# ZikangYuan/sr_livo

Hardware: AMD Instinct MI355X
Metric: sweeps/s (full ESIKF solve of a 64k-pt Livox sweep vs 1M-pt voxel map) (higher is better)
Workload: dtype f64; 1 GPU; HEADLINE: stream of 4 distinct 65536-keypoint livox sweeps (own poses and priors), 978481-pt voxel map (1000000 target), max_num_residuals=2147483647, r=1, K=20; one full ESIKF solve per sweep, every sweep crosses PCIe once (uploaded on the copy stream during the solve before it: resident in HBM when its solve starts); sweeps drawn with seeds 20251309 + 100 j, keeping those that take sweep 0's 2 E; parallelism=single GPU

## Files before the change

include/srlivo_hip_debug.h:

```cpp
#ifndef SRLIVO_HIP_DEBUG_H
#define SRLIVO_HIP_DEBUG_H

#include "srlivo_hip.h"

#ifdef __cplusplus
extern "C" {
#endif

int srl_debug_set_select_mode(srl_ctx *ctx, int select_mode);

int srl_debug_radix_sort_pairs(srl_ctx *ctx, const uint32_t *keys, int n, int bits, uint32_t *keys_sorted, uint32_t *positions_sorted);

int srl_debug_color_map_rebuilds(srl_ctx *ctx, int32_t *voxel_table, int32_t *grid_table);

int srl_debug_set_frame_order_mode(srl_ctx *ctx, int mode);
int srl_debug_frame_order_used(srl_ctx *ctx, int *used);

int srl_debug_set_gather_counts(srl_ctx *ctx, int nranks, int rank, const int64_t *counts);

int srl_debug_set_ablate(srl_ctx *ctx, int bits);
int srl_debug_set_fused_reduce(srl_ctx *ctx, int enable);
int srl_debug_set_bound_culling(srl_ctx *ctx, int enable);
int srl_debug_set_pose_box(srl_ctx *ctx, int kind);
int srl_debug_set_arm_linger(srl_ctx *ctx, double host_linger_us, double kernel_linger_us);
int srl_debug_pass_stamps(srl_ctx *ctx, int enable, long long *gpu_out, long long *host_out);
int srl_debug_frame_timing(srl_ctx *ctx, int enable, double out16[16]);
int srl_debug_set_frame_epoch(srl_ctx *ctx, int frames_to_wrap);
int srl_debug_set_launch_shape(srl_ctx *ctx, int keypoints_per_wave, int waves_per_workgroup);
int srl_debug_set_search_select_mode(srl_ctx *ctx, int select_mode);
int srl_debug_heap_topk(const double *distances, int n, int K, int32_t *out_index);
int srl_debug_device_sqrt(srl_ctx *ctx, const double *in, int n, double *out);
int srl_debug_block_times(srl_ctx *ctx, double *out, int max_blocks, int *nblocks);

#ifdef __cplusplus
}
#endif
#endif
```

sr_livo_amd/capi.py:

```python
import ctypes as C
import os
import re

import numpy as np

_HERE = os.path.dirname(os.path.abspath(__file__))
LIB_PATH = os.environ.get("SRL_LIB_PATH") or os.path.join(_HERE, "libsrlivo_hip.so")
INCLUDE_DIR = os.path.join(os.path.dirname(_HERE), "include")

SRL_OK = 0
SRL_ERR_NO_DEVICE = -1
SRL_ERR_BAD_ARG = -3
SRL_ERR_UNSUPPORTED = -4
SRL_ERR_COMM = -7
SRL_ERR_NAN_PLANARITY = -8
SRL_ERR_NOT_ENOUGH_RESIDUALS = -9
SRL_COMM_ID_BYTES = 128


SRL_PEER_HANDLE_BYTES = 64


class SrlError(RuntimeError):
    def __init__(self, status, what, detail=""):
# ... 184 lines not shown
        "srl_fetch_residuals": ([p, p, p, p, p, p, p], C.c_int),
        "srl_search_neighbors": ([p, p, C.c_int, C.c_int, C.c_double, C.c_int, C.c_int, p, p, p], C.c_int),
        "srl_transform_points": ([p, p, C.c_int, dp, dp, dp, dp, p], C.c_int),
        "srl_frame_upload": ([p, p, C.c_int], C.c_int),
        "srl_frame_undistort": ([p, p, p, p, C.c_int, p, C.c_int, C.c_double, C.c_int, dp, dp, p, p], C.c_int),
        "srl_frame_take": ([p, p, C.c_int], C.c_int),
        "srl_frame_subsample": ([p, p, C.c_int, C.c_double, C.POINTER(C.c_int)], C.c_int),
        "srl_frame_take_subsampled": ([p, p, C.c_int, p, p, p], C.c_int),
        "srl_frame_size": ([p, C.POINTER(C.c_int)], C.c_int),
        "srl_frame_select_keypoints": ([p, dp, dp, dp, dp, C.c_double, p, C.POINTER(C.c_int)], C.c_int),
        "srl_frame_commit_report": ([p, dp, dp, dp, dp, C.c_double, C.c_int, C.c_double, C.c_int, p, p, p, C.POINTER(C.c_int),
                                     C.POINTER(C.c_int)], C.c_int),
        "srl_frame_commit": ([p, dp, dp, dp, dp, C.c_double, C.c_int, C.c_double, C.c_int, p, C.POINTER(C.c_int)], C.c_int),
        "srl_comm_unique_id": ([p], C.c_int),
        "srl_comm_init_rank": ([p, C.c_int, C.c_int, p], C.c_int),
        "srl_comm_destroy": ([p], C.c_int),
        "srl_comm_set_library": ([C.c_char_p], C.c_int),
        "srl_comm_suspend": ([p, C.c_int], C.c_int),
        "srl_comm_info": ([p, C.POINTER(C.c_int), C.POINTER(C.c_int), C.POINTER(C.c_int), C.POINTER(C.c_int), C.POINTER(C.c_int64)], C.c_int),
        "srl_comm_set_host_callbacks": ([p, C.c_int, C.c_int, ALLREDUCE_FN, ALLGATHER_FN, p], C.c_int),
        "srl_debug_set_gather_counts": ([p, C.c_int, C.c_int, C.POINTER(C.c_int64)], C.c_int),
        "srl_peer_export": ([p, p, C.POINTER(p)], C.c_int),
        "srl_peer_attach": ([p, C.c_int, C.c_int, p, C.POINTER(p)], C.c_int),
        "srl_peer_set_deadline_ms": ([p, C.c_int], C.c_int),
        "srl_peer_stats": ([p, C.POINTER(C.c_int64), C.POINTER(C.c_int)], C.c_int),
        "srl_peer_detach": ([p], C.c_int),
        "srl_shard_range": ([C.c_int, C.c_int, C.c_int, C.POINTER(C.c_int), C.POINTER(C.c_int)], None),
        "srl_shard_budget": ([C.c_int, C.POINTER(C.c_int64), C.c_int, C.c_int, C.POINTER(C.c_int64), C.POINTER(C.c_int)], None),
        "srl_get_timing": ([p, C.POINTER(Timing)], C.c_int),
        "srl_debug_block_times": ([p, p, C.c_int, C.POINTER(C.c_int)], C.c_int),
        "srl_debug_set_ablate": ([p, C.c_int], C.c_int),
        "srl_debug_set_fused_reduce": ([p, C.c_int], C.c_int),
        "srl_debug_set_bound_culling": ([p, C.c_int], C.c_int),
        "srl_debug_set_pose_box": ([p, C.c_int], C.c_int),
        "srl_debug_set_arm_linger": ([p, C.c_double, C.c_double], C.c_int),
        "srl_debug_pass_stamps": ([p, C.c_int, p, p], C.c_int),
        "srl_debug_frame_timing": ([p, C.c_int, p], C.c_int),
        "srl_debug_set_frame_epoch": ([p, C.c_int], C.c_int),
        "srl_set_armed_launch": ([p, C.c_int], C.c_int),
        "srl_disarm": ([p], C.c_int),
        "srl_solve_end": ([p], C.c_int),
        "srl_get_arm_stats": ([p, C.POINTER(C.c_uint64)], C.c_int),
        "srl_debug_set_launch_shape": ([p, C.c_int, C.c_int], C.c_int),
        "srl_debug_set_search_select_mode": ([p, C.c_int], C.c_int),
        "srl_debug_set_select_mode": ([p, C.c_int], C.c_int),
        "srl_debug_set_frame_order_mode": ([p, C.c_int], C.c_int),
        "srl_debug_radix_sort_pairs": ([p, p, C.c_int, C.c_int, p, p], C.c_int),
        "srl_debug_frame_order_used": ([p, C.POINTER(C.c_int)], C.c_int),
        "srl_debug_heap_topk": ([p, C.c_int, C.c_int, p], C.c_int),
        "srl_debug_device_sqrt": ([p, p, C.c_int, p], C.c_int),
        "srl_set_profiling": ([p, C.c_int], C.c_int),
        "srl_set_profiling_period": ([p, C.c_int], C.c_int),
        "srl_timing_mark": ([p], C.c_int),
        "srl_lio_create": ([C.c_int, C.POINTER(p)], C.c_int),
        "srl_lio_destroy": ([p], C.c_int),
        "srl_lio_ctx": ([p], p),
        "srl_lio_last_error": ([p], C.c_char_p),
        "srl_lio_set_extrinsics": ([p, dp, dp], C.c_int),
        "srl_lio_set_laser_point_cov": ([p, C.c_double], C.c_int),
        "srl_lio_last_solve_launches": ([p, C.POINTER(C.c_int)], C.c_int),
        "srl_lio_eskf_get_state": ([p, dp], C.c_int),
        "srl_lio_eskf_set_state": ([p, dp], C.c_int),
        "srl_lio_eskf_get_cov": ([p, dp], C.c_int),
        "srl_lio_eskf_set_cov": ([p, dp], C.c_int),
        "srl_lio_eskf_set_noise": ([p, C.c_double, C.c_double, C.c_double, C.c_double], C.c_int),
        "srl_lio_eskf_init_imu": ([p, dp, dp], C.c_int),
# ... 463 lines not shown
        return node.value if rc == 0 else None

    def fetch_neighbors(self, K=20):
        _, n, _ = self.sweep_shard()
        ids = np.empty((n, K), dtype=np.int32)
        status = np.empty(n, dtype=np.uint8)
        ncand = np.empty(n, dtype=np.int32)
        self._chk(self.lib.srl_fetch_neighbors(self.h, _ptr(ids), _ptr(status), _ptr(ncand)), "srl_fetch_neighbors")
        return ids, status, ncand

    def fetch_residuals(self):
        _, n, _ = self.sweep_shard()
        normal = np.empty((n, 3)); a2d = np.empty(n); w = np.empty(n); off = np.empty(n); d = np.empty(n); J = np.empty((n, 6))
        self._chk(self.lib.srl_fetch_residuals(self.h, _ptr(normal), _ptr(a2d), _ptr(w), _ptr(off), _ptr(d), _ptr(J)), "srl_fetch_residuals")
        return dict(normal=normal, a2D=a2d, weight=w, norm_offset=off, distance=d, jacobian=J)

    def search_neighbors(self, world_xyz, nb=1, size=1.0, K=20, thr=1):
        q = _f64(world_xyz, (-1, 3))
        ids = np.empty((len(q), K), dtype=np.int32)
        xyz = np.empty((len(q), K, 3), dtype=np.float32)
        nf = np.empty(len(q), dtype=np.int32)
        self._chk(self.lib.srl_search_neighbors(self.h, _ptr(q), len(q), nb, size, K, thr, _ptr(ids), _ptr(xyz), _ptr(nf)), "srl_search_neighbors")
        return ids, xyz, nf

    def set_launch_shape(self, kpw, wpb):
        self._chk(self.lib.srl_debug_set_launch_shape(self.h, int(kpw), int(wpb)), "srl_debug_set_launch_shape")

    def set_fused_reduce(self, on):
        self._chk(self.lib.srl_debug_set_fused_reduce(self.h, 1 if on else 0), "srl_debug_set_fused_reduce")

    def set_bound_culling(self, on):
        self._chk(self.lib.srl_debug_set_bound_culling(self.h, 1 if on else 0), "srl_debug_set_bound_culling")

    def set_search_select_mode(self, mode):
        self._chk(self.lib.srl_debug_set_search_select_mode(self.h, int(mode)), "srl_debug_set_search_select_mode")

    def set_armed_launch(self, on):
        mode = int(on) if on in (0, 1, 2) and not isinstance(on, bool) else (1 if on else 0)
        self._chk(self.lib.srl_set_armed_launch(self.h, mode), "srl_set_armed_launch")

    def solve_end(self):
        self._chk(self.lib.srl_solve_end(self.h), "srl_solve_end")

    def disarm(self):
        self._chk(self.lib.srl_disarm(self.h), "srl_disarm")

    def arm_stats(self):
        out = (C.c_uint64 * 4)()
        self._chk(self.lib.srl_get_arm_stats(self.h, out), "srl_get_arm_stats")
        return dict(zip(("armed", "fired", "cancelled", "expired"), (int(v) for v in out)))

    def set_pose_box(self, kind):
        self._chk(self.lib.srl_debug_set_pose_box(self.h, int(kind)), "srl_debug_set_pose_box")

    FRAME_STAGES = ("upload", "select_group", "select_download", "select_host_order", "select_gather", "commit_transform", "commit_download",
                    "insert_sort", "insert_segments", "insert_lookup_create", "insert_replay")

    def set_frame_epoch(self, frames_to_wrap):
        self._chk(self.lib.srl_debug_set_frame_epoch(self.h, int(frames_to_wrap)), "srl_debug_set_frame_epoch")

    def frame_timing(self, enable=True):
        out = np.zeros(16)
        self._chk(self.lib.srl_debug_frame_timing(self.h, 1 if enable else 0, _ptr(out)), "srl_debug_frame_timing")
        return dict(zip(self.FRAME_STAGES, (float(v) for v in out)))

    def pass_stamps(self, enable=True, read=True):
# ... 582 lines not shown
```

sr_livo_amd/csrc/srl_capi.cpp:

```cpp
#include "../../include/srlivo_hip.h"
#include "../../include/srlivo_hip_debug.h"
#include "host/srl_la.h"
#include "srl_device.h"
#include "srl_hash.h"
#include "srl_heap.h"

#include <hip/hip_runtime.h>
#include <sched.h>

#include <algorithm>
#include <atomic>
#include <chrono>
#include <climits>
#include <cstdio>
#include <cstdlib>
#include <cstring>
#include <mutex>
#include <string>
#include <vector>

struct SrlMapState;
int srl_map_insert_device(struct srl_ctx *ctx, const double *world_xyz, int n, double voxel_size, int cap,
                          double min_distance_points, int min_num_points, int *num_added);

#include "srl_ctx.h"
int srl_map_insert_report_device(srl_ctx *ctx, const double *world_xyz, int n, double voxel_size, int cap, double min_distance_points, int min_num_points,
                                 double ref_z, uint8_t *outcome, srl_cloud_point *cloud, int *num_cloud, int *num_added);

namespace {

unsigned next_pow2(unsigned v) { unsigned p = 1; while (p < v) p <<= 1; return p; }
inline long long steady_ns() { return std::chrono::duration_cast<std::chrono::nanoseconds>(std::chrono::steady_clock::now().time_since_epoch()).count(); }

constexpr int SRL_MAX_DEVICES = 64;
std::atomic<int> g_live_ctx[SRL_MAX_DEVICES];
inline int live_contexts(int device) { return (device >= 0 && device < SRL_MAX_DEVICES) ? g_live_ctx[device].load(std::memory_order_relaxed) : 1; }

int ensure_work(srl_ctx *ctx, int n) {
    if (n <= ctx->work_cap) return SRL_OK;
    const int cap = std::max(n, 1024);
    const int nblocks = std::max((cap + SRL_KPB - 1) / SRL_KPB, 1024 + 8);
    int rc;
    if ((rc = ensure(ctx, ctx->d_rec, (size_t)cap * 8))) return rc;
    if ((rc = ensure(ctx, ctx->d_status, (size_t)cap))) return rc;
    if ((rc = ensure(ctx, ctx->d_bound, (size_t)cap * 4))) return rc;
    ctx->bound_n = 0;
    if ((rc = ensure(ctx, ctx->d_partials, (size_t)nblocks * SRL_PART_STRIDE))) return rc;
    if ((rc = ensure(ctx, ctx->d_binfo, (size_t)nblocks))) return rc;
    ctx->work_cap = cap;
    ctx->block_cap = nblocks;
    return SRL_OK;
}

bool srl_is_pinned(const void *p) {
    hipPointerAttribute_t attr;
    if (hipPointerGetAttributes(&attr, p) != hipSuccess) { (void)hipGetLastError(); return false; }
    return attr.type == hipMemoryTypeHost;
}

int srl_ring_init(srl_ctx *ctx) {
    if (ctx->h_ring) return SRL_OK;
    HIPCHK(ctx, hipHostMalloc((void **)&ctx->h_ring, (size_t)srl_ctx::RING_SLOTS * srl_ctx::RING_SLOT_BYTES, hipHostMallocDefault));
    for (int i = 0; i < srl_ctx::RING_SLOTS; i++) { HIPCHK(ctx, hipEventCreateWithFlags(&ctx->ring_ev[i], hipEventDisableTiming)); ctx->ring_busy[i] = false; }
    return SRL_OK;
}

int ensure_taps(srl_ctx *ctx, int n, int K) {
    if (n <= ctx->tap_cap && K <= ctx->tap_K) return SRL_OK;
    const int cap = std::max(n, ctx->tap_cap), kk = std::max(K, ctx->tap_K);
    int rc;
    if ((rc = ensure(ctx, ctx->d_tap_ids, (size_t)cap * kk))) return rc;
    if ((rc = ensure(ctx, ctx->d_tap_ncand, (size_t)cap))) return rc;
    if ((rc = ensure(ctx, ctx->d_tap_normal, (size_t)cap * 3))) return rc;
    if ((rc = ensure(ctx, ctx->d_tap_a2d, (size_t)cap))) return rc;
    if ((rc = ensure(ctx, ctx->d_tap_offset, (size_t)cap))) return rc;
    ctx->tap_cap = cap;
    ctx->tap_K = kk;
    return SRL_OK;
}
// ... 66 lines not shown
    }
    {
        const size_t row_bytes = (size_t)(SRL_FUSED_MAX_BLOCKS + SRL_FUSED_MAX_GROUPS) * SRL_ROW_GRANULES * 8;
        if (hipMalloc((void **)&ctx->d_granules, row_bytes) != hipSuccess || hipMemset(ctx->d_granules, 0, row_bytes) != hipSuccess) { delete ctx; return SRL_ERR_HIP; }
    }
    if (hipHostMalloc((void **)&ctx->h_mail, sizeof(SrlMailbox), hipHostMallocCoherent | hipHostMallocMapped) != hipSuccess) {
        delete ctx;
        return SRL_ERR_HIP;
    }
    std::memset(ctx->h_mail, 0, sizeof(SrlMailbox));
    for (int i = 0; i < 4; i++) hipEventCreate(&ctx->ev[i]);
    if (device < SRL_MAX_DEVICES) g_live_ctx[device].fetch_add(1, std::memory_order_relaxed);
    ctx->counted = true;
    *out = ctx;
    return SRL_OK;
}

int srl_ctx_destroy(srl_ctx *ctx) {
    if (!ctx) return SRL_OK;
    hipSetDevice(ctx->device);
    if (ctx->counted && ctx->device < SRL_MAX_DEVICES) g_live_ctx[ctx->device].fetch_sub(1, std::memory_order_relaxed);
    if (ctx->armed) srl_ctx_disarm(ctx);
    if (ctx->stream) hipStreamSynchronize(ctx->stream);
    if (ctx->copy_stream) hipStreamSynchronize(ctx->copy_stream);
    if (ctx->color) srl_color_map_destroy(ctx);
    if (ctx->pose_box_pinned) hipHostFree(ctx->pose_box_pinned);
    if (ctx->pose_box_dev) hipFree(ctx->pose_box_dev);
    if (ctx->d_pose_relay) hipFree(ctx->d_pose_relay);
    if (ctx->comm && srl_rccl()) srl_rccl()->CommDestroy(ctx->comm);
    if (ctx->parked_comm && srl_rccl()) srl_rccl()->CommDestroy(ctx->parked_comm);
    if (ctx->d_sub_kept) hipFree(ctx->d_sub_kept);
    if (ctx->d_sub_seen) hipFree(ctx->d_sub_seen);
    void *bufs[] = {ctx->d_corr_in, ctx->d_corr_rel, ctx->d_corr_imu, ctx->d_corr_raw, ctx->d_corr_seg, ctx->d_frame_raw, ctx->d_frame_world, ctx->d_table, ctx->d_slabs, ctx->d_raw, ctx->d_rec, ctx->d_status, ctx->d_partials, ctx->d_binfo,
                    ctx->d_out, ctx->d_count, ctx->d_bound, ctx->d_granules, ctx->d_rec_granules, ctx->d_raw_next, ctx->d_stage_next, ctx->d_stage_cur, ctx->d_tap_ids, ctx->d_tap_ncand, ctx->d_tap_normal, ctx->d_tap_a2d,
                    ctx->d_tap_offset, ctx->d_gather, ctx->d_peer, ctx->d_mail};
    for (int r = 0; r < SRL_MAX_PEERS; r++) if (ctx->peer_mapped[r]) hipIpcCloseMemHandle(ctx->peer_mapped[r]);
    if (ctx->d_inbox) hipFree(ctx->d_inbox);
    for (void *b : bufs) if (b) hipFree(b);
    if (ctx->h_out) hipHostFree(ctx->h_out);
    if (ctx->h_count) hipHostFree(ctx->h_count);
    if (ctx->h_mail) hipHostFree(ctx->h_mail);
    if (ctx->h_arm_stamps) hipHostFree(ctx->h_arm_stamps);
    if (ctx->h_scratch) hipHostFree(ctx->h_scratch);
    if (ctx->h_frame_x) hipHostFree(ctx->h_frame_x);
    for (SrlEpochTable *t : {&ctx->sel_table, &ctx->ins_table}) { if (t->keyw) hipFree(t->keyw); if (t->minw) hipFree(t->minw); }
    if (ctx->d_frame_sync) hipFree(ctx->d_frame_sync);
    if (ctx->d_tr1_sched) hipFree(ctx->d_tr1_sched);
    if (ctx->h_insert_cnt) hipHostFree(ctx->h_insert_cnt);
    if (ctx->ev_insert) hipEventDestroy(ctx->ev_insert);
    if (ctx->ev_world) hipEventDestroy(ctx->ev_world);
    if (ctx->ev_frame_read) hipEventDestroy(ctx->ev_frame_read);
    if (ctx->h_ring) { hipHostFree(ctx->h_ring); for (int i = 0; i < srl_ctx::RING_SLOTS; i++) if (ctx->ring_ev[i]) hipEventDestroy(ctx->ring_ev[i]); }
    for (auto &b : ctx->pool_free) hipFree(b.p);
    ctx->pool_free.clear();
    for (int i = 0; i < 4; i++) if (ctx->ev[i]) hipEventDestroy(ctx->ev[i]);
    for (int i = 0; i < srl_ctx::PROF_RING; i++) for (int k = 0; k < 2; k++) if (ctx->ring[i][k]) hipEventDestroy(ctx->ring[i][k]);
    for (int sl = 0; sl < 2; sl++) for (int k = 0; k < 2; k++) if (ctx->up_ev[sl][k]) hipEventDestroy(ctx->up_ev[sl][k]);
    if (ctx->upload_ev) hipEventDestroy(ctx->upload_ev);
    if (ctx->copy_stream) { hipStreamSynchronize(ctx->copy_stream); hipStreamDestroy(ctx->copy_stream); }
    if (ctx->prefix_stream) { hipStreamSynchronize(ctx->prefix_stream); hipStreamDestroy(ctx->prefix_stream); }
    if (ctx->stream) hipStreamDestroy(ctx->stream);
    delete ctx;
    return SRL_OK;
}

const char *srl_last_error(const srl_ctx *ctx) { return ctx ? ctx->err.c_str() : "null context"; }

int srl_map_upload(srl_ctx *ctx, const int16_t *keys_xyz, const int32_t *counts, const float *xyz, int V, int cap) {
    if (!ctx || V < 0 || (V > 0 && (!keys_xyz || !counts || !xyz))) return SRL_ERR_BAD_ARG;
    SRL_DISARM(ctx);
    if (cap != SRL_VOXEL_CAP) { ctx->err = "max_num_points_in_voxel must be 20"; return SRL_ERR_UNSUPPORTED; }
    HIPCHK(ctx, hipSetDevice(ctx->device));
    { const int rcs = srl_map_settle(ctx); if (rcs) return rcs; }
    ctx->bound_n = 0;
    const unsigned slab_cap = std::max<unsigned>(1024u, (unsigned)V + (unsigned)V / 2u + 4096u);
    if (slab_cap > SRL_MAX_SLABS) { ctx->err = "map too large: slab byte offsets are 32-bit (16.7 M voxels)"; return SRL_ERR_UNSUPPORTED; }
    const unsigned table_cap = next_pow2(std::max<unsigned>(2048u, SRL_TABLE_FACTOR * slab_cap));
    std::vector<SrlSlab> slabs((size_t)V);
    std::vector<SrlMapSlot> table((size_t)table_cap);
    for (auto &s : table) { s.key = SRL_EMPTY_KEY; s.slab = 0; s.count = 0; }
    long long npts = 0;
    const unsigned mask = table_cap - 1;
    for (int v = 0; v < V; v++) {
        SrlSlab &s = slabs[v];
        std::memset(&s, 0, sizeof s);
        const int c = counts[v];
        if (c < 0 || c > cap) { ctx->err = "voxel count out of range"; return SRL_ERR_BAD_ARG; }
        for (int i = 0; i < c; i++)
            for (int d = 0; d < 3; d++) s.xyz[i][d] = xyz[((size_t)v * cap + i) * 3 + d];
        s.count = (unsigned)c;
        s.key = srl_pack_key(keys_xyz[3 * v], keys_xyz[3 * v + 1], keys_xyz[3 * v + 2]);
        npts += c;
        unsigned h = srl_hash_key(s.key) & mask;
        while (table[h].key != SRL_EMPTY_KEY) {
            if (table[h].key == s.key) { ctx->err = "duplicate voxel key in upload"; return SRL_ERR_BAD_ARG; }
            h = (h + 1) & mask;
        }
        table[h].key = s.key;
        table[h].slab = (unsigned)v;
        table[h].count = (unsigned)c;
    }
    if (ctx->d_slabs) { HIPCHK(ctx, hipFree(ctx->d_slabs)); ctx->d_slabs = nullptr; }
    if (ctx->d_table) { HIPCHK(ctx, hipFree(ctx->d_table)); ctx->d_table = nullptr; }
    HIPCHK(ctx, hipMalloc((void **)&ctx->d_slabs, ((size_t)slab_cap + 1) * SRL_SLAB_BYTES));
    HIPCHK(ctx, hipMemsetD32Async((hipDeviceptr_t)(ctx->d_slabs + (size_t)slab_cap * SRL_SLAB_BYTES), 0x7f800000, SRL_SLAB_BYTES / 4, ctx->stream));
    HIPCHK(ctx, hipMalloc((void **)&ctx->d_table, (size_t)table_cap * sizeof(SrlMapSlot)));
    HIPCHK(ctx, hipMemsetAsync(ctx->d_slabs, 0, (size_t)slab_cap * SRL_SLAB_BYTES, ctx->stream));
// ... 78 lines not shown
        std::memcpy(ctx->h_ring + (size_t)slot * srl_ctx::RING_SLOT_BYTES, src + off, len);
        {
            hipError_t e__ = hipMemcpyAsync(reinterpret_cast<char *>(d_stage) + off, ctx->h_ring + (size_t)slot * srl_ctx::RING_SLOT_BYTES, len,
                                            hipMemcpyHostToDevice, st);
            if (e__ != hipSuccess) {
                char buf[256];
                std::snprintf(buf, sizeof buf, "ring upload: %s (dst %p + %zu, ring %p slot %d, len %zu, stream %p, main stream %p)", hipGetErrorString(e__),
                              (void *)d_stage, off, (void *)ctx->h_ring, slot, len, (void *)st, (void *)ctx->stream);
                ctx->err = buf;
                return SRL_ERR_HIP;
            }
        }
        HIPCHK(ctx, hipEventRecord(ctx->ring_ev[slot], st));
        ctx->ring_busy[slot] = true;
        off += len;
    }
    return SRL_OK;
}
}

int srl_sweep_upload(srl_ctx *ctx, const double *raw_xyz, int n) {
    if (!ctx || n < 0 || (n > 0 && !raw_xyz)) return SRL_ERR_BAD_ARG;
    SRL_DISARM(ctx);
    HIPCHK(ctx, hipSetDevice(ctx->device));
    int b = 0, cnt = 0;
    srl_shard_range(n, ctx->nranks, ctx->rank, &b, &cnt);
    ctx->total_n = n;
    ctx->shard_begin = b;
    ctx->n = cnt;
    ctx->sweep_loaded = true;
    ctx->taps_valid = false;
    ctx->passes_in_solve = 0;
    ctx->tail_pending = false;
    ctx->bound_n = 0;
    if (cnt > ctx->sweep_cap) {
        const int cap = std::max(cnt, 1024);
        int rc = ensure(ctx, ctx->d_raw, (size_t)cap * 3);
        if (rc) return rc;
        ctx->sweep_cap = cap;
    }
    int rc = ensure_work(ctx, cnt);
    if (rc) return rc;
    if (cnt > 0) {
        int rcu = upload_aos(ctx, reinterpret_cast<const char *>(raw_xyz + (size_t)b * 3), (size_t)cnt * 3 * sizeof(double), ctx->d_rec, ctx->stream);
        if (rcu) return rcu;
        HIPCHK(ctx, srl_launch_aos_to_soa(ctx->d_rec, cnt, ctx->d_raw, ctx->d_raw + ctx->sweep_cap, ctx->d_raw + 2 * (size_t)ctx->sweep_cap, ctx->stream));
    }
    ctx->soa_valid_n = cnt;
    return SRL_OK;
}

int srl_sweep_wait(srl_ctx *ctx) {
    if (!ctx) return SRL_ERR_BAD_ARG;
    SRL_DISARM(ctx);
    if (ctx->upload_pending) {
        HIPCHK(ctx, hipSetDevice(ctx->device));
        HIPCHK(ctx, hipEventSynchronize(ctx->upload_ev));
        if (ctx->prefix_stream) HIPCHK(ctx, hipStreamSynchronize(ctx->prefix_stream));
        ctx->upload_pending = false;
    }
    return SRL_OK;
}

int srl_sweep_prefetch(srl_ctx *ctx, const double *raw_xyz, int n) {
    if (!ctx || n < 0 || (n > 0 && !raw_xyz)) return SRL_ERR_BAD_ARG;
    HIPCHK(ctx, hipSetDevice(ctx->device));
    if (!ctx->copy_stream) SRL_DISARM(ctx);
// ... 31 lines not shown
            ctx->up_one_dma[slot] = true;
        }
    } else {
        ctx->up_one_dma[slot] = true;
    }
    HIPCHK(ctx, hipEventRecord(ctx->up_ev[slot][1], ctx->copy_stream));
    ctx->next_ready = ctx->up_ev[slot][1];
    ctx->next_slot = slot; ctx->next_prefix_n = ctx->up_one_dma[slot] ? cnt : pre;
    ctx->next_n = cnt; ctx->next_begin = b; ctx->next_total = n;
    return SRL_OK;
}

int srl_sweep_swap(srl_ctx *ctx) {
    if (!ctx) return SRL_ERR_BAD_ARG;
    if (ctx->next_n < 0) { SRL_DISARM(ctx); ctx->err = "srl_sweep_swap: nothing prefetched"; return SRL_ERR_NO_SWEEP; }
    HIPCHK(ctx, hipSetDevice(ctx->device));
    const bool one_dma = ctx->up_one_dma[ctx->next_slot];
    hipEvent_t ev_full = ctx->up_ev[ctx->next_slot][1], ev_pre = ctx->up_ev[ctx->next_slot][one_dma ? 1 : 0];
    hipError_t up_pre = hipEventQuery(ev_pre);
    hipError_t up = (one_dma || up_pre != hipSuccess) ? up_pre : hipEventQuery(ev_full);
    if (up_pre == hipErrorNotReady && ctx->armed && ctx->next_n <= ctx->work_cap) {
        const long long t_give_up = steady_ns() + 25000;
        while ((up_pre = hipEventQuery(ev_pre)) == hipErrorNotReady && steady_ns() < t_give_up) { }
    }
    for (hipError_t e : {up, up_pre})
        if (e != hipSuccess && e != hipErrorNotReady) { ctx->err = std::string("hipEventQuery: ") + hipGetErrorString(e); return SRL_ERR_HIP; }
    if (up_pre != hipSuccess || ctx->next_n > ctx->work_cap) SRL_DISARM(ctx);
    if (up_pre != hipSuccess) {
        HIPCHK(ctx, hipStreamWaitEvent(ctx->stream, ev_full, 0));
        if (!one_dma) HIPCHK(ctx, hipStreamWaitEvent(ctx->stream, ev_pre, 0));
        up = hipSuccess;
    }
    ctx->tail_pending = up != hipSuccess;
    ctx->bound_n = 0;
    ctx->cur_slot = ctx->next_slot;
    ctx->cur_prefix_n = up == hipSuccess ? ctx->next_n : ctx->next_prefix_n;
    ctx->passes_in_solve = 0;
    std::swap(ctx->d_raw, ctx->d_raw_next);
    std::swap(ctx->sweep_cap, ctx->next_cap);
    std::swap(ctx->d_stage_cur, ctx->d_stage_next);
    std::swap(ctx->stage_cur_cap, ctx->stage_next_cap);
    ctx->soa_valid_n = 0;
    ctx->n = ctx->next_n; ctx->shard_begin = ctx->next_begin; ctx->total_n = ctx->next_total;
    ctx->next_n = -1;
    ctx->sweep_loaded = true;
    ctx->taps_valid = false;
    return ensure_work(ctx, ctx->n);
}

int srl_thread_pin_to_gpu_numa(srl_ctx *ctx, int *numa_node) {
    if (!ctx) return SRL_ERR_BAD_ARG;
    if (numa_node) *numa_node = -1;
    char bus[64] = {0};
    if (hipDeviceGetPCIBusId(bus, (int)sizeof bus, ctx->device) != hipSuccess) { (void)hipGetLastError(); return SRL_ERR_UNSUPPORTED; }
    for (char *c = bus; *c; ++c) if (*c >= 'A' && *c <= 'F') *c = (char)(*c - 'A' + 'a');
    const std::string base = std::string("/sys/bus/pci/devices/") + bus;
    int node = -1;
    if (FILE *f = std::fopen((base + "/numa_node").c_str(), "r")) { if (std::fscanf(f, "%d", &node) != 1) node = -1; std::fclose(f); }
    char list[1024] = {0};
    if (FILE *f = std::fopen((base + "/local_cpulist").c_str(), "r")) { if (!std::fgets(list, (int)sizeof list, f)) list[0] = 0; std::fclose(f); }
    if (node < 0 || !list[0]) return SRL_ERR_UNSUPPORTED;
    cpu_set_t allowed, want;
    CPU_ZERO(&want);
    if (sched_getaffinity(0, sizeof allowed, &allowed) != 0) return SRL_ERR_UNSUPPORTED;
    int any = 0;
    for (const char *p = list; *p && *p != '\n';) {
        char *end = nullptr;
// ... 380 lines not shown
    a.size_voxel = o->size_voxel_map;
    a.max_dist = o->max_dist_to_plane_icp;
    {
        double lw = std::abs(o->weight_alpha), ln = std::abs(o->weight_neighborhood);
        const double sum = lw + ln;
        lw /= sum;
        ln /= sum;
        a.lambda_w = lw;
        a.lambda_n = ln;
    }
    a.power_planarity = o->power_planarity;
    a.nbr_scale = o->max_dist_to_plane_icp * o->min_number_neighbors;
    a.K = p.K;
    a.min_nb = o->min_number_neighbors;
    a.thr_cap = p.thr;
    a.select_mode = ctx->select_mode;
    a.ablate = ctx->ablate;
    a.stamps = ctx->h_arm_stamps;
    a.rec = ctx->d_rec;
    a.status = ctx->d_status;
    a.partials = ctx->d_partials;
    a.binfo = ctx->d_binfo;
    if (ctx->taps) {
        a.tap_ids = ctx->d_tap_ids;
        a.tap_ncand = ctx->d_tap_ncand;
        a.tap_normal = ctx->d_tap_normal;
        a.tap_a2d = ctx->d_tap_a2d;
        a.tap_offset = ctx->d_tap_offset;
    }
    {
        float sv = (float)o->size_voxel_map;
        int sv_bits; std::memcpy(&sv_bits, &sv, 4);
        const int sig[4] = {p.K, p.nb, p.thr, sv_bits};
        if (std::memcmp(sig, ctx->bound_sig, sizeof sig) != 0) { ctx->bound_n = 0; std::memcpy(ctx->bound_sig, sig, sizeof sig); }
        a.bound_out = ctx->d_bound;
        a.bound_in = ctx->bound_mode != 0 ? ctx->d_bound : nullptr;
        a.bound_use = a.bound_in ? std::min(ctx->bound_n, n_eff) : 0;
    }
    if (p.fused) {
        a.granules = ctx->d_granules;
        a.mailbox = p.transport == Transport::rccl ? ctx->d_mail : ctx->h_mail;
        a.mail_tagged = p.tagged_mail ? 1 : 0;
    }
    if (p.fuse_cut) {
        a.rec_granules = ctx->d_rec_granules;
        a.cut_max = o->max_num_residuals;
    }
}

static int grow_pass_buffers(srl_ctx *ctx, const PassPlan &p) {
    int rc;
    ctx->taps_valid = false;
    if (ctx->taps) {
        if ((rc = ensure_taps(ctx, ctx->n, p.K))) return rc;
        if (ctx->n > 0) {
            HIPCHK(ctx, hipMemsetAsync(ctx->d_tap_ids, 0xFF, (size_t)ctx->n * p.K * sizeof(int), ctx->stream));
            HIPCHK(ctx, hipMemsetAsync(ctx->d_tap_normal, 0, (size_t)ctx->n * 3 * sizeof(double), ctx->stream));
            HIPCHK(ctx, hipMemsetAsync(ctx->d_tap_a2d, 0, (size_t)ctx->n * sizeof(double), ctx->stream));
            HIPCHK(ctx, hipMemsetAsync(ctx->d_tap_offset, 0, (size_t)ctx->n * sizeof(double), ctx->stream));
        }
    }
    ctx->last_nblocks = p.nblocks;
    if (p.nblocks > ctx->block_cap) {
        if ((rc = ensure(ctx, ctx->d_partials, (size_t)p.nblocks * SRL_PART_STRIDE))) return rc;
        if ((rc = ensure(ctx, ctx->d_binfo, (size_t)p.nblocks))) return rc;
        ctx->block_cap = p.nblocks;
    }
    if (ctx->profiling == 2 && ctx->ring_head - ctx->ring_tail >= (unsigned)srl_ctx::PROF_RING && (rc = drain_ring(ctx, true))) return rc;
    if (p.fused && p.transport == Transport::rccl && !ctx->d_mail && (rc = ensure(ctx, ctx->d_mail, 1))) return rc;
    const size_t need = (size_t)p.nblocks * p.kpb * 16;
    if (p.fuse_cut && need > ctx->rec_granule_cap) {
        if ((rc = ensure(ctx, ctx->d_rec_granules, need))) return rc;
        HIPCHK(ctx, hipMemsetAsync(ctx->d_rec_granules, 0, need * sizeof(unsigned long long), ctx->stream));
        ctx->rec_granule_cap = need;
    }
    return SRL_OK;
}

struct ExchangeTag { unsigned long long seq; unsigned epoch; int slot; };
static ExchangeTag exchange_tag(unsigned long long seq) {
    if ((unsigned)seq == 0u) ++seq;
    return {seq, (unsigned)seq, (int)(seq & 1ull)};
}
static ExchangeTag next_exchange(srl_ctx *ctx) {
    const ExchangeTag t = exchange_tag(ctx->peer_seq + 1);
    ctx->peer_seq = t.seq;
    return t;
}

static SrlAssocArgs arm_signature(const SrlAssocArgs &src) {
    SrlAssocArgs sg = src;
    std::memset(sg.Rn, 0, sizeof sg.Rn); std::memset(sg.R, 0, sizeof sg.R); std::memset(sg.t, 0, sizeof sg.t);
    std::memset(sg.t_last, 0, sizeof sg.t_last);
    sg.pose_box = nullptr; sg.pose_relay = nullptr; sg.pose_relayed = 0; sg.pose_epoch = 0; sg.arm_linger_ticks = 0;
    sg.raw_x = sg.raw_y = sg.raw_z = nullptr; sg.alt_x = sg.alt_y = sg.alt_z = nullptr; sg.n = 0; sg.aos = nullptr; sg.alt_aos = nullptr;
    sg.bound_use = 0;
    return sg;
}

static int fire_or_cancel(srl_ctx *ctx, const PassPlan &p, SrlAssocArgs &a, unsigned long long &seq_now, bool &fired) {
    fired = false;
    bool needs_tail = false;
    if (ctx->tail_pending) {
        if (hipEventQuery(ctx->up_ev[ctx->cur_slot][1]) == hipSuccess) { ctx->tail_pending = false; ctx->cur_prefix_n = ctx->n; }
        else needs_tail = a.n > ctx->cur_prefix_n;
        (void)hipGetLastError();
    }
    if (!ctx->armed) return SRL_OK;
    const SrlAssocArgs sg = arm_signature(a);
    const double age_us = (double)(steady_ns() - ctx->armed_at_ns) * 1e-3;
    const bool on_raw = a.raw_x == ctx->armed_raw && ctx->sweep_cap == ctx->armed_raw_cap && a.aos == nullptr;
    const bool on_alt = !on_raw && ctx->armed_alt != nullptr && a.raw_x == ctx->armed_alt && ctx->sweep_cap == ctx->armed_alt_cap &&
                        a.aos != nullptr && a.aos == ctx->armed_alt_aos;
    if (p.arm_ok && !needs_tail && age_us < ctx->arm_host_linger_us && p.nb == ctx->armed_nb && p.kpw == ctx->armed_kpw &&
        p.nblocks <= ctx->armed_nblocks && (on_raw || on_alt) && std::memcmp(&sg, &ctx->armed_sig, sizeof sg) == 0) {
        pose_box_write(ctx, a.Rn, a.R, a.t, (unsigned)seq_now, SRL_ARM_GO | (on_alt ? SRL_ARM_ALT : 0u), (unsigned)a.n, a.t_last);
        ctx->armed = false;
        ctx->armed_ring = -1;
        ctx->arm_stats[1]++;
        ctx->cur_measured = ctx->armed_measured;
        ctx->cur_gen = ctx->armed_gen;
        fired = true;
        return SRL_OK;
    }
    if (const int rc = srl_ctx_disarm(ctx)) return rc;
    seq_now = ++ctx->seq;
    if (p.fused) a.seq = seq_now;
    return SRL_OK;
}

static int prof_role(const srl_ctx *ctx) {
    if (ctx->prof_period <= 1) return 2;
    const unsigned long long r = ctx->prof_count % (unsigned long long)ctx->prof_period;
    return r == 1 ? 2 : (r == 0 ? 1 : 0);
}

static int launch_assoc(srl_ctx *ctx, const PassPlan &p, const SrlAssocArgs &args, bool armed) {
    if (!armed && ctx->tail_pending) {
        HIPCHK(ctx, hipStreamWaitEvent(ctx->stream, ctx->up_ev[ctx->cur_slot][1], 0));
        ctx->tail_pending = false; ctx->cur_prefix_n = ctx->n;
    }
    const bool prof = ctx->profiling == 1, prof_light = ctx->profiling == 2;
    const int role = prof_light ? prof_role(ctx) : 0;
    int prev = -1;
    if (armed && role != 0) {
        int rc;
        if (ctx->ring_head - ctx->ring_tail >= (unsigned)srl_ctx::PROF_RING - 2 && (rc = drain_ring(ctx, true))) return rc;
        if (ctx->ring_head != 0 && !ctx->ring_void[(ctx->ring_head - 1) % srl_ctx::PROF_RING] && ctx->ring_last_count == (long long)ctx->prof_count - 1)
            prev = (int)((ctx->ring_head - 1) % srl_ctx::PROF_RING);
    }
    const unsigned slot = ctx->ring_head % srl_ctx::PROF_RING;
    if (prof) HIPCHK(ctx, hipEventRecord(ctx->ev[0], ctx->stream));
    if (role == 2 && prev < 0) HIPCHK(ctx, hipEventRecord(ctx->ring[slot][0], ctx->stream));
    HIPCHK(ctx, srl_launch_assoc(args, p.nb, p.kpw, p.wpb, ctx->stream));
    if (prof) HIPCHK(ctx, hipEventRecord(ctx->ev[1], ctx->stream));
    if (role != 0) {
        HIPCHK(ctx, hipEventRecord(ctx->ring[slot][1], ctx->stream));
        ctx->ring_prev[slot] = prev; ctx->ring_marker[slot] = role == 1; ctx->ring_void[slot] = false; ctx->ring_gen[slot] = ctx->timing_gen;
        ctx->ring_last_count = (long long)ctx->prof_count;
        ctx->ring_head++;
    }
    if (prof_light) ctx->prof_count++;
    const bool measured = !prof_light || role == 2;
    if (armed) { ctx->armed_ring = role != 0 ? (int)slot : -1; ctx->armed_measured = measured; ctx->armed_gen = ctx->timing_gen; }
    else { ctx->cur_measured = measured; ctx->cur_gen = ctx->timing_gen; }
    return SRL_OK;
}

static bool arm_wanted(const srl_ctx *ctx) {
    return ctx->arm_mode == 2 ||
           (live_contexts(ctx->device) <= 1 && !ctx->peer_shares_device && !ctx->comm_shares_device &&
            (ctx->next_n >= 0 || ctx->expected_passes == 0 || ctx->passes_in_solve + 1 < ctx->expected_passes));
}

static int arm_next(srl_ctx *ctx, const PassPlan &p, const SrlAssocArgs &a) {
    int rc;
    if ((rc = ensure_pose_box(ctx))) return rc;
    SrlAssocArgs nx = a;
    nx.seq = ctx->seq + 1;
    nx.bound_use = a.bound_in ? a.n : 0;
    const bool has_alt = ctx->d_raw_next != nullptr && ctx->next_cap > 0 && ctx->d_stage_next != nullptr;
    nx.aos = nullptr;
    nx.alt_aos = has_alt ? ctx->d_stage_next : nullptr;
    nx.alt_x = has_alt ? ctx->d_raw_next : nullptr;
    nx.alt_y = has_alt ? ctx->d_raw_next + ctx->next_cap : nullptr;
    nx.alt_z = has_alt ? ctx->d_raw_next + 2 * (size_t)ctx->next_cap : nullptr;
    if (p.transport == Transport::peer) {
        const ExchangeTag t = exchange_tag(ctx->peer_seq + 1);
        nx.peer_epoch = t.epoch;
        nx.peer_slot = t.slot;
    }
    nx.pose_box = ctx->h_pose_box;
    nx.pose_relay = ctx->d_pose_relay;
    nx.pose_relayed = ctx->pose_box_kind == 1 ? 0 : 1;
    nx.pose_epoch = (unsigned)nx.seq;
    nx.arm_linger_ticks = ctx->arm_linger_ticks;
    if ((rc = launch_assoc(ctx, p, nx, true))) return rc;
    ctx->armed_sig = arm_signature(nx);
    ctx->armed_nb = p.nb; ctx->armed_kpw = p.kpw; ctx->armed_nblocks = p.nblocks;
    ctx->armed_raw = nx.raw_x; ctx->armed_raw_cap = ctx->sweep_cap;
    ctx->armed_alt = nx.alt_x; ctx->armed_alt_cap = has_alt ? ctx->next_cap : 0; ctx->armed_alt_aos = nx.alt_aos;
    ctx->armed_at_ns = steady_ns();
    ctx->armed = true;
    ctx->arm_stats[0]++;
    return SRL_OK;
}

static int reduce_unfused(srl_ctx *ctx, const PassPlan &p, const srl_icp_opts *o, int n_eff, unsigned long long seq) {
    int64_t budget = o->max_num_residuals;
    int mode = 0;
    const long long *gather = nullptr;
    if (p.transport == Transport::single || !p.cut) {
        srl_shard_budget(o->max_num_residuals, nullptr, ctx->nranks, ctx->rank, &budget, &mode);
// ... 113 lines not shown
    if (ctx->h_out->pad != 0 || ctx->h_out->d_timeout > 0.5) {
        ctx->err = "fused final reduction timed out waiting for a workgroup's row";
        if (fired && p.transport == Transport::rccl) ctx->arm_stats[3]++;
        return SRL_INTERNAL_FUSED_TIMEOUT;
    }
    return SRL_OK;
}

static int finish_pass(srl_ctx *ctx, const PassPlan &p, const srl_icp_opts *o, const SrlAssocArgs &a, int n_eff, long long last_visited_local,
                       unsigned long long seq, bool fired, srl_normal_eq *out) {
    const SrlDevOut &r = *ctx->h_out;
    const long long visited_total = (long long)(r.d_visited + 0.5);
    if (p.fused && !p.fuse_cut) {
        const long long expect = ctx->nranks > 1 ? (long long)ctx->total_n : (long long)n_eff;
        if (visited_total != expect) {
            char buf[256];
            std::snprintf(buf, sizeof buf, "fused pass visited %lld of %lld keypoints (fired %d, seq %llu; residuals %.0f, time-out flag %.0f, marker %lld)", visited_total, expect,
                          (int)fired, seq, r.d_num_res, r.d_timeout, (long long)r.pad);
            ctx->err = buf;
            return SRL_ERR_HIP;
        }
    }
    std::memcpy(out->HtH, r.HtH, sizeof out->HtH);
    std::memcpy(out->Hth, r.Hth, sizeof out->Hth);
    out->loss_sum = r.loss;
    out->num_residuals = (int32_t)(r.d_num_res + 0.5);
    out->success = out->num_residuals >= o->min_number_neighbors ? 1 : 0;
    out->sum_candidates = (int64_t)(r.d_sum_pk + 0.5);
    out->last_visited = visited_total - 1;
    out->nan_error = r.d_nan > 0.5 ? 1 : 0;
    out->num_fallback = (int32_t)(r.d_fallback + 0.5);

    if (a.aos != nullptr && n_eff > ctx->soa_valid_n) ctx->soa_valid_n = n_eff;
    ctx->bound_n = n_eff;
    ctx->last_K = p.K;
    ctx->last_nb = p.nb;
    ctx->last_visited_local = last_visited_local;
    ctx->taps_valid = ctx->taps;
    return SRL_OK;
}

struct PassClock { std::chrono::steady_clock::time_point entry, prep, launched, enq, res; };

static long long clock_ns(std::chrono::steady_clock::time_point t) {
    return std::chrono::duration_cast<std::chrono::nanoseconds>(t.time_since_epoch()).count();
}

static int account_pass(srl_ctx *ctx, const PassPlan &p, int n_eff, const PassClock &c) {
    using us = std::chrono::duration<double, std::micro>;
    using ms = std::chrono::duration<double, std::milli>;
    const bool prof = ctx->profiling == 1, prof_light = ctx->profiling == 2;
    if (prof) {
        HIPCHK(ctx, hipEventSynchronize(ctx->ev[3]));
        hipEventElapsedTime(&ctx->timing.assoc_ms, ctx->ev[0], ctx->ev[1]);
        hipEventElapsedTime(&ctx->timing.reduce_ms, ctx->ev[1], ctx->ev[2]);
        hipEventElapsedTime(&ctx->timing.total_ms, ctx->ev[0], ctx->ev[3]);
        ctx->timing.calls += 1;
        ctx->timing.sum_assoc_ms += ctx->timing.assoc_ms;
        ctx->timing.sum_reduce_ms += ctx->timing.reduce_ms;
        ctx->timing.sum_total_ms += ctx->timing.total_ms;
        ctx->timing.sum_keypoints += n_eff;
        const auto t_end = std::chrono::steady_clock::now();
        ctx->timing.sum_host_launch_us += us(c.enq - c.entry).count();
        ctx->timing.sum_host_wait_us += us(c.res - c.enq).count();
        ctx->timing.sum_host_total_us += us(t_end - c.entry).count();
    }
// ... 154 lines not shown
    HIPCHK(ctx, hipMemcpyAsync(d_in, raw_xyz, (size_t)n * 3 * sizeof(double), hipMemcpyHostToDevice, ctx->stream));
    SrlXform X;
    const srl::Mat3 R = srl::Quat(q[0], q[1], q[2], q[3]).toRotationMatrix();
    std::memcpy(X.R, R.a, sizeof X.R);
    std::memcpy(X.t, t, sizeof X.t);
    std::memcpy(X.R_il, R_il, sizeof X.R_il);
    std::memcpy(X.t_il, t_il, sizeof X.t_il);
    HIPCHK(ctx, srl_launch_transform(d_in, n, X, d_o, ctx->stream));
    HIPCHK(ctx, hipMemcpyAsync(out_xyz, d_o, (size_t)n * 3 * sizeof(double), hipMemcpyDeviceToHost, ctx->stream));
    HIPCHK(ctx, hipStreamSynchronize(ctx->stream));
    return SRL_OK;
}

int srl_debug_set_ablate(srl_ctx *ctx, int bits) {
    if (!ctx) return SRL_ERR_BAD_ARG;
    SRL_DISARM(ctx);
    ctx->ablate = bits;
    return SRL_OK;
}
int srl_debug_set_launch_shape(srl_ctx *ctx, int keypoints_per_wave, int waves_per_workgroup) {
    if (!ctx) return SRL_ERR_BAD_ARG;
    SRL_DISARM(ctx);
    if (keypoints_per_wave != 0 && keypoints_per_wave != 2 && keypoints_per_wave != 3 && keypoints_per_wave != 6 && keypoints_per_wave != 12 && keypoints_per_wave != 4 && keypoints_per_wave != 8 && keypoints_per_wave != 16) return SRL_ERR_BAD_ARG;
    if (waves_per_workgroup != 0 && waves_per_workgroup != 4 && waves_per_workgroup != 16) return SRL_ERR_BAD_ARG;
    ctx->force_kpw = keypoints_per_wave;
    ctx->force_wpb = waves_per_workgroup;
    return SRL_OK;
}
int srl_debug_set_bound_culling(srl_ctx *ctx, int enable) {
    if (!ctx) return SRL_ERR_BAD_ARG;
    SRL_DISARM(ctx);
    ctx->bound_mode = enable ? 1 : 0;
    ctx->bound_n = 0;
    return SRL_OK;
}
int srl_debug_set_fused_reduce(srl_ctx *ctx, int enable) {
    if (!ctx) return SRL_ERR_BAD_ARG;
    SRL_DISARM(ctx);
    ctx->fuse_reduce = enable != 0;
    return SRL_OK;
}
int srl_debug_set_select_mode(srl_ctx *ctx, int select_mode) {
    if (!ctx || select_mode < 0 || select_mode > 5) return SRL_ERR_BAD_ARG;
    SRL_DISARM(ctx);
    ctx->select_mode = select_mode;
    return SRL_OK;
}
int srl_debug_set_frame_order_mode(srl_ctx *ctx, int mode) {
    if (!ctx || mode < 0 || mode > 1) return SRL_ERR_BAD_ARG;
    ctx->frame_order_mode = mode;
    return SRL_OK;
}
int srl_debug_frame_order_used(srl_ctx *ctx, int *used) {
    if (!ctx || !used) return SRL_ERR_BAD_ARG;
    *used = ctx->frame_order_used;
    return SRL_OK;
}
int srl_debug_set_search_select_mode(srl_ctx *ctx, int select_mode) {
    if (!ctx || select_mode < 0 || select_mode > 5) return SRL_ERR_BAD_ARG;
    ctx->search_select_mode = select_mode;
    return SRL_OK;
}
int srl_debug_heap_topk(const double *distances, int n, int K, int32_t *out_index) {
    if (n < 0 || K < 1 || K > SRL_MAX_NEIGHBORS || (n > 0 && !distances) || !out_index) return SRL_ERR_BAD_ARG;
    double hd[SRL_MAX_NEIGHBORS];
    int he[SRL_MAX_NEIGHBORS];
// ... 381 lines not shown
```

sr_livo_amd/csrc/srl_ctx.h:

```cpp
#pragma once
#include "../../include/srlivo_hip.h"
#include "srl_device.h"
#include "host/tr1_relation.h"

#include <hip/hip_runtime.h>
#include "srl_rccl.h"

#include <string>
#include <vector>

struct SrlEpochTable {
    unsigned long long *keyw = nullptr;
    unsigned long long *minw = nullptr;
    unsigned cap = 0;
    unsigned epoch16 = 0;
    unsigned counter32 = 0;
};

#define SRL_PEER_POISON_WORD SRL_PEER_INBOX_GRANULES
#define SRL_PEER_DEVICE_WORD (SRL_PEER_INBOX_GRANULES + 1)
#define SRL_PEER_INBOX_ALLOC_GRANULES (SRL_PEER_INBOX_GRANULES + 8)

struct srl_ctx {
    int device = 0;
// ... 9 lines not shown
    long long num_points = 0;

    double *d_raw = nullptr;
    int sweep_cap = 0;
    int n = 0;
    int shard_begin = 0;
    int total_n = 0;
    bool sweep_loaded = false;
    int search_select_mode = 0;
    int select_mode = 0;
    int ablate = 0;
    void (*overlap_fn)(void *) = nullptr;
    void *overlap_user = nullptr;

    double *d_raw_next = nullptr;
    double *d_stage_next = nullptr;
    double *d_stage_cur = nullptr;
    int soa_valid_n = 0;
    int next_cap = 0, stage_next_cap = 0, stage_cur_cap = 0;
    int next_n = -1, next_begin = 0, next_total = 0;
    hipStream_t copy_stream = nullptr;
    hipStream_t prefix_stream = nullptr;
    int num_cu = 256;
    hipEvent_t next_ready = nullptr;
    hipEvent_t up_ev[2][2] = {};
    bool up_one_dma[2] = {true, true};
    int next_slot = 0;
    int next_prefix_n = 0;
    int prefix_hint = 0;
    float *d_bound = nullptr;
    int bound_n = 0;
    int bound_sig[4] = {0, 0, 0, 0};
    int bound_mode = 1;
    bool tail_pending = false;
    int cur_slot = 0, cur_prefix_n = 0;

    double *d_frame_raw = nullptr;
    double *d_frame_world = nullptr;
    int frame_cap = 0;
    int frame_n = -1;
    int frame_world_n = -1;
    bool frame_world_seen = false;
    struct SrlColorMap *color = nullptr;
    double *d_corr_in = nullptr, *d_corr_rel = nullptr, *d_corr_imu = nullptr, *d_corr_raw = nullptr;
    int *d_corr_seg = nullptr;
    int corr_cap = 0;
    int corr_n = -1;
    int *d_sub_kept = nullptr;
    unsigned *d_sub_seen = nullptr;
    int sub_cap = 0;
    int sub_n = -1;
    unsigned sub_seen_tag = 0;

    bool frame_timing = false;
    double frame_stage_us[16] = {};
    long long frame_stage_last_ns = 0;

    hipEvent_t upload_ev = nullptr;
    bool upload_pending = false;

    static constexpr int RING_SLOTS = 4;
    static constexpr int RING_SLOT_BYTES = 256 * 1024;
    char *h_ring = nullptr;
    hipEvent_t ring_ev[RING_SLOTS] = {};
    bool ring_busy[RING_SLOTS] = {};
    unsigned ring_next = 0;
// ... 245 lines not shown
```

sr_livo_amd/csrc/srl_device.h:

```cpp
#pragma once
#include <hip/hip_runtime.h>
#include <stddef.h>
#include <stdint.h>


#define SRL_CAP 20
#define SRL_SLAB_BYTES 256
#define SRL_MAX_SLABS 16777215u
#ifndef SRL_KPB
#define SRL_KPB 64
#endif
#ifndef SRL_ASSOC_WAVES_PER_SIMD
#define SRL_ASSOC_WAVES_PER_SIMD 4
#endif
#define SRL_BLOCK 256
#define SRL_SURV_CAP 64
#define SRL_WAVE_SCRATCH 2048
#define SRL_MAXK 32
#define SRL_EMPTY_KEY 0xFFFFFFFFFFFFFFFFull
#define SRL_TABLE_FACTOR 4u
#define SRL_PART_STRIDE 32
#define SRL_ROW_GRANULES 128
#define SRL_FUSED_MAX_BLOCKS 2048
#define SRL_FUSED_GROUP 256
#define SRL_FUSED_MAX_GROUPS (SRL_FUSED_MAX_BLOCKS / SRL_FUSED_GROUP)
#define SRL_FUSED_CUT_MAX_KPB 64

enum : int {
    SRL_ROW_HTH = 0,
    SRL_ROW_HTH_V = 21,
    SRL_ROW_LOSS = 27,
    SRL_ROW_SUMS = 28,
    SRL_ROW_ACCEPTED = 28,
    SRL_ROW_SUM_PK = 29,
    SRL_ROW_NAN = 30,
    SRL_ROW_FALLBACK = 31,
};
static_assert(SRL_ROW_FALLBACK + 1 == SRL_PART_STRIDE, "a row is SRL_PART_STRIDE doubles");
#define SRL_ROW_TIMEOUT_MARK 0x7117ll
struct SrlRowPair { int ia, ib; };
__host__ __device__ constexpr SrlRowPair srl_row_tri_pair(int c) {
    int r = 0;
    while (c >= 6 - r) { c -= 6 - r; ++r; }
    return SrlRowPair{r, r + c};
}
__host__ __device__ constexpr int srl_row_tri_comp(int i0, int i1) {
    const int ia = i0 < i1 ? i0 : i1, ib = i0 < i1 ? i1 : i0;
    return SRL_ROW_HTH + ia * 6 - (ia * (ia - 1)) / 2 + (ib - ia);
}
__host__ __device__ constexpr SrlRowPair srl_row_pair(int c) {
    return c < SRL_ROW_HTH_V ? srl_row_tri_pair(c) : (c < SRL_ROW_LOSS ? SrlRowPair{c - SRL_ROW_HTH_V, 6} : SrlRowPair{7, 7});
// ... 3 lines not shown
}
constexpr bool srl_row_layout_ok() {
    int c = 0;
    for (int ia = 0; ia < 6; ++ia)
        for (int ib = ia; ib < 6; ++ib, ++c) {
            const SrlRowPair p = srl_row_tri_pair(c);
            if (p.ia != ia || p.ib != ib || srl_row_tri_comp(ia, ib) != c || srl_row_tri_comp(ib, ia) != c) return false;
        }
    return c == SRL_ROW_HTH_V;
}
static_assert(srl_row_layout_ok(), "component -> (ia, ib) -> component is the identity and walks the upper triangle row by row");

struct SrlMapSlot {
    unsigned long long key;
    unsigned slab;
    unsigned count;
};
static_assert(sizeof(SrlMapSlot) == 16, "slot must be 16 bytes");

struct SrlSlab {
    float xyz[SRL_CAP][3];
    unsigned count;
    unsigned pad;
    unsigned long long key;
};
static_assert(sizeof(SrlSlab) == SRL_SLAB_BYTES, "slab must be 256 bytes");

struct SrlBlockInfo {
    int accepted;
    unsigned sum_pk;
    int nan_first;
    int num_fallback;
    int planes;
    int pad[3];
};
static_assert(sizeof(SrlBlockInfo) == 32, "block info is 32 bytes");

struct SrlDevOut {
    double HtH[36];
    double Hth[6];
    double loss;
    double d_num_res;
    double d_total_accepted;
    double d_sum_pk;
    double d_nan;
    double d_fallback;
    double d_visited;
    double d_timeout;
    long long last_visited;
    long long pad;
};

struct SrlMailbox {
    SrlDevOut out;
    unsigned long long seq;
    unsigned long long expired;
    unsigned long long pad[10];
    unsigned long long g[2 * (sizeof(SrlDevOut) / 8)];
};
static_assert(sizeof(SrlDevOut) == 52 * 8 && offsetof(SrlDevOut, pad) == 51 * 8, "SrlDevOut is 52 words, the marker word last");
static_assert(offsetof(SrlMailbox, g) % 64 == 0, "the tagged record starts on a cache line");

#define SRL_POSE_BOX_CTRL 42
#define SRL_POSE_BOX_N 43
#define SRL_POSE_BOX_TLAST 44
#define SRL_POSE_BOX_USED 50
#define SRL_POSE_BOX_WRITTEN 56
// ... 32 lines not shown
    double t_il[3];
    double size_voxel;
    double max_dist;
    double lambda_w, lambda_n;
    double power_planarity;
    double nbr_scale;
    int K;
    int min_nb;
    int thr_cap;
    int select_mode;
    int ablate;
    unsigned long long *granules;
    unsigned long long *rec_granules;
    long long cut_max;
    SrlMailbox *mailbox;
    int mail_tagged;
    int pad_mail;
    unsigned long long seq;
    const unsigned long long *pose_box;
    const double *alt_x, *alt_y, *alt_z;
    const double *alt_aos;
    unsigned long long *pose_relay;
    int pose_relayed;
    int pad_relay;
    unsigned pose_epoch;
    unsigned arm_linger_ticks;
    long long *stamps;
    const SrlPeerTable *peer;
    unsigned peer_epoch;
    int peer_slot;
    const float *bound_in;
    float *bound_out;
    int bound_use;
    int pad_bound;
    double *rec;
    unsigned char *status;
    double *partials;
    SrlBlockInfo *binfo;
    int *tap_ids;
    int *tap_ncand;
    double *tap_normal;
    double *tap_a2d;
    double *tap_offset;
};

#define SRL_POSE_DOUBLES 24
static_assert(sizeof(SrlAssocArgs) <= 4096, "the struct travels in the kernarg segment");

struct SrlReduceArgs {
    const double *rec;
    const unsigned char *status;
    const double *partials;
    const SrlBlockInfo *binfo;
    int n;
    int nblocks;
    long long max_res;
    const long long *gather;
    int rank;
    int max_num_residuals;
    SrlDevOut *out;
    SrlMailbox *mailbox;
    unsigned long long seq;
    int kpb;
};

struct SrlSearchArgs {
    const double *q;
// ... 34 lines not shown
```

sr_livo_amd/csrc/srl_frame_kernels.hip:

```cpp
#include "srl_ctx.h"
#include "srl_frame_scratch.h"
#include "srl_hash.h"
#include "host/srl_la.h"
#include "host/tr1_order.h"


#include <algorithm>
#include <chrono>
#include <cstdio>
#include <cstdlib>
#include <cstring>
#include <vector>

int srl_map_insert_impl(srl_ctx *ctx, const double *world_xyz, bool on_device, int n, double voxel_size,
                        double min_distance_points, int min_num_points, int *num_added, bool defer_counters,
                        const SrlFrameTransform *xf = nullptr, int (*after_first_kernel)(srl_ctx *, void *) = nullptr, void *user = nullptr,
                        const SrlInsertReport *report = nullptr);

namespace {

using Xf = SrlXf;

__global__ void k_frame_world(const double *raw, int n, const Xf X, double *world) {
    const int i = blockIdx.x * blockDim.x + threadIdx.x;
// ... 768 lines not shown
        C.gather_raw = ctx->d_frame_raw; C.gx = sx; C.gy = sy; C.gz = sz;
        rc = grid_chain_enqueue(ctx, C, n, [&](const GroupArgs &G) {
            hipLaunchKernelGGL(k_select_group, dim3((n + 255) / 256), dim3(256), 0, st, ctx->d_frame_raw, n, X, sample_voxel_size, G);
        });
        if (rc) return rc;
        srl_stage_end(ctx, 1);
        tp1 = std::chrono::steady_clock::now();
        rc = grid_chain_wait(ctx, C, "keypoint selection");
        if (rc) return rc;
        srl_stage_end(ctx, 2);
        tp2 = std::chrono::steady_clock::now();
        m = C.m;
        rc = grid_chain_order(ctx, C);
        if (rc) return rc;
        srl_stage_end(ctx, 3);
        if (C.list_on_host) {
            tp3 = std::chrono::steady_clock::now();
            if (m > 0) {
                hipLaunchKernelGGL(k_gather_soa, dim3((m + 255) / 256), dim3(256), 0, st, ctx->d_frame_raw, C.h_list, m, sx, sy, sz);
                HIPCHK(ctx, hipGetLastError());
            }
        } else {
            tp3 = tp2;
            if (keypoint_index && m > 0) {
                HIPCHK(ctx, hipMemcpyAsync(C.h_list, C.d_list, (size_t)m * 4, hipMemcpyDeviceToHost, st));
                HIPCHK(ctx, hipStreamSynchronize(st));
            }
        }
        if (keypoint_index) std::memcpy(keypoint_index, C.h_list, (size_t)m * 4);
    } else {
        srl_stage_end(ctx, 3);
    }
    if (num_keypoints) *num_keypoints = m;
    ctx->total_n = m; ctx->shard_begin = 0; ctx->n = m; ctx->sweep_loaded = true; ctx->taps_valid = false; ctx->bound_n = 0; ctx->tail_pending = false;
    ctx->soa_valid_n = m; ctx->passes_in_solve = 0;
    if (n > 0) { const int rcm = srl_mark_frame_read(ctx); if (rcm) return rcm; }
    srl_stage_end(ctx, 4);
    if (trace) {
        const auto tp4 = std::chrono::steady_clock::now();
        auto us = [](std::chrono::steady_clock::time_point a, std::chrono::steady_clock::time_point b) { return std::chrono::duration<double, std::micro>(b - a).count(); };
        std::fprintf(stderr, "[srl_frame_select_keypoints] n %d -> %d (order %d): enqueue %.0f us, wait %.0f us, host order replay %.0f us, gather + rest %.0f us\n",
                     n, m, ctx->frame_order_used, us(tp0, tp1), us(tp1, tp2), us(tp2, tp3), us(tp3, tp4));
    }
    return SRL_OK;
}

}

namespace {
int frame_commit_impl(srl_ctx *ctx, const double q[4], const double t[3], const double R_il[9], const double t_il[3], double voxel_size, int cap,
                      double min_distance_points, int min_num_points, double *world_out, int *num_added, const SrlInsertReport *report) {
    if (!ctx || !q || !t || !R_il || !t_il) return SRL_ERR_BAD_ARG;
    SRL_DISARM(ctx);
    if (cap != SRL_VOXEL_CAP) { ctx->err = "max_num_points_in_voxel must be 20"; return SRL_ERR_UNSUPPORTED; }
    if (ctx->frame_n < 0 || !ctx->d_frame_raw) { ctx->err = "no frame uploaded"; return SRL_ERR_NO_SWEEP; }
    HIPCHK(ctx, hipSetDevice(ctx->device));
    const int n = ctx->frame_n;
    if (num_added) *num_added = 0;
    if (n == 0) return SRL_OK;
    SrlFrameTransform xf;
    xf.raw = ctx->d_frame_raw; xf.world = ctx->d_frame_world;
    fill_xf(xf.X, q, t, R_il, t_il);
    struct Download { double *world_out; int n; } dl = {world_out, n};
    auto world_ready = [](srl_ctx *c, void *user) -> int {
        const Download *d = static_cast<const Download *>(user);
        { const int rcm = srl_mark_frame_read(c); if (rcm) return rcm; }
        if (d->world_out) {
// ... 43 lines not shown
```

sr_livo_amd/csrc/srl_kernels.hip:

```cpp
#include "srl_device.h"
#include "srl_hash.h"
#include "srl_heap.h"

#include <math.h>
#include <type_traits>

namespace {

struct alignas(8) VoxEnt { unsigned slab; unsigned count; };
struct Surv { double d2; float x, y, z; unsigned id; };
static_assert(sizeof(Surv) == 24, "survivor record is 24 bytes");
static_assert(SRL_SURV_CAP * 24 + (SRL_MAXK + 1) * 8 <= SRL_WAVE_SCRATCH, "general-path scratch (survivors + sorted d2) must fit");
static_assert(64 * 8 + SRL_MAXK * 16 + SRL_MAXK * 4 <= SRL_WAVE_SCRATCH, "heap replay scratch must fit");

__device__ __forceinline__ int lane_id() {
    return __builtin_amdgcn_mbcnt_hi(~0u, __builtin_amdgcn_mbcnt_lo(~0u, 0));
}
__device__ __forceinline__ int lanes_below(unsigned long long m) {
    return __builtin_amdgcn_mbcnt_hi((unsigned)(m >> 32), __builtin_amdgcn_mbcnt_lo((unsigned)m, 0));
}

struct Cand { bool valid; double d2; float x, y, z; unsigned id; };

__device__ __forceinline__ Cand eval_cand(int e, int nv, const VoxEnt *vox, const unsigned char *slabs,
// ... 329 lines not shown
        const unsigned f_lo = found ? m_lo : (~m_lo & 0x7FFFFFFu), f_hi = found ? m_hi : (~m_hi & 0x7FFFFFFu);
        const int below = upper ? (int)__builtin_amdgcn_mbcnt_hi(f_hi, 0u) : (int)__builtin_amdgcn_mbcnt_lo(f_lo, 0u);
        const int nv_own = upper ? nv_b : nv_a;
        VoxEnt ve; ve.slab = found ? slab : 0u; ve.count = found ? cnt : 0u;
        vox[(upper ? 32 : 0) + (found ? below : nv_own + below)] = ve;
    }
    __builtin_amdgcn_wave_barrier();
    return nv_a | (nv_b << 8);
}

struct LdsSink {
    float *col;
    int row;
    int plane;
    int *tap_ids;
    __device__ __forceinline__ void put(int rank, float x, float y, float z, unsigned id) {
        float *p = col + rank * row;
        p[0] = x;
        p[plane] = y;
        p[2 * plane] = z;
        if (tap_ids) tap_ids[rank] = (int)id;
    }
};

struct alignas(16) SurvRec { float x, y, z; int code; };
#define SRL_PAIR_MAX_ROUNDS 4

__device__ __forceinline__ float d2_f32(float px, float py, float pz, float qx, float qy, float qz) {
#pragma clang fp contract(fast)
    const float dx = px - qx, dy = py - qy, dz = pz - qz;
    return dx * dx + dy * dy + dz * dz;
}

template <class Sink>
__device__ __forceinline__ int finish_survivors(double qx, double qy, double qz, int c, const VoxEnt *vox, int K, void *scratch,
                                                int lane, Sink &sink, double *tau_out = nullptr) {
    SurvRec *recs = reinterpret_cast<SurvRec *>(__builtin_assume_aligned(scratch, 16));
    double *keys = reinterpret_cast<double *>(reinterpret_cast<unsigned char *>(scratch) + 1024);
    double *sorted = keys + 66;
    __builtin_amdgcn_wave_barrier();
    const bool act = lane < c;
    SurvRec me;
    me.x = me.y = me.z = 0.0f; me.code = 0;
    double my = __builtin_huge_val();
    if (act) {
        me = recs[lane];
        const double dx = (double)me.x - qx;
        const double dy = (double)me.y - qy;
        const double dz = (double)me.z - qz;
        my = (dx * dx + dy * dy) + dz * dz;
    }
    keys[lane] = my;
    if (lane < K + 3) keys[64 + lane] = lane < 2 ? __builtin_huge_val() : __builtin_nan("");
    __builtin_amdgcn_wave_barrier();
    int rank = 0;
    if (c <= 32) {
        const double mine = keys[lane & 31];
        const double2 *kp = reinterpret_cast<const double2 *>(keys + (lane >> 5) * 16);
        int r = 0;
#pragma unroll
        for (int j = 0; j < 8; ++j) {
            const double2 kk = kp[j];
            r += (kk.x < mine) ? 1 : 0;
            r += (kk.y < mine) ? 1 : 0;
        }
        rank = r + __shfl_xor(r, 32);
    } else {
#pragma unroll 4
        for (int j = 0; j < c; j += 2) {
            const double2 kk = *reinterpret_cast<const double2 *>(keys + j);
            rank += (kk.x < my) ? 1 : 0;
            rank += (kk.y < my) ? 1 : 0;
        }
    }
    const bool win = act && rank < K;
    if (act && rank <= K) sorted[rank] = my;
    __builtin_amdgcn_wave_barrier();
    bool bad = false;
    if (lane >= 1 && lane <= K && lane < c) bad = !(sorted[lane] > sorted[lane - 1] * SRL_NEAR_TIE);
    if (__ballot(bad)) return SEL_TIE;
    if (tau_out && act && rank == K - 1) *tau_out = my;
    if (win) {
        const VoxEnt ve = vox[me.code >> 5];
        sink.put(rank, me.x, me.y, me.z, ve.slab * SRL_CAP + ((unsigned)me.code & 31u));
    }
    __builtin_amdgcn_wave_barrier();
    return SEL_DONE;
}

template <int R>
__device__ __forceinline__ void cand_issue(const VoxEnt *vox, const unsigned char *slabs, unsigned inf_off, const LaneRole &role,
                                           float (&px)[R], float (&py)[R], float (&pz)[R], int &total_out) {
    VoxEnt ve[R];
    const int cbase = role.c0 < 3 ? role.c0 : 0;
#pragma unroll
    for (int j = 0; j < R; ++j) ve[j] = vox[3 * j + cbase];
    const unsigned slot_eff = role.c0 < 3 ? (unsigned)role.slot : 31u;
    const unsigned slot_off = (unsigned)role.slot * 12u;
    unsigned off[R];
    int total = 0;
#pragma unroll
    for (int j = 0; j < R; ++j) {
        const bool h = slot_eff < ve[j].count;
        total += __popcll(__ballot(h));
        off[j] = h ? ve[j].slab * (unsigned)SRL_SLAB_BYTES + slot_off : inf_off;
    }
#pragma unroll
    for (int j = 0; j < R; ++j) {
        const float *p = reinterpret_cast<const float *>(slabs + off[j]);
        px[j] = p[0]; py[j] = p[1]; pz[j] = p[2];
    }
    total_out = total;
}

template <int R>
__device__ __forceinline__ float cand_d2f(const float (&px)[R], const float (&py)[R], const float (&pz)[R], const float *qf, float (&d2f)[R]) {
    const float qxf = qf[0], qyf = qf[1], qzf = qf[2];
    float lmin = __builtin_huge_valf();
#pragma unroll
    for (int j = 0; j < R; ++j) {
        d2f[j] = d2_f32(px[j], py[j], pz[j], qxf, qyf, qzf);
        lmin = fminf(lmin, d2f[j]);
    }
    return lmin;
}
__device__ __forceinline__ float thr_from_bisection(unsigned lo, const float *qf) {
    const float tau_f = __uint_as_float(lo | 0x3FFFFu);
    float thr = 3.4028235e38f;
    if (tau_f < __builtin_huge_valf()) thr = qf[3] + qf[4] * tau_f;
    return thr;
}
template <int R>
__device__ __forceinline__ void cand_compact(const float (&px)[R], const float (&py)[R], const float (&pz)[R], const float (&d2f)[R], float thr,
                                             const unsigned long long (&svm)[R], const LaneRole &role, SurvRec *recs) {
    const int code0 = (role.c0 << 5) | role.slot;
    int base = 0;
    (void)d2f; (void)thr;
#pragma unroll
    for (int j = 0; j < R; ++j) {
        {
            if (__builtin_amdgcn_inverse_ballot_w64(svm[j])) {
                SurvRec r; r.x = px[j]; r.y = py[j]; r.z = pz[j]; r.code = code0 + ((3 * j) << 5);
                recs[base + lanes_below(svm[j])] = r;
            }
            base += __popcll(svm[j]);
        }
    }
}

template <int R, class Sink>
__device__ __forceinline__ int cand_select(const float (&px)[R], const float (&py)[R], const float (&pz)[R], double qx, double qy, double qz,
                                           const float *qf, const VoxEnt *vox, int K, void *scratch, int lane, const LaneRole &role, Sink &sink,
                                           int ablate) {
    float d2f[R];
    const unsigned v = __float_as_uint(cand_d2f<R>(px, py, pz, qf, d2f));
    unsigned lo = 0;
#pragma unroll
    for (int bit = 30; bit >= 18; --bit) {
        const unsigned trial = lo | (1u << bit);
        const int cnt = __popcll(__ballot(v < trial));
        lo = (cnt < K) ? trial : lo;
    }
    const float thr = thr_from_bisection(lo, qf);
    SurvRec *recs = reinterpret_cast<SurvRec *>(__builtin_assume_aligned(scratch, 16));
    unsigned long long svm[R];
    int c = 0;
#pragma unroll
    for (int j = 0; j < R; ++j) {
        svm[j] = __ballot(d2f[j] <= thr);
        c += __popcll(svm[j]);
    }
    if (c > 64) return SEL_OVERFLOW;
    cand_compact<R>(px, py, pz, d2f, thr, svm, role, recs);
    if (ablate & 2) return SEL_DONE;
    return finish_survivors(qx, qy, qz, c, vox, K, scratch, lane, sink, reinterpret_cast<double *>(const_cast<float *>(qf) + 6));
}

template <int R, class Sink>
__device__ __forceinline__ int select_topk_f32_r(double qx, double qy, double qz, const float *qf, int nv, const VoxEnt *vox,
                                                  const unsigned char *slabs, unsigned inf_off, int K, void *scratch, int lane,
                                                  const LaneRole &role, Sink &sink, int &total_out, int ablate) {
    (void)nv;
    float px[R], py[R], pz[R];
    cand_issue<R>(vox, slabs, inf_off, role, px, py, pz, total_out);
    return cand_select<R>(px, py, pz, qx, qy, qz, qf, vox, K, scratch, lane, role, sink, ablate);
}

__device__ __forceinline__ int finish_pair(const double *qa, const double *qb, int ca, int cb, const VoxEnt *vox, int K, void *scratch, int lane,
                                           const LdsSink &sink_a, const LdsSink &sink_b, const float *qfa, const float *qfb) {
    SurvRec *recs = reinterpret_cast<SurvRec *>(__builtin_assume_aligned(scratch, 16));
    double *keys = reinterpret_cast<double *>(reinterpret_cast<unsigned char *>(scratch) + 1024);
    double *sorted = keys + 64;
    __builtin_amdgcn_wave_barrier();
    const int h = lane >> 5, i = lane & 31;
    const int c = h ? cb : ca;
    const bool act = i < c;
    const double *q = h ? qb : qa;
    SurvRec me;
    me.x = me.y = me.z = 0.0f; me.code = 0;
    double my = __builtin_huge_val();
    if (act) {
        me = recs[lane];
        const double dx = (double)me.x - q[0];
        const double dy = (double)me.y - q[1];
        const double dz = (double)me.z - q[2];
        my = (dx * dx + dy * dy) + dz * dz;
    }
    keys[lane] = my;
    sorted[lane] = __builtin_nan("");
    __builtin_amdgcn_wave_barrier();
    const double2 *kp = reinterpret_cast<const double2 *>(keys + 32 * h);
    int rank = 0;
#pragma unroll
    for (int j = 0; j < 16; ++j) {
        const double2 kk = kp[j];
        rank += (kk.x < my) ? 1 : 0;
        rank += (kk.y < my) ? 1 : 0;
    }
    const bool win = act && rank < K;
    if (act && rank <= K) sorted[32 * h + rank] = my;
    __builtin_amdgcn_wave_barrier();
    bool bad = false;
    if (i >= 1 && i <= K && i < c) bad = !(sorted[32 * h + i] > sorted[32 * h + i - 1] * SRL_NEAR_TIE);
    const unsigned long long bm = __ballot(bad);
    const bool tie_a = (unsigned)bm != 0u, tie_b = (unsigned)(bm >> 32) != 0u;
    if (win && !(h ? tie_b : tie_a)) {
        const VoxEnt ve = vox[32 * h + (me.code >> 5)];
        LdsSink s = sink_a;
        if (h) { s.col = sink_b.col; s.tap_ids = sink_b.tap_ids; }
        s.put(rank, me.x, me.y, me.z, ve.slab * SRL_CAP + ((unsigned)me.code & 31u));
        if (rank == K - 1) *reinterpret_cast<double *>(const_cast<float *>(h ? qfb : qfa) + 6) = my;
    }
    __builtin_amdgcn_wave_barrier();
    return (tie_a ? SEL_TIE : SEL_DONE) | ((tie_b ? SEL_TIE : SEL_DONE) << 8);
}

template <int R>
__device__ __forceinline__ int select_pair_f32_r(const double *qa, const double *qb, const float *qfa, const float *qfb, const VoxEnt *vox,
                                                 const unsigned char *slabs, unsigned inf_off, int K, void *scratch, int lane,
                                                 const LaneRole &role, LdsSink &sink_a, LdsSink &sink_b, int &total_a, int &total_b, int ablate) {
    float ax[R], ay[R], az[R], bx[R], by[R], bz[R];
    cand_issue<R>(vox, slabs, inf_off, role, ax, ay, az, total_a);
    cand_issue<R>(vox + 32, slabs, inf_off, role, bx, by, bz, total_b);
    float da[R], db[R];
    const unsigned va = __float_as_uint(cand_d2f<R>(ax, ay, az, qfa, da));
    const unsigned vb = __float_as_uint(cand_d2f<R>(bx, by, bz, qfb, db));
    constexpr unsigned BAND_LO = 0x38000000u, BAND_HI = 0x40000000u, BAND_LAST = 0x3FFC0000u;
    const unsigned ca_v = va < BAND_LO ? BAND_LO : (va > BAND_HI ? BAND_HI : va);
    const unsigned cb_v = vb < BAND_LO ? BAND_LO : (vb > BAND_HI ? BAND_HI : vb);
    unsigned lo_a = BAND_LO, lo_b = BAND_LO;
#pragma unroll
    for (int bit = 26; bit >= 18; --bit) {
        const unsigned ta = lo_a | (1u << bit), tb = lo_b | (1u << bit);
        const int cnt_a = __popcll(__ballot(ca_v < ta));
        const int cnt_b = __popcll(__ballot(cb_v < tb));
        lo_a = (cnt_a < K) ? ta : lo_a;
        lo_b = (cnt_b < K) ? tb : lo_b;
    }
    if (lo_a == BAND_LAST || lo_b == BAND_LAST) {
        lo_a = 0; lo_b = 0;
#pragma nounroll
        for (int bit = 30; bit >= 18; --bit) {
            const unsigned ta = lo_a | (1u << bit), tb = lo_b | (1u << bit);
            const int cnt_a = __popcll(__ballot(va < ta));
            const int cnt_b = __popcll(__ballot(vb < tb));
            lo_a = (cnt_a < K) ? ta : lo_a;
            lo_b = (cnt_b < K) ? tb : lo_b;
        }
    }
    const float thr_a = thr_from_bisection(lo_a, qfa), thr_b = thr_from_bisection(lo_b, qfb);
    unsigned long long sa[R], sb[R];
    int ca = 0, cb = 0;
#pragma unroll
    for (int j = 0; j < R; ++j) {
        sa[j] = __ballot(da[j] <= thr_a);
        sb[j] = __ballot(db[j] <= thr_b);
        ca += __popcll(sa[j]);
        cb += __popcll(sb[j]);
    }
    SurvRec *recs = reinterpret_cast<SurvRec *>(__builtin_assume_aligned(scratch, 16));
    if (ca <= 32 && cb <= 32 && K <= 31 && !(ablate & (2 | 512))) {
        cand_compact<R>(ax, ay, az, da, thr_a, sa, role, recs);
        cand_compact<R>(bx, by, bz, db, thr_b, sb, role, recs + 32);
        return finish_pair(qa, qb, ca, cb, vox, K, scratch, lane, sink_a, sink_b, qfa, qfb);
    }
    int done_a = SEL_OVERFLOW, done_b = SEL_OVERFLOW;
    if (ca <= 64) {
        cand_compact<R>(ax, ay, az, da, thr_a, sa, role, recs);
        done_a = (ablate & 2) ? SEL_DONE : finish_survivors(qa[0], qa[1], qa[2], ca, vox, K, scratch, lane, sink_a, reinterpret_cast<double *>(const_cast<float *>(qfa) + 6));
    }
    __builtin_amdgcn_wave_barrier();
    if (cb <= 64) {
        cand_compact<R>(bx, by, bz, db, thr_b, sb, role, recs);
        done_b = (ablate & 2) ? SEL_DONE : finish_survivors(qb[0], qb[1], qb[2], cb, vox + 32, K, scratch, lane, sink_b, reinterpret_cast<double *>(const_cast<float *>(qfb) + 6));
    }
    return done_a | (done_b << 8);
}

template <class Sink>
__device__ __forceinline__ int select_topk_f32(double qx, double qy, double qz, const float *qf, int nv, const VoxEnt *vox,
                                                const unsigned char *slabs, unsigned inf_off, int K, void *scratch, int lane,
                                                const LaneRole &role, Sink &sink, int &total_out, int ablate) {
    switch ((nv + 2) / 3) {
        case 0: case 1: case 2: case 3:
            return select_topk_f32_r<3>(qx, qy, qz, qf, nv, vox, slabs, inf_off, K, scratch, lane, role, sink, total_out, ablate);
        case 4: return select_topk_f32_r<4>(qx, qy, qz, qf, nv, vox, slabs, inf_off, K, scratch, lane, role, sink, total_out, ablate);
        case 5: return select_topk_f32_r<5>(qx, qy, qz, qf, nv, vox, slabs, inf_off, K, scratch, lane, role, sink, total_out, ablate);
        case 6: return select_topk_f32_r<6>(qx, qy, qz, qf, nv, vox, slabs, inf_off, K, scratch, lane, role, sink, total_out, ablate);
        case 7: return select_topk_f32_r<7>(qx, qy, qz, qf, nv, vox, slabs, inf_off, K, scratch, lane, role, sink, total_out, ablate);
        default: return select_topk_f32_r<9>(qx, qy, qz, qf, nv, vox, slabs, inf_off, K, scratch, lane, role, sink, total_out, ablate);
    }
}

template <class Sink>
__device__ __forceinline__ int select_topk_f32_loop(double qx, double qy, double qz, const float *qf, int nv, const VoxEnt *vox,
                                                    const unsigned char *slabs, unsigned inf_off, int K, void *scratch, int lane,
                                                    const LaneRole &role, Sink &sink, int &total_out) {
    const float kInfF = __builtin_huge_valf();
    const float qxf = qf[0], qyf = qf[1], qzf = qf[2];
    const int rounds = (nv + 2) / 3;
    const int cbase = role.c0 < 3 ? role.c0 : 0;
    const unsigned slot_eff = role.c0 < 3 ? (unsigned)role.slot : 31u;
    const unsigned slot_off = (unsigned)role.slot * 12u;
    float lmin = kInfF;
    int total = 0;
    constexpr int CH = 4;
    auto cand_off = [&](int j, bool &has) {
        const int jj = j < rounds ? j : rounds - 1;
        const VoxEnt ve = vox[3 * jj + cbase];
        has = (j < rounds) && (slot_eff < ve.count);
        return has ? ve.slab * (unsigned)SRL_SLAB_BYTES + slot_off : inf_off;
    };
    for (int j0 = 0; j0 < rounds; j0 += CH) {
        unsigned off[CH];
#pragma unroll
        for (int u = 0; u < CH; ++u) { bool h; off[u] = cand_off(j0 + u, h); total += __popcll(__ballot(h)); }
        float x[CH], y[CH], z[CH];
#pragma unroll
        for (int u = 0; u < CH; ++u) { const float *p = reinterpret_cast<const float *>(slabs + off[u]); x[u] = p[0]; y[u] = p[1]; z[u] = p[2]; }
#pragma unroll
        for (int u = 0; u < CH; ++u) lmin = fminf(lmin, d2_f32(x[u], y[u], z[u], qxf, qyf, qzf));
    }
    total_out = total;
// ... 30 lines not shown
            }
        }
    }
    if (c > 64) return SEL_OVERFLOW;
    return finish_survivors(qx, qy, qz, c, vox, K, scratch, lane, sink, reinterpret_cast<double *>(const_cast<float *>(qf) + 6));
}

struct D3 { double x, y, z; };
__device__ __forceinline__ D3 d3(double x, double y, double z) { D3 r; r.x = x; r.y = y; r.z = z; return r; }
__device__ __forceinline__ D3 sub(D3 a, D3 b) { return d3(a.x - b.x, a.y - b.y, a.z - b.z); }
__device__ __forceinline__ double dot3(D3 a, D3 b) { return (a.x * b.x + a.y * b.y) + a.z * b.z; }
__device__ __forceinline__ D3 matvec(const double *M, D3 v) {
    return d3((M[0] * v.x + M[1] * v.y) + M[2] * v.z, (M[3] * v.x + M[4] * v.y) + M[5] * v.z,
              (M[6] * v.x + M[7] * v.y) + M[8] * v.z);
}
__device__ __forceinline__ D3 add(D3 a, D3 b) { return d3(a.x + b.x, a.y + b.y, a.z + b.z); }
__device__ __forceinline__ double rcp_nr(double b) {
    double r = __builtin_amdgcn_rcp(b);
    r = __builtin_fma(__builtin_fma(-b, r, 1.0), r, r);
    r = __builtin_fma(__builtin_fma(-b, r, 1.0), r, r);
    return r;
}
__device__ __forceinline__ D3 normalized3_fast(D3 a) {
    const double z = dot3(a, a);
    if (z > 0.0) { const double inv = rcp_nr(sqrt(z)); return d3(a.x * inv, a.y * inv, a.z * inv); }
    return a;
}
__device__ __forceinline__ D3 normalized3(D3 a) {
    const double z = dot3(a, a);
    if (z > 0.0) { const double n = sqrt(z); return d3(a.x / n, a.y / n, a.z / n); }
    return a;
}

__device__ void eig3_jacobi(const double Ain[3][3], double ev[3], D3 &n0) {
    double a[3][3], V[3][3];
    double scale = 0.0;
#pragma unroll
    for (int i = 0; i < 3; i++)
#pragma unroll
        for (int j = 0; j < 3; j++) scale = fmax(scale, fabs(Ain[i][j]));
    if (!(scale > 0.0)) scale = 1.0;
#pragma unroll
    for (int i = 0; i < 3; i++)
#pragma unroll
        for (int j = 0; j < 3; j++) { a[i][j] = Ain[i][j] / scale; V[i][j] = (i == j) ? 1.0 : 0.0; }
    for (int sweep = 0; sweep < 32; sweep++) {
        const double off = a[0][1] * a[0][1] + a[0][2] * a[0][2] + a[1][2] * a[1][2];
        if (off < 1e-40) break;
#pragma unroll
        for (int p = 0; p < 2; p++) {
#pragma unroll
            for (int q = p + 1; q < 3; q++) {
                const double apq = a[p][q];
                if (apq == 0.0) continue;
                const double theta = (a[q][q] - a[p][p]) / (2.0 * apq);
                double t = 1.0 / (fabs(theta) + sqrt(theta * theta + 1.0));
                if (theta < 0.0) t = -t;
                const double c = 1.0 / sqrt(t * t + 1.0);
                const double s = t * c;
                const int r = 3 - p - q;
                const double app = a[p][p], aqq = a[q][q];
                a[p][p] = app - t * apq;
                a[q][q] = aqq + t * apq;
                a[p][q] = a[q][p] = 0.0;
                const double arp = a[r][p], arq = a[r][q];
                a[r][p] = a[p][r] = c * arp - s * arq;
                a[r][q] = a[q][r] = s * arp + c * arq;
// ... 55 lines not shown
    const double e1 = 3.0 * q - e0 - e2;
    ev[0] = e0; ev[1] = e1; ev[2] = e2;
    const D3 r0 = d3(a00 - e0, a01, a02), r1 = d3(a01, a11 - e0, a12), r2 = d3(a02, a12, a22 - e0);
    const D3 x01 = d3(r0.y * r1.z - r0.z * r1.y, r0.z * r1.x - r0.x * r1.z, r0.x * r1.y - r0.y * r1.x);
    const D3 x02 = d3(r0.y * r2.z - r0.z * r2.y, r0.z * r2.x - r0.x * r2.z, r0.x * r2.y - r0.y * r2.x);
    const D3 x12 = d3(r1.y * r2.z - r1.z * r2.y, r1.z * r2.x - r1.x * r2.z, r1.x * r2.y - r1.y * r2.x);
    const double n01 = dot3(x01, x01), n02 = dot3(x02, x02), n12 = dot3(x12, x12);
    D3 best = x01;
    double nb = n01;
    if (n02 > nb) { best = x02; nb = n02; }
    if (n12 > nb) { best = x12; nb = n12; }
    if (!(nb > 0.0)) {
        const double q0 = dot3(r0, r0), q1 = dot3(r1, r1), q2 = dot3(r2, r2);
        D3 r = r0;
        double qr = q0;
        if (q1 > qr) { r = r1; qr = q1; }
        if (q2 > qr) { r = r2; qr = q2; }
        if (!(qr > 0.0)) { n0 = d3(1.0, 0.0, 0.0); return; }
        const double ax = fabs(r.x), ay = fabs(r.y), az = fabs(r.z);
        D3 c;
        if (ax <= ay && ax <= az) c = d3(0.0, r.z, -r.y);
        else if (ay <= az) c = d3(-r.z, 0.0, r.x);
        else c = d3(r.y, -r.x, 0.0);
        const double ic = rcp_nr(sqrt(dot3(c, c)));
        n0 = d3(c.x * ic, c.y * ic, c.z * ic);
        return;
    }
    const double inv = rcp_nr(sqrt(nb));
    n0 = d3(best.x * inv, best.y * inv, best.z * inv);
}

struct LdsLayout {
    int nb_row;
    int off_nb, off_pw, off_pimu, off_qf, off_kv, off_nfound, off_ncand, off_next, off_defer;
    int off_wave, wave_bytes, off_vox, off_scratch;
    int off_wpart, off_winfo, total;
    int off_pose;
};
__host__ __device__ inline LdsLayout lds_layout(int K, int nb_voxels, int kpw, int wpb, int armed = 0) {
    const int kpb = wpb * kpw;
    LdsLayout L;
    L.nb_row = ((kpb + 31) & ~31) + 17;
    auto up16 = [](int x) { return (x + 15) & ~15; };
    int o = 0;
    L.off_nb = o;      o += up16(3 * K * L.nb_row * 4);
    L.off_pw = o;      o += up16(kpb * 3 * 8);
    L.off_pimu = o;    o += up16(kpb * 3 * 8);
    L.off_qf = o;      o += up16(kpb * 8 * 4);
    L.off_kv = o;      o += up16((kpb + 2) * 4 * 4);
    L.off_nfound = o;  o += up16(kpb * 4);
    L.off_ncand = o;   o += up16(kpb * 4);
    L.off_next = o;    o += 16;
    L.off_defer = o;   o += up16(kpb * 2);
    L.off_wave = o;
    int w = 0;
    L.off_vox = w;     w += (nb_voxels == 1 ? 64 : 128) * 8;
    L.off_scratch = w; w += SRL_WAVE_SCRATCH;
    L.wave_bytes = w;
    o += wpb * w;
    L.off_wpart = o;   o += wpb * 32 * 8;
    L.off_winfo = o;   o += wpb * 8 * 4;
    L.off_pose = o;
    if (armed) o += up16((SRL_POSE_DOUBLES + 2) * 8);
    L.total = o;
    return L;
}


#if defined(__HIP_DEVICE_COMPILE__)
typedef const __attribute__((address_space(4))) char *KargBytes;
#else
typedef const char *KargBytes;
#endif
#if defined(__HIP_DEVICE_COMPILE__)
__device__ __forceinline__ void store_granule_pair(unsigned long long *dst, unsigned tag, unsigned long long w) {
    typedef unsigned v4u __attribute__((ext_vector_type(4)));
    v4u v;
    v.x = (unsigned)w; v.y = tag; v.z = (unsigned)(w >> 32); v.w = tag;
    asm volatile("global_store_dwordx4 %0, %1, off sc0 sc1\n\ts_nop 1" :: "v"(dst), "v"(v) : "memory");
}
#else
__device__ inline void store_granule_pair(unsigned long long *, unsigned, unsigned long long) {}
#endif
// ... 81 lines not shown
    }
}

#if defined(__HIP_DEVICE_COMPILE__) && defined(SRL_ARM_STAMPS)
__device__ __forceinline__ void arm_stamp(KargBytes karg, int slot) {
#if !defined(SRL_STAMP_DETAIL)
    if (slot >= 16) return;
#endif
    typedef const __attribute__((address_space(4))) SrlAssocArgs *KP;
    KP q = (KP)karg;
    asm volatile("" : "+s"(q));
    long long *st = q->stamps;
    if (st != nullptr && threadIdx.x == 0) {
        const bool first = blockIdx.x == 0, last = blockIdx.x == gridDim.x - 1;
        if (slot >= 16) { if (last) __hip_atomic_store(st + ((q->seq & 63ull) * 32 + slot), (long long)wall_clock64(), __ATOMIC_RELAXED, __HIP_MEMORY_SCOPE_SYSTEM); return; }
        if (first) __hip_atomic_store(st + ((q->seq & 63ull) * 32 + slot), (long long)wall_clock64(), __ATOMIC_RELAXED, __HIP_MEMORY_SCOPE_SYSTEM);
        if (last) __hip_atomic_store(st + ((q->seq & 63ull) * 32 + 8 + slot), (long long)wall_clock64(), __ATOMIC_RELAXED, __HIP_MEMORY_SCOPE_SYSTEM);
    }
}
#else
__device__ inline void arm_stamp(KargBytes, int) {}
#endif

#ifndef SRL_P2_POLICY
#define SRL_P2_POLICY 1
#endif
#if SRL_P2_POLICY == 0
__host__ __device__ constexpr int p2_lanes_per_keypoint(int kpb) { return kpb >= 48 ? 1 : (kpb >= 32 ? 2 : 4); }
#else
__host__ __device__ constexpr int p2_lanes_per_keypoint(int kpb) { return kpb >= 192 ? 1 : (kpb >= 128 ? 2 : 4); }
#endif
__host__ __device__ constexpr int p2_keypoints_per_wave(int kpb) { return 64 / p2_lanes_per_keypoint(kpb); }

template <int NB, int FAST, int KPW, int WPB, int DBG = 0, int ARMED = 0>
__device__ __forceinline__ bool assoc_tile(KargBytes karg, const SrlAssocArgs &A, const int tile) {
    constexpr int KPB = WPB * KPW;
    extern __shared__ __attribute__((aligned(16))) unsigned char smem[];
    const int Kn = A.K;
    const int abl = DBG ? A.ablate : 0;
    constexpr bool POSE_LDS = ARMED != 0;
    const LdsLayout L = lds_layout(Kn, NB, KPW, WPB, ARMED);
    const int NB_ROW = L.nb_row;
    const int tid = threadIdx.x;
    const int lane = lane_id();
    const int wave = tid >> 6;
    float *s_nb = reinterpret_cast<float *>(smem + L.off_nb);
    const int nb_plane = Kn * NB_ROW;
    double *s_pw = reinterpret_cast<double *>(smem + L.off_pw);
    double *s_pimu = reinterpret_cast<double *>(smem + L.off_pimu);
    float *s_qf = reinterpret_cast<float *>(smem + L.off_qf);
    int *s_kv = reinterpret_cast<int *>(smem + L.off_kv);
    int *s_nfound = reinterpret_cast<int *>(smem + L.off_nfound);
    int *s_ncand = reinterpret_cast<int *>(smem + L.off_ncand);
    int *s_next = reinterpret_cast<int *>(smem + L.off_next);
    unsigned short *s_defer = reinterpret_cast<unsigned short *>(smem + L.off_defer);
    unsigned char *wbase = smem + L.off_wave + wave * L.wave_bytes;
    VoxEnt *vox = reinterpret_cast<VoxEnt *>(wbase + L.off_vox);
    Surv *surv = reinterpret_cast<Surv *>(wbase + L.off_scratch);
    double *s_wpart = reinterpret_cast<double *>(smem + L.off_wpart);
    int *s_winfo = reinterpret_cast<int *>(smem + L.off_winfo);

    const long long dbg_t0 = (DBG && (abl & 128)) ? (long long)wall_clock64() : 0;
#if defined(__HIP_DEVICE_COMPILE__)
    typedef const __attribute__((address_space(4))) SrlAssocArgs *KernargPtr;
#endif
    double *s_pose = reinterpret_cast<double *>(smem + L.off_pose);
    auto n_pass = [&]() -> int {
        if constexpr (ARMED) return __builtin_amdgcn_readfirstlane(reinterpret_cast<const int *>(s_pose + SRL_POSE_DOUBLES)[1]);
        else return A.n;
    };
    int n_fallback = 0;
#if defined(__HIP_DEVICE_COMPILE__)
    auto tile_stamp = [&](int slot) {
        if constexpr (ARMED) {
            arm_stamp(karg, slot - 8);
        }
    };
#else
    auto tile_stamp = [&](int) {};
#endif
    tile_stamp(10);
    bool use_bounds = A.bound_in != nullptr && A.bound_use > 0;
    if constexpr (ARMED) use_bounds = use_bounds && reinterpret_cast<const int *>(s_pose + SRL_POSE_DOUBLES)[2] == 0 && n_pass() == A.n;
    const int bbase_kp = tile * KPB;
    const int wbase_kp = bbase_kp + wave * KPW;

    if (tid < 4) s_next[tid] = 0;
    if (lane < KPW) {
        const int kq = wave * KPW + lane;
        const int g = wbase_kp + lane;
        D3 p_imu = d3(0, 0, 0), p_w = d3(0, 0, 0);
        if constexpr (ARMED) {
            if (g < n_pass()) {
                p_imu = d3(s_pimu[kq * 3 + 0], s_pimu[kq * 3 + 1], s_pimu[kq * 3 + 2]);
                p_w = add(matvec(s_pose, p_imu), d3(s_pose[18], s_pose[19], s_pose[20]));
            }
        } else {
            if (g < A.n) {
                D3 raw;
                if (A.aos != nullptr) {
                    const double *p = A.aos + 3 * (size_t)g;
                    raw = d3(p[0], p[1], p[2]);
                    const_cast<double *>(A.raw_x)[g] = raw.x; const_cast<double *>(A.raw_y)[g] = raw.y; const_cast<double *>(A.raw_z)[g] = raw.z;
                } else {
                    raw = d3(A.raw_x[g], A.raw_y[g], A.raw_z[g]);
                }
                p_imu = add(matvec(A.R_il, raw), d3(A.t_il[0], A.t_il[1], A.t_il[2]));
                p_w = add(matvec(A.Rn, p_imu), d3(A.t[0], A.t[1], A.t[2]));
            }
            s_pimu[kq * 3 + 0] = p_imu.x; s_pimu[kq * 3 + 1] = p_imu.y; s_pimu[kq * 3 + 2] = p_imu.z;
        }
        s_pw[kq * 3 + 0] = p_w.x; s_pw[kq * 3 + 1] = p_w.y; s_pw[kq * 3 + 2] = p_w.z;
        const bool unit = A.size_voxel == 1.0;
        const int kv[3] = {(int)(short)(int)(unit ? p_w.x : p_w.x / A.size_voxel), (int)(short)(int)(unit ? p_w.y : p_w.y / A.size_voxel),
                           (int)(short)(int)(unit ? p_w.z : p_w.z / A.size_voxel)};
        {
// ... 1 lines not shown
            const float u = 5.9604645e-8f;
            const float am = fmaxf(fmaxf(fabsf(qxf), fabsf(qyf)), fabsf(qzf)) * u + 1e-30f;
            const float h = 4.0f * am * 0.5001f;
            const float m0 = h * (1.0f + 1e-6f) + 8.0f * u * 1e-6f + 4.0f * am * am;
            const float m1 = 2.0f * h + 16.0f * u;
            float *qf = s_qf + kq * 8;
            qf[0] = qxf; qf[1] = qyf; qf[2] = qzf;
            qf[3] = (2.0f * m0) * 1.00001f;
            qf[4] = (1.0f + 2.0f * m1) * 1.00001f;
            float r2 = __builtin_huge_valf();
            if (use_bounds && g < A.bound_use) {
                const float4 bp = reinterpret_cast<const float4 *>(A.bound_in)[g];
                const float ex = qxf - bp.x, ey = qyf - bp.y, ez = qzf - bp.z;
                const float mag = fmaxf(fabsf(qxf) + fabsf(qyf) + fabsf(qzf), fabsf(bp.x) + fabsf(bp.y) + fabsf(bp.z));
                const float slack = 1e-3f + 1e-6f * mag;
                const float rt = sqrtf(bp.w) * 1.000001f;
                const float sz = (float)A.size_voxel;
                const float bq[3] = {bp.x, bp.y, bp.z};
                bool inside = true;
#pragma unroll
                for (int ax = 0; ax < 3; ++ax) {
                    const int vlo = kv[ax] - NB, vhi = kv[ax] + NB;
                    const float lo = (float)(vlo > 0 ? vlo : vlo - 1) * sz, hi = (float)(vhi < 0 ? vhi : vhi + 1) * sz;
                    inside = inside && (bq[ax] - rt) - slack >= lo && (bq[ax] + rt) + slack <= hi;
                }
                if (inside) {
                    const float r = rt + sqrtf(ex * ex + ey * ey + ez * ez) * 1.000001f + slack;
                    r2 = (r * r) * 1.00001f;
                }
            }
            qf[5] = r2;
            *reinterpret_cast<double *>(qf + 6) = __builtin_huge_val();
        }
        s_kv[kq * 4 + 0] = kv[0];
        s_kv[kq * 4 + 1] = kv[1];
        s_kv[kq * 4 + 2] = kv[2];
        s_nfound[kq] = 0;
        s_ncand[kq] = 0;
    } else if (wave == WPB - 1 && lane < KPW + 2) {
        const int kq = KPB + (lane - KPW);
        s_kv[kq * 4 + 0] = 0; s_kv[kq * 4 + 1] = 0; s_kv[kq * 4 + 2] = 0;
    }
    __syncthreads();
    tile_stamp(11);

    {
        const int left = n_pass() - bbase_kp;
        const int n_here = __builtin_amdgcn_readfirstlane(left < KPB ? left : KPB);
        auto make_sink = [&](int kl) {
            LdsSink sink;
            sink.col = s_nb + kl;
            sink.row = NB_ROW;
            sink.plane = nb_plane;
            sink.tap_ids = A.tap_ids ? (A.tap_ids + (size_t)(bbase_kp + kl) * Kn) : nullptr;
            return sink;
        };
        auto keypoint_general = [&](int kl, bool tie) {
            const double qx = s_pw[kl * 3 + 0], qy = s_pw[kl * 3 + 1], qz = s_pw[kl * 3 + 2];
            LdsSink sink = make_sink(kl);
            int total = 0, fb = 0;
            const int nv = probe_voxels<NB>(qx, qy, qz, A.size_voxel, A.thr_cap, A.table, A.table_mask, vox, lane);
            select_topk(qx, qy, qz, nv, vox, A.slabs, Kn, tie ? 5 : A.select_mode, surv, lane, sink, total, fb);
            n_fallback += (NB == 1) ? 1 : fb;
            if (lane == 0) {
                s_nfound[kl] = total < Kn ? total : Kn;
                s_ncand[kl] = total;
            }
        };
        if constexpr (NB == 1 && FAST != 0) {
            const LaneRole role = lane_role(lane);
            const int npairs = n_here > 0 ? (n_here + 1) >> 1 : 0;
            auto take = [&]() { int p = 0; if (lane == 0) p = atomicAdd(s_next, 1); return __builtin_amdgcn_readfirstlane(p); };
            int cur = take();
            ProbeReq preq;
            if (!(abl & 32)) preq = probe_issue(s_kv, 2 * (cur < npairs ? cur : npairs), role, A.table, A.table_mask, lane);
            while (cur < npairs) {
                const int nxt = take();
                const int nv_pair = __builtin_amdgcn_readfirstlane((abl & 8) ? 0 : probe_finish(preq, A.thr_cap, A.table, A.table_mask, vox, lane, s_ncand + 2 * cur, use_bounds, s_qf + 16 * cur,
                                                                                                               s_kv + 8 * cur, &role, (float)A.size_voxel));
                if (!(abl & 32)) preq = probe_issue(s_kv, 2 * (nxt < npairs ? nxt : npairs), role, A.table, A.table_mask, lane);
                auto file = [&](int kl, int done, int total) {
                    (void)total;
                    if (done == SEL_DONE) {
                    } else {
                        s_defer[atomicAdd(s_next + 1, 1)] = (unsigned short)(kl | (done == SEL_TIE ? 0x8000 : 0));
                    }
                };
                const int r_a = (int)((((unsigned)nv_pair & 0xFFu) + 2u) * 0x5556u >> 16), r_b = (int)(((((unsigned)nv_pair >> 8) & 0xFFu) + 2u) * 0x5556u >> 16);
                const int r_max = r_a > r_b ? r_a : r_b;
                if (2 * cur + 1 < n_here && r_max <= SRL_PAIR_MAX_ROUNDS && !(abl & (4 | 256))) {
                    const int kl = 2 * cur;
                    LdsSink sink_a = make_sink(kl), sink_b = make_sink(kl + 1);
                    int total_a = 0, total_b = 0, done;
                    if (r_max <= 2) done = select_pair_f32_r<2>(s_pw + kl * 3, s_pw + kl * 3 + 3, s_qf + kl * 8, s_qf + kl * 8 + 8, vox, A.slabs, A.inf_off, Kn, surv, lane, role, sink_a, sink_b, total_a, total_b, abl);
                    else if (r_max <= 3) done = select_pair_f32_r<3>(s_pw + kl * 3, s_pw + kl * 3 + 3, s_qf + kl * 8, s_qf + kl * 8 + 8, vox, A.slabs, A.inf_off, Kn, surv, lane, role, sink_a, sink_b, total_a, total_b, abl);
                    else done = select_pair_f32_r<4>(s_pw + kl * 3, s_pw + kl * 3 + 3, s_qf + kl * 8, s_qf + kl * 8 + 8, vox, A.slabs, A.inf_off, Kn, surv, lane, role, sink_a, sink_b, total_a, total_b, abl);
                    (void)total_a; (void)total_b;
                    if (done != (SEL_DONE | (SEL_DONE << 8))) {
                        if (lane == 0) {
                            if ((done & 0xFF) != SEL_DONE) s_defer[atomicAdd(s_next + 1, 1)] = (unsigned short)(kl | ((done & 0xFF) == SEL_TIE ? 0x8000 : 0));
                            if ((done >> 8) != SEL_DONE) s_defer[atomicAdd(s_next + 1, 1)] = (unsigned short)((kl + 1) | ((done >> 8) == SEL_TIE ? 0x8000 : 0));
                        }
                    }
                } else {
#pragma nounroll
                    for (int h = 0; h < 2; ++h) {
                        const int kl = 2 * cur + h;
                        if (kl >= n_here) break;
                        const int nv_fast = h ? (nv_pair >> 8) : (nv_pair & 0xFF);
                        const double qx = s_pw[kl * 3 + 0], qy = s_pw[kl * 3 + 1], qz = s_pw[kl * 3 + 2];
                        LdsSink sink = make_sink(kl);
                        int total = nv_fast;
                        int done = SEL_DONE;
                        if (!(abl & 4)) done = select_topk_f32(qx, qy, qz, s_qf + kl * 8, nv_fast, vox + 32 * h, A.slabs, A.inf_off, Kn, surv, lane, role, sink, total, abl);
                        if (lane == 0) file(kl, done, total);
                    }
                }
                cur = nxt;
            }
        } else if constexpr (NB == 2 && FAST != 0) {
            const LaneRole role = lane_role(lane);
            auto take = [&]() { int p = 0; if (lane == 0) p = atomicAdd(s_next, 1); return __builtin_amdgcn_readfirstlane(p); };
            for (int kl = take(); kl < n_here; kl = take()) {
                const double qx = s_pw[kl * 3 + 0], qy = s_pw[kl * 3 + 1], qz = s_pw[kl * 3 + 2];
                int total_all = 0;
                const int nv = probe_voxels<NB>(qx, qy, qz, A.size_voxel, A.thr_cap, A.table, A.table_mask, vox, lane, use_bounds ? s_qf + kl * 8 : nullptr, &total_all);
                if (lane < 3) { VoxEnt z; z.slab = 0u; z.count = 0u; vox[nv + lane] = z; }
                __builtin_amdgcn_wave_barrier();
                LdsSink sink = make_sink(kl);
                int total = 0;
                const int done = select_topk_f32_loop(qx, qy, qz, s_qf + kl * 8, nv, vox, A.slabs, A.inf_off, Kn, surv, lane, role, sink, total);
                total = total_all;
                if (lane == 0) {
                    if (done == SEL_DONE) {
                        s_nfound[kl] = total < Kn ? total : Kn;
                        s_ncand[kl] = total;
                    } else {
                        s_defer[atomicAdd(s_next + 1, 1)] = (unsigned short)(kl | (done == SEL_TIE ? 0x8000 : 0));
                    }
                }
            }
        } else {
            for (int kl = wave * KPW; kl < (wave + 1) * KPW && kl < n_here; ++kl) keypoint_general(kl, false);
        }
        if constexpr (FAST != 0) {
            __syncthreads();
            const int n_defer = __builtin_amdgcn_readfirstlane(s_next[1]);
            if (n_defer > 0) {
                auto take2 = [&]() { int p = 0; if (lane == 0) p = atomicAdd(s_next + 2, 1); return __builtin_amdgcn_readfirstlane(p); };
                for (int i = take2(); i < n_defer; i = take2()) {
                    const int e = __builtin_amdgcn_readfirstlane((int)s_defer[i]);
                    keypoint_general(e & 0x7FFF, (e & 0x8000) != 0);
                }
            }
        }
    }
    __syncthreads();
    tile_stamp(12);

    if (abl & 64) return true;
#if defined(__HIP_DEVICE_COMPILE__)
    KernargPtr bp = (KernargPtr)karg;
    asm volatile("" : "+s"(bp));
    const __attribute__((address_space(4))) SrlAssocArgs &b = *bp;
#else
    const SrlAssocArgs &b = A;
#endif
    constexpr int LPK = p2_lanes_per_keypoint(KPB);
// ... 81 lines not shown
        for (int i = 0; i < 9; ++i) Rm[i] = POSE_LDS ? s_pose[9 + i] : b.R[i];
#pragma unroll
        for (int i = 0; i < 3; ++i) tv[i] = POSE_LDS ? s_pose[18 + i] : b.t[i];
        const D3 pe = add(matvec(Rm, p_imu), d3(tv[0], tv[1], tv[2]));
        dist = dot3(nv, pe) + off;
        status = 1;
        if (b.tap_normal && sl == 0) {
            b.tap_normal[(size_t)g * 3 + 0] = nv.x; b.tap_normal[(size_t)g * 3 + 1] = nv.y; b.tap_normal[(size_t)g * 3 + 2] = nv.z;
            b.tap_a2d[g] = a2D;
            b.tap_offset[g] = off;
        }
        if (dist < b.max_dist && !nan_bad) {
            status = 2;
            J[0] = nv.x * weight; J[1] = nv.y * weight; J[2] = nv.z * weight;
            const double m0 = -nv.x, m1 = -nv.y, m2 = -nv.z;
            const double r0 = (m0 * Rm[0] + m1 * Rm[3]) + m2 * Rm[6];
            const double r1 = (m0 * Rm[1] + m1 * Rm[4]) + m2 * Rm[7];
            const double r2 = (m0 * Rm[2] + m1 * Rm[5]) + m2 * Rm[8];
            const double s0 = (r0 * 0.0 + r1 * p_imu.z) + r2 * (-p_imu.y);
            const double s1 = (r0 * (-p_imu.z) + r1 * 0.0) + r2 * p_imu.x;
            const double s2 = (r0 * p_imu.y + r1 * (-p_imu.x)) + r2 * 0.0;
            J[3] = s0 * weight; J[4] = s1 * weight; J[5] = s2 * weight;
        }
    }
    if constexpr (ARMED) arm_stamp(karg, 23);
    if (g < n2 && sl == 0 && b.bound_out != nullptr) {
        const float *qf = reinterpret_cast<const float *>(smem + L.off_qf) + kl * 8;
        const double tau = *reinterpret_cast<const double *>(qf + 6);
        float4 bo;
        bo.x = qf[0]; bo.y = qf[1]; bo.z = qf[2];
        bo.w = (float)tau * 1.0000002f;
        reinterpret_cast<float4 *>(b.bound_out)[g] = bo;
    }
    if (g < n2 && b.write_rec && sl == 0) {
        double2 *r = reinterpret_cast<double2 *>(b.rec + (size_t)g * 8);
        double2 v;
        v.x = J[0]; v.y = J[1]; r[0] = v;
        v.x = J[2]; v.y = J[3]; r[1] = v;
        v.x = J[4]; v.y = J[5]; r[2] = v;
        v.x = dist; v.y = weight; r[3] = v;
        b.status[g] = (unsigned char)status;
        if (b.tap_ncand) b.tap_ncand[g] = s_ncand[kl];
    }

    if (b.rec_granules != nullptr && owner_lane && sl == 0) {
        typedef __attribute__((address_space(1))) unsigned long long gu64r;
        const bool accd = status == 2;
        const double rec8[8] = {J[0], J[1], J[2], J[3], J[4], J[5], dist, weight};
        const unsigned long long tag = (unsigned long long)(unsigned)b.seq << 32;
        gu64r *dst = (gu64r *)(b.rec_granules + ((size_t)blockIdx.x * KPB + kl) * 16);
#pragma unroll
        for (int d = 0; d < 8; ++d) {
            const unsigned long long bits = accd ? (unsigned long long)__double_as_longlong(rec8[d]) : 0ull;
            __hip_atomic_store(dst + 2 * d, tag | (bits & 0xFFFFFFFFull), __ATOMIC_RELAXED, __HIP_MEMORY_SCOPE_AGENT);
            __hip_atomic_store(dst + 2 * d + 1, tag | (bits >> 32), __ATOMIC_RELAXED, __HIP_MEMORY_SCOPE_AGENT);
        }
    }

    if (p2_wave) {
        static_assert(P2W * KP2 * 64 <= WPB * (64 * 8 + SRL_WAVE_SCRATCH), "phase-2 rows must fit in the phase-1 per-wave regions");
        double *s_row = reinterpret_cast<double *>(smem + L.off_wave) + w2 * (KP2 * 8);
        const bool accd = status == 2;
        if (sl == 0 && klw < KP2) {
            const double h = dist * weight;
            double4 v;
            v.x = accd ? J[0] : 0.0; v.y = accd ? J[1] : 0.0; v.z = accd ? J[2] : 0.0; v.w = accd ? J[3] : 0.0;
// ... 33 lines not shown
        const unsigned long long nan_mask = __ballot(nan_bad);
        const unsigned long long pln_mask = __ballot((status == 1 || status == 2) && sl == 0);
        int pk = (g < n2 && sl == 0) ? s_ncand[kl] : 0;
#pragma unroll
        for (int off = 32; off >= 1; off >>= 1) pk += __shfl_xor(pk, off);
        if (lane == 0) {
            s_winfo[wave * 8 + 3] = n_fallback;
            if (p2_wave) {
                s_winfo[w2 * 8 + 0] = __popcll(acc_mask);
                s_winfo[w2 * 8 + 1] = pk;
                s_winfo[w2 * 8 + 2] = nan_mask ? 1 + w2 * KP2 + (int)__builtin_ctzll(nan_mask) / LPK : 0;
                s_winfo[w2 * 8 + 4] = __popcll(pln_mask);
                const unsigned long long km = per_keypoint(acc_mask);
                s_winfo[w2 * 8 + 5] = (int)(unsigned)km;
                s_winfo[w2 * 8 + 6] = (int)(unsigned)(km >> 32);
            }
        }
    }
    __syncthreads();
    tile_stamp(13);

    if (DBG && (b.ablate & 128) && (tid == 28 || tid == 29 || tid == 30))
        b.partials[(size_t)blockIdx.x * SRL_PART_STRIDE + tid] =
            (tid == 28) ? (double)dbg_t0 : ((tid == 29) ? (double)(long long)wall_clock64() : (double)__builtin_amdgcn_s_getreg(6164) );
    if (tid < SRL_ROW_SUMS && b.granules == nullptr) {
        double v = s_wpart[tid];
#pragma unroll
        for (int w = 1; w < P2W; ++w) v += s_wpart[w * 32 + tid];
        b.partials[(size_t)blockIdx.x * SRL_PART_STRIDE + tid] = v;
    }
    if (tid == 0) {
        SrlBlockInfo bi;
        bi.accepted = 0; bi.sum_pk = 0; bi.nan_first = 0; bi.num_fallback = 0; bi.planes = 0;
        bi.pad[0] = bi.pad[1] = bi.pad[2] = 0;
        for (int w = 0; w < WPB; ++w) bi.num_fallback += s_winfo[w * 8 + 3];
        for (int w = 0; w < P2W; ++w) {
            bi.accepted += s_winfo[w * 8 + 0]; bi.sum_pk += (unsigned)s_winfo[w * 8 + 1];
            if (bi.nan_first == 0) bi.nan_first = s_winfo[w * 8 + 2];
            bi.planes += s_winfo[w * 8 + 4];
        }
        b.binfo[blockIdx.x] = bi;
    }
    return b.granules == nullptr;
}

template <class Take>
__device__ __forceinline__ bool peer_exchange(const SrlPeerTable *pt, unsigned epoch, int slot, int lane, int nwords,
                                              unsigned long long mine, Take take) {
    typedef __attribute__((address_space(1))) unsigned long long gu64;
    const int G = pt->nranks, me = pt->rank;
    const bool act = lane < nwords;
    const unsigned long long tag = (unsigned long long)epoch << 32;
    const size_t slot_off = (size_t)slot * SRL_MAX_PEERS * (2 * SRL_PEER_ROW);
    if (act) {
        const unsigned long long lo = tag | (unsigned)mine, hi = tag | (unsigned)(mine >> 32);
        for (int r = 0; r < G; ++r) {
            unsigned long long *dst = pt->inbox[r] + slot_off + (size_t)me * (2 * SRL_PEER_ROW);
            __hip_atomic_store((gu64 *)(dst + lane), lo, __ATOMIC_RELAXED, __HIP_MEMORY_SCOPE_SYSTEM);
            __hip_atomic_store((gu64 *)(dst + SRL_PEER_ROW + lane), hi, __ATOMIC_RELAXED, __HIP_MEMORY_SCOPE_SYSTEM);
        }
    }
    bool ok = true;
    const unsigned long long *own = pt->inbox[me] + slot_off;
    for (int r = 0; r < G; ++r) {
        if (act) {
            const unsigned long long *src = own + (size_t)r * (2 * SRL_PEER_ROW);
            unsigned long long x0, x1;
// ... 203 lines not shown
                    else if (tid == 47) v = s_part[SRL_ROW_FALLBACK];
                    else if (tid == 48) v = (double)n_total;
                    else if (tid == 49) v = *s_bad ? 1.0 : 0.0;
                    double sum = 0.0;
                    const bool ok = peer_exchange(b.peer, b.peer_epoch, b.peer_slot, lane, SRL_REDUCED_DOUBLES, (unsigned long long)__double_as_longlong(v),
                                                  [&](int, unsigned long long w) { sum += __longlong_as_double((long long)w); });
                    double *od = reinterpret_cast<double *>(out);
                    if (tid < SRL_REDUCED_DOUBLES) od[tid] = sum;
                    else if (tid == SRL_REDUCED_DOUBLES) out->last_visited = (long long)n_total - 1;
                    else if (tid == SRL_REDUCED_DOUBLES + 1) out->pad = ok ? 0ll : SRL_PEER_TIMEOUT_MARK;
                }
            }
        }
        if (!peer_done) {
            SrlOutTail t;
            t.num_res = s_part[SRL_ROW_ACCEPTED];
            t.total_accepted = s_part[SRL_ROW_ACCEPTED];
            t.sum_pk = s_part[SRL_ROW_SUM_PK];
            t.nan = s_part[SRL_ROW_NAN] > 0.0 ? 1.0 : 0.0;
            t.fallback = s_part[SRL_ROW_FALLBACK];
            t.visited = (double)n_total;
            t.timeout = *s_bad ? 1.0 : 0.0;
            t.last_visited = (long long)n_total - 1;
            t.pad = *s_bad ? SRL_ROW_TIMEOUT_MARK : 0ll;
            write_dev_out(out, tid, s_part, t, put);
        }
        arm_stamp(karg, 19);
        mail_out(out);
        arm_stamp(karg, 20);
    }
#endif
}

template <int NB, int FAST, int KPW, int WPB, int DBG = 0, int ARMED = 0>
__device__ __forceinline__ void assoc_body(const SrlAssocArgs &a) {
    constexpr int KPB = WPB * KPW;
    extern __shared__ __attribute__((aligned(16))) unsigned char smem[];
    const int tid = threadIdx.x;
    if (a.ablate & 16) return;
#if defined(__HIP_DEVICE_COMPILE__)
    typedef const __attribute__((address_space(4))) SrlAssocArgs *KernargPtr;
#endif
    auto carve = [&]() -> LdsLayout { return lds_layout(a.K, NB, KPW, WPB, ARMED); };
    if constexpr (ARMED) {
#if defined(__HIP_DEVICE_COMPILE__)
        typedef __attribute__((address_space(1))) unsigned long long gu64a;
        const LdsLayout L = carve();
        double *s_pose = reinterpret_cast<double *>(smem + L.off_pose);
        int *s_ctrl = reinterpret_cast<int *>(s_pose + SRL_POSE_DOUBLES);
        arm_stamp((KargBytes)__builtin_amdgcn_kernarg_segment_ptr(), 0);
        {
            const int lane0 = tid & 63, wave0 = tid >> 6;
            if (lane0 < KPW) {
                const int kq = wave0 * KPW + lane0;
                const int g = (int)blockIdx.x * KPB + kq;
                double *s_pimu = reinterpret_cast<double *>(smem + L.off_pimu);
                D3 p_imu = d3(0, 0, 0);
                if (g < a.n) p_imu = add(matvec(a.R_il, d3(a.raw_x[g], a.raw_y[g], a.raw_z[g])), d3(a.t_il[0], a.t_il[1], a.t_il[2]));
                s_pimu[kq * 3 + 0] = p_imu.x; s_pimu[kq * 3 + 1] = p_imu.y; s_pimu[kq * 3 + 2] = p_imu.z;
            }
        }
        if (tid < 64) {
            const int lane = tid;
            const unsigned epoch = a.pose_epoch;
            const bool relayed = a.pose_relayed != 0;
            const bool leader = !relayed || blockIdx.x == 0;
            const bool act = lane < SRL_POSE_BOX_USED;
// ... 45 lines not shown
                            if (alt) {
                                typedef const __attribute__((address_space(1))) double gf64c;
                                gf64c *p = (gf64c *)(a.alt_aos + 3 * (size_t)g);
                                raw = d3(__hip_atomic_load(p, __ATOMIC_RELAXED, __HIP_MEMORY_SCOPE_SYSTEM),
                                         __hip_atomic_load(p + 1, __ATOMIC_RELAXED, __HIP_MEMORY_SCOPE_SYSTEM),
                                         __hip_atomic_load(p + 2, __ATOMIC_RELAXED, __HIP_MEMORY_SCOPE_SYSTEM));
                                const_cast<double *>(a.alt_x)[g] = raw.x; const_cast<double *>(a.alt_y)[g] = raw.y; const_cast<double *>(a.alt_z)[g] = raw.z;
                            } else {
                                raw = d3(a.raw_x[g], a.raw_y[g], a.raw_z[g]);
                            }
                            p_imu = add(matvec(a.R_il, raw), d3(a.t_il[0], a.t_il[1], a.t_il[2]));
                        }
                        s_pimu[kq * 3 + 0] = p_imu.x; s_pimu[kq * 3 + 1] = p_imu.y; s_pimu[kq * 3 + 2] = p_imu.z;
                    }
                }
            }
            if (code != (int)SRL_ARM_GO) {
                if (code == (int)SRL_ARM_EXPIRED && blockIdx.x == gridDim.x - 1 && tid == 0) {
                    __hip_atomic_store(&a.mailbox->expired, a.seq, __ATOMIC_RELAXED, __HIP_MEMORY_SCOPE_SYSTEM);
                }
                if (code == (int)SRL_ARM_EXPIRED && blockIdx.x == gridDim.x - 1 && tid < 64 && !a.mail_tagged && a.peer == nullptr) {
                    constexpr int NW = (int)(sizeof(SrlDevOut) / 8);
                    unsigned long long w = 0ull;
                    if (tid == (int)(offsetof(SrlDevOut, d_timeout) / 8)) w = (unsigned long long)__double_as_longlong(1.0);
                    if (tid == (int)(offsetof(SrlDevOut, pad) / 8)) w = (unsigned long long)SRL_ROW_TIMEOUT_MARK;
                    if (tid == (int)(offsetof(SrlDevOut, last_visited) / 8)) w = ~0ull;
                    if (tid < NW) __hip_atomic_store(reinterpret_cast<unsigned long long *>(&a.mailbox->out) + tid, w, __ATOMIC_RELAXED, __HIP_MEMORY_SCOPE_SYSTEM);
                }
                return;
            }
        }
#endif
    }
    if (assoc_tile<NB, FAST, KPW, WPB, DBG, ARMED>((KargBytes)__builtin_amdgcn_kernarg_segment_ptr(), a, (int)blockIdx.x)) return;
    double row_v = 0.0;
    constexpr int P2W_T = (KPB + p2_keypoints_per_wave(KPB) - 1) / p2_keypoints_per_wave(KPB);
    if (tid < 32) {
        const LdsLayout L = carve();
        const double *s_wpart = reinterpret_cast<const double *>(smem + L.off_wpart);
        const int *s_winfo = reinterpret_cast<const int *>(smem + L.off_winfo);
        double v = 0.0;
        if (tid < SRL_ROW_SUMS) {
            v = s_wpart[tid];
#pragma unroll
            for (int w = 1; w < P2W_T; ++w) v += s_wpart[w * 32 + tid];
        } else {
            int acc = 0, pk = 0, nanf = 0, fb = 0;
            for (int w = 0; w < WPB; ++w) fb += s_winfo[w * 8 + 3];
            for (int w = 0; w < P2W_T; ++w) { acc += s_winfo[w * 8 + 0]; pk += s_winfo[w * 8 + 1]; if (nanf == 0) nanf = s_winfo[w * 8 + 2]; }
            v = tid == SRL_ROW_ACCEPTED ? (double)acc : (tid == SRL_ROW_SUM_PK ? (double)(unsigned)pk : (tid == SRL_ROW_NAN ? (double)nanf : (double)fb));
        }
        row_v = v;
    }
#if defined(__HIP_DEVICE_COMPILE__)
    KernargPtr bq = (KernargPtr)__builtin_amdgcn_kernarg_segment_ptr();
    asm volatile("" : "+s"(bq));
    const __attribute__((address_space(4))) SrlAssocArgs &b = *bq;
#else
    const SrlAssocArgs &b = a;
#endif
    const LdsLayout L = lds_layout(b.K, NB, KPW, WPB, ARMED);
    const int *s_winfo = reinterpret_cast<const int *>(smem + L.off_winfo);

    typedef __attribute__((address_space(1))) unsigned long long gu64;
    const unsigned epoch = (unsigned)b.seq;
    constexpr int KP2 = p2_keypoints_per_wave(KPB);
    constexpr int P2W = (KPB + KP2 - 1) / KP2;
    const bool finishes = blockIdx.x == gridDim.x - 1 ||
                          (b.cut_max == 0 && (int)gridDim.x > 2 * SRL_FUSED_GROUP && ((int)blockIdx.x % SRL_FUSED_GROUP) == SRL_FUSED_GROUP - 1);
    if (tid < 32) {
#if defined(__HIP_DEVICE_COMPILE__)
        if (finishes) reinterpret_cast<double *>(smem + SRL_OWN_ROW_OFFSET)[tid] = row_v;
        else row_store(rows_rsrc(b.granules), (int)blockIdx.x, tid, epoch, row_v);
#endif
    } else if (tid >= 64 && tid < 72 && b.cut_max > 0) {
        const int j = tid - 64;
        unsigned word = 0u;
        if (KP2 >= 32) {
            const int w = (32 * j) / KP2;
            if (w < P2W) word = (unsigned)s_winfo[w * 8 + 5 + (((32 * j) % KP2) >> 5)];
        } else {
#pragma unroll
            for (int t = 0; t < 32 / KP2; ++t) {
                const int w = (32 * j) / KP2 + t;
                if (w < P2W) word |= (unsigned)s_winfo[w * 8 + 5] << (t * KP2);
            }
        }
        __hip_atomic_store((gu64 *)(b.granules + (size_t)blockIdx.x * SRL_ROW_GRANULES + tid), ((unsigned long long)epoch << 32) | word,
                           __ATOMIC_RELAXED, __HIP_MEMORY_SCOPE_AGENT);
    }
    if constexpr (ARMED) arm_stamp((KargBytes)__builtin_amdgcn_kernarg_segment_ptr(), 6);
    if (!finishes) return;
    int n_total = b.n;
    if constexpr (ARMED) n_total = __builtin_amdgcn_readfirstlane(reinterpret_cast<const int *>(smem + L.off_pose + SRL_POSE_DOUBLES * 8)[1]);
    finish_rows<KPW, WPB>((KargBytes)__builtin_amdgcn_kernarg_segment_ptr(), epoch, n_total);
    if constexpr (ARMED) arm_stamp((KargBytes)__builtin_amdgcn_kernarg_segment_ptr(), 7);
}

template <int NB, int FAST, int KPW, int WPB, int DBG = 0>
__global__ void __launch_bounds__(64 * WPB, WPB == 16 ? 1 : SRL_ASSOC_WAVES_PER_SIMD) srl_assoc_kernel(const SrlAssocArgs a) {
    assoc_body<NB, FAST, KPW, WPB, DBG>(a);
}
template <int NB, int KPW>
__global__ void __launch_bounds__(1024, 1) srl_assoc_armed_kernel(const SrlAssocArgs a) {
    assoc_body<NB, 1, KPW, 16, 0, 1>(a);
}
__global__ void __launch_bounds__(1024) srl_reduce_kernel(const SrlReduceArgs a, int mode_in) {
    __shared__ long long s_wtot[16];
    __shared__ double s_rec[256 * 8];
    __shared__ unsigned char s_stat[256];
    __shared__ int s_wcnt[4];
    __shared__ int s_first;
    __shared__ double s_part[32][SRL_PART_STRIDE];
    __shared__ long long s_tot[4];
    __shared__ int s_cut[4];
    __shared__ int s_nan_min;
    const int tid = threadIdx.x;
    const int nb = a.nblocks;

    int mode = mode_in;
    long long max_res = a.max_res;
    if (a.gather) {
        long long prior = 0;
        for (int r = 0; r < a.rank; ++r) prior += a.gather[r];
        if (a.max_num_residuals > 0) {
            max_res = (long long)a.max_num_residuals - prior;
            mode = max_res <= 0 ? 2 : 0;
        } else {
            mode = prior > 0 ? 2 : 1;
        }
    }

    long long acc = 0, pk = 0, fb = 0;
    int nan_min = 0x7fffffff;
    const int per = (nb + 1023) / 1024;
    const int b0 = tid * per;
    const int b1 = (b0 + per < nb) ? b0 + per : nb;
    for (int b = b0; b < b1; ++b) {
// ... 198 lines not shown
}

}

hipError_t srl_launch_sqrt(double *io, int n, hipStream_t s) {
    if (n <= 0) return hipSuccess;
    hipLaunchKernelGGL(srl_sqrt_kernel, dim3((n + 255) / 256), dim3(256), 0, s, io, n);
    return hipGetLastError();
}

template <int KPW, int WPB>
static hipError_t launch_assoc_cfg(const SrlAssocArgs &a, int nb_voxels, hipStream_t s) {
    const int nblocks = (a.n + WPB * KPW - 1) / (WPB * KPW);
    const bool armed = a.pose_box != nullptr;
    const LdsLayout L = lds_layout(a.K, nb_voxels, KPW, WPB, armed ? 1 : 0);
    const dim3 blk(64 * WPB);
    auto launch = [&](auto kern) {
        if (L.total > 64 * 1024) {
            static thread_local const void *done_fn = nullptr;
            static thread_local int done_bytes = 0, done_dev = -1;
            int dev = -1;
            hipGetDevice(&dev);
            const void *fn = reinterpret_cast<const void *>(kern);
            if (fn != done_fn || L.total > done_bytes || dev != done_dev) {
                hipError_t e = hipFuncSetAttribute(fn, hipFuncAttributeMaxDynamicSharedMemorySize, SRL_LDS_LIMIT);
                if (e != hipSuccess) return e;
                done_fn = fn; done_bytes = SRL_LDS_LIMIT; done_dev = dev;
            }
        }
        hipLaunchKernelGGL(kern, dim3(nblocks), blk, L.total, s, a);
        return hipGetLastError();
    };
    const bool fast = a.select_mode == 0 || a.select_mode == 4;
    if (armed) {
        if constexpr (WPB == 16) { if (fast && a.ablate == 0) return nb_voxels == 1 ? launch(srl_assoc_armed_kernel<1, KPW>) : launch(srl_assoc_armed_kernel<2, KPW>); }
        return hipErrorInvalidConfiguration;
    }
    if constexpr (KPW == 16 && WPB == 16) { if (a.ablate != 0 && nb_voxels == 1 && fast) return launch(srl_assoc_kernel<1, 1, 16, 16, 1>); }
    if (nb_voxels == 1) return fast ? launch(srl_assoc_kernel<1, 1, KPW, WPB>) : launch(srl_assoc_kernel<1, 0, KPW, WPB>);
    return fast ? launch(srl_assoc_kernel<2, 1, KPW, WPB>) : launch(srl_assoc_kernel<2, 0, KPW, WPB>);
}
hipError_t srl_launch_assoc(const SrlAssocArgs &a, int nb_voxels, int kpw, int wpb, hipStream_t s) {
    if (a.n <= 0) return hipSuccess;
    if (wpb == 16) {
        if (kpw == 2) return launch_assoc_cfg<2, 16>(a, nb_voxels, s);
        if (kpw == 3) return launch_assoc_cfg<3, 16>(a, nb_voxels, s);
        if (kpw == 4) return launch_assoc_cfg<4, 16>(a, nb_voxels, s);
        if (kpw == 6) return launch_assoc_cfg<6, 16>(a, nb_voxels, s);
        if (kpw == 8) return launch_assoc_cfg<8, 16>(a, nb_voxels, s);
        if (kpw == 12) return launch_assoc_cfg<12, 16>(a, nb_voxels, s);
        return launch_assoc_cfg<16, 16>(a, nb_voxels, s);
    }
    if (kpw != 4 && kpw != 8 && kpw != 16) return hipErrorInvalidConfiguration;
    if (kpw == 4) return launch_assoc_cfg<4, 4>(a, nb_voxels, s);
    if (kpw == 8) return launch_assoc_cfg<8, 4>(a, nb_voxels, s);
    return launch_assoc_cfg<16, 4>(a, nb_voxels, s);
}
int srl_assoc_lds_bytes(int K, int nb_voxels, int kpw, int wpb) { return lds_layout(K, nb_voxels, kpw, wpb).total; }

hipError_t srl_launch_reduce(const SrlReduceArgs &a, int mode, hipStream_t s) {
    hipLaunchKernelGGL(srl_reduce_kernel, dim3(1), dim3(1024), 0, s, a, mode);
    return hipGetLastError();
}

__global__ void __launch_bounds__(64) srl_publish_kernel(const SrlDevOut *src, SrlMailbox *mb, unsigned long long seq) {
    const int tid = threadIdx.x;
    constexpr int NW = (int)(sizeof(SrlDevOut) / 8);
    const unsigned long long *s = reinterpret_cast<const unsigned long long *>(src);
    unsigned long long *d = reinterpret_cast<unsigned long long *>(&mb->out);
    if (tid < NW) __hip_atomic_store(d + tid, s[tid], __ATOMIC_RELAXED, __HIP_MEMORY_SCOPE_SYSTEM);
    asm volatile("s_waitcnt vmcnt(0)" ::: "memory");
// ... 69 lines not shown
```

sr_livo_amd/csrc/srl_map_kernels.hip:

```cpp
#include "srl_ctx.h"
#include "srl_frame_scratch.h"
#include "srl_hash.h"


#include <cstring>
#include <vector>

namespace {


template <bool XF>
__global__ void k_point_slots(const double *xyz, int n, double voxel_size, unsigned long long *keyw, unsigned mask, unsigned epoch16, unsigned *slot_out,
                              unsigned *idx, int *new_flag, const SrlFrameTransform T) {
    const int i = blockIdx.x * blockDim.x + threadIdx.x;
    if (i >= n) return;
    double wx, wy, wz;
    if (XF) {
        srl_transform_point(T.X, T.raw[(size_t)i * 3], T.raw[(size_t)i * 3 + 1], T.raw[(size_t)i * 3 + 2], wx, wy, wz);
        T.world[(size_t)i * 3] = wx; T.world[(size_t)i * 3 + 1] = wy; T.world[(size_t)i * 3 + 2] = wz;
    } else {
        wx = xyz[(size_t)i * 3]; wy = xyz[(size_t)i * 3 + 1]; wz = xyz[(size_t)i * 3 + 2];
    }
    const float fx = (float)wx, fy = (float)wy, fz = (float)wz;
    const short kx = (short)(int)((double)fx / voxel_size);
// ... 302 lines not shown
    HIPCHK(ctx, b_rank.alloc(ctx, (size_t)V * 4));
    HIPCHK(ctx, b_cnt.alloc(ctx, 64));
    HIPCHK(ctx, b_sc.alloc(ctx, srl_scan_scratch_ints(V) * 4));
    unsigned long long *d_removed = b_cnt.as<unsigned long long>();
    int *d_surv = b_cnt.as<int>() + 2;
    HIPCHK(ctx, hipMemsetAsync(b_cnt.p, 0, 16, st));
    hipLaunchKernelGGL(k_prune_mark, dim3(std::min((V + 1023) / 1024, SRL_PRUNE_MARK_BLOCKS)), dim3(1024), 0, st, ctx->d_slabs, V, location[0], location[1],
                       location[2], distance * distance, b_keep.as<int>(), d_removed);
    HIPCHK(ctx, hipGetLastError());
    srl_scan(SrlIntArrayIn{b_keep.as<int>()}, PruneRankSink{b_rank.as<int>(), d_surv, V}, V, b_sc.as<int>(), st);
    HIPCHK(ctx, hipGetLastError());
    { const int rc = ensure_host_scratch(ctx, 64); if (rc) return rc; }
    HIPCHK(ctx, hipMemcpyAsync(ctx->h_scratch, b_cnt.p, 16, hipMemcpyDeviceToHost, st));
    HIPCHK(ctx, hipStreamSynchronize(st));
    long long pts_removed = 0;
    int V_new = 0;
    std::memcpy(&pts_removed, ctx->h_scratch, 8);
    std::memcpy(&V_new, ctx->h_scratch + 8, 4);
    if (V_new == V) return SRL_OK;
    if (V_new > 0) {
        DevBuf b_dst;
        HIPCHK(ctx, b_dst.alloc(ctx, (size_t)V_new * SRL_SLAB_BYTES));
        hipLaunchKernelGGL(k_prune_compact, dim3((V + 15) / 16), dim3(256), 0, st, ctx->d_slabs, V, b_keep.as<int>(), b_rank.as<int>(), b_dst.as<unsigned char>());
        HIPCHK(ctx, hipGetLastError());
        HIPCHK(ctx, hipMemcpyAsync(ctx->d_slabs, b_dst.p, (size_t)V_new * SRL_SLAB_BYTES, hipMemcpyDeviceToDevice, st));
    }
    HIPCHK(ctx, hipMemsetAsync(ctx->d_slabs + (size_t)V_new * SRL_SLAB_BYTES, 0, (size_t)(V - V_new) * SRL_SLAB_BYTES, st));
    hipLaunchKernelGGL(k_fill_empty, dim3((ctx->table_cap + 255) / 256), dim3(256), 0, st, ctx->d_table, ctx->table_cap);
    if (V_new > 0)
        hipLaunchKernelGGL(k_rebuild_table, dim3((V_new + 255) / 256), dim3(256), 0, st, ctx->d_slabs, V_new, ctx->d_table, ctx->table_cap - 1);
    HIPCHK(ctx, hipGetLastError());
    ctx->num_voxels = V_new;
    ctx->num_points -= pts_removed;
    ctx->bound_n = 0;
    ctx->taps_valid = false;
    if (num_voxels_removed) *num_voxels_removed = V - V_new;
    if (num_points_removed) *num_points_removed = pts_removed;
    return SRL_OK;
}

extern "C" int srl_map_probe_checksum(srl_ctx *ctx, const double *world_xyz, int n, int stride, double voxel_size, uint64_t *checksum) {
    if (!ctx || !checksum || !(voxel_size > 0.0) || (world_xyz && n < 0) || stride < 1) return SRL_ERR_BAD_ARG;
    SRL_DISARM(ctx);
    *checksum = 0;
    if (!ctx->d_table) return SRL_ERR_NO_MAP;
    HIPCHK(ctx, hipSetDevice(ctx->device));
    { const int rcs = srl_map_settle(ctx); if (rcs) return rcs; }
    const double *d_pts = nullptr;
    DevBuf b_pts, b_sum;
    if (world_xyz) {
        if (n == 0) return SRL_OK;
        HIPCHK(ctx, b_pts.alloc(ctx, (size_t)n * 3 * sizeof(double)));
        HIPCHK(ctx, hipMemcpyAsync(b_pts.p, world_xyz, (size_t)n * 3 * sizeof(double), hipMemcpyHostToDevice, ctx->stream));
        d_pts = b_pts.as<double>();
    } else {
        if (ctx->frame_world_n <= 0 || !ctx->d_frame_world) return SRL_OK;
        n = ctx->frame_world_n;
        d_pts = ctx->d_frame_world;
    }
    HIPCHK(ctx, b_sum.alloc(ctx, 256));
    HIPCHK(ctx, hipMemsetAsync(b_sum.p, 0, 8, ctx->stream));
    const int probes = (n + stride - 1) / stride;
    hipLaunchKernelGGL(k_probe_checksum, dim3((probes + 255) / 256), dim3(256), 0, ctx->stream, d_pts, n, stride, voxel_size, ctx->d_table, ctx->table_cap - 1,
                       ctx->d_slabs, b_sum.as<unsigned long long>());
    HIPCHK(ctx, hipGetLastError());
    unsigned long long out = 0ull;
    HIPCHK(ctx, hipMemcpyAsync(&out, b_sum.p, 8, hipMemcpyDeviceToHost, ctx->stream));
// ... 49 lines not shown
    HIPCHK(ctx, b_in.alloc(ctx, (size_t)n * 4)); HIPCHK(ctx, b_k.alloc(ctx, (size_t)n * 4)); HIPCHK(ctx, b_v.alloc(ctx, (size_t)n * 4));
    HIPCHK(ctx, b_tk.alloc(ctx, (size_t)n * 4)); HIPCHK(ctx, b_tv.alloc(ctx, (size_t)n * 4));
    DevBuf b_sc;
    HIPCHK(ctx, b_sc.alloc(ctx, srl_radix_scratch_ints(n) * 4));
    HIPCHK(ctx, hipMemcpyAsync(b_in.p, keys, (size_t)n * 4, hipMemcpyHostToDevice, ctx->stream));
    srl_radix_sort_pairs(b_in.as<unsigned>(), nullptr, b_k.as<unsigned>(), b_v.as<unsigned>(), b_tk.as<unsigned>(), b_tv.as<unsigned>(), n, (unsigned)bits, ctx->stream,
                         b_sc.as<int>());
    HIPCHK(ctx, hipGetLastError());
    HIPCHK(ctx, hipMemcpyAsync(keys_sorted, b_k.p, (size_t)n * 4, hipMemcpyDeviceToHost, ctx->stream));
    HIPCHK(ctx, hipMemcpyAsync(positions_sorted, b_v.p, (size_t)n * 4, hipMemcpyDeviceToHost, ctx->stream));
    HIPCHK(ctx, hipStreamSynchronize(ctx->stream));
    return SRL_OK;
}

int srl_map_insert_device(srl_ctx *ctx, const double *world_xyz, int n, double voxel_size, int cap,
                          double min_distance_points, int min_num_points, int *num_added) {
    (void)cap;
    return srl_map_insert_impl(ctx, world_xyz, false, n, voxel_size, min_distance_points, min_num_points, num_added, false);
}
int srl_map_insert_report_device(srl_ctx *ctx, const double *world_xyz, int n, double voxel_size, int cap, double min_distance_points, int min_num_points,
                                 double ref_z, uint8_t *outcome, srl_cloud_point *cloud, int *num_cloud, int *num_added) {
    (void)cap;
    const SrlInsertReport rep = {ref_z, outcome, cloud, num_cloud};
    return srl_map_insert_impl(ctx, world_xyz, false, n, voxel_size, min_distance_points, min_num_points, num_added, false, nullptr, nullptr, nullptr, &rep);
}

int srl_map_insert_impl(srl_ctx *ctx, const double *world_xyz, bool on_device, int n, double voxel_size,
                        double min_distance_points, int min_num_points, int *num_added, bool defer_counters,
                        const SrlFrameTransform *xf, int (*after_first_kernel)(srl_ctx *, void *), void *user, const SrlInsertReport *report) {
    if (num_added) *num_added = 0;
    if (report && report->num_cloud) *report->num_cloud = 0;
    if (n == 0) return SRL_OK;
    if (!(voxel_size > 0.0)) return SRL_ERR_BAD_ARG;
    ctx->bound_n = 0;
    HIPCHK(ctx, hipSetDevice(ctx->device));
    hipStream_t st = ctx->stream;
    { const int rcs = srl_map_settle(ctx); if (rcs) return rcs; }
    if (!ctx->h_insert_cnt) {
        HIPCHK(ctx, hipHostMalloc((void **)&ctx->h_insert_cnt, 64, hipHostMallocDefault));
        HIPCHK(ctx, hipEventCreateWithFlags(&ctx->ev_insert, hipEventDisableTiming));
    }
    if (!ctx->d_table) {
        ctx->slab_cap = 0; ctx->table_cap = 0; ctx->num_voxels = 0; ctx->num_points = 0;
        int rc = srl_ctx_grow_map(ctx, 4096u, 8192u);
        if (rc) return rc;
    }
    const bool frame_sized = n <= SRL_SCAN_MAX;
    if (frame_sized) {
        const unsigned need_slabs = (unsigned)ctx->num_voxels + (unsigned)n;
        if (need_slabs > ctx->slab_cap || SRL_TABLE_FACTOR * need_slabs > ctx->table_cap) {
            int rc = srl_ctx_grow_map(ctx, need_slabs, SRL_TABLE_FACTOR * need_slabs);
            if (rc) return rc;
        }
    }

    DevBuf b_xyz, b_keys2, b_idx, b_idx2, b_prefix, b_start, b_cnt, b_slot, b_isnew, b_first, b_newflag, b_outcome, b_cloud;
    const double *d_xyz = world_xyz;
    if (!on_device) {
        HIPCHK(ctx, b_xyz.alloc(ctx, (size_t)n * 3 * sizeof(double)));
        HIPCHK(ctx, hipMemcpyAsync(b_xyz.p, world_xyz, (size_t)n * 3 * sizeof(double), hipMemcpyHostToDevice, st));
        d_xyz = b_xyz.as<double>();
    }
    HIPCHK(ctx, b_keys2.alloc(ctx, (size_t)n * 8));
    HIPCHK(ctx, b_idx.alloc(ctx, (size_t)n * 4));
    HIPCHK(ctx, b_idx2.alloc(ctx, (size_t)n * 4));
    HIPCHK(ctx, b_prefix.alloc(ctx, (size_t)n * 4));
    HIPCHK(ctx, b_start.alloc(ctx, (size_t)n * 4));
// ... 111 lines not shown
```

Before: 10740 sweeps/s.

## Cache per-keypoint candidate shortlists across ESIKF passes for KNN reuse

The first association pass of a sweep now records, for each keypoint, a shortlist of up to 64 candidate point slots inside a widened radius, along with a safety margin derived from the K-th neighbour distance. Later passes in the same solve use a list-reading kernel variant that searches only the shortlist when the pose change keeps the query inside that margin. This cuts repeated voxel-slab gathers and bisection work during the nearest-neighbour search. In exchange it adds list-writing cost and extra memory traffic on the first pass, more kernel template variants, and invalidation bookkeeping wherever the map or sweep changes.

```diff
diff --git a/include/srlivo_hip_debug.h b/include/srlivo_hip_debug.h
--- a/include/srlivo_hip_debug.h
+++ b/include/srlivo_hip_debug.h
@@ -21,6 +21,8 @@
 int srl_debug_set_ablate(srl_ctx *ctx, int bits);
 int srl_debug_set_fused_reduce(srl_ctx *ctx, int enable);
 int srl_debug_set_bound_culling(srl_ctx *ctx, int enable);
+int srl_debug_set_shortlists(srl_ctx *ctx, int enable);
+int srl_debug_shortlist_served(srl_ctx *ctx, long long *served);
 int srl_debug_set_pose_box(srl_ctx *ctx, int kind);
 int srl_debug_set_arm_linger(srl_ctx *ctx, double host_linger_us, double kernel_linger_us);
 int srl_debug_pass_stamps(srl_ctx *ctx, int enable, long long *gpu_out, long long *host_out);
diff --git a/sr_livo_amd/capi.py b/sr_livo_amd/capi.py
--- a/sr_livo_amd/capi.py
+++ b/sr_livo_amd/capi.py
@@ -240,6 +240,8 @@
         "srl_debug_set_ablate": ([p, C.c_int], C.c_int),
         "srl_debug_set_fused_reduce": ([p, C.c_int], C.c_int),
         "srl_debug_set_bound_culling": ([p, C.c_int], C.c_int),
+        "srl_debug_set_shortlists": ([p, C.c_int], C.c_int),
+        "srl_debug_shortlist_served": ([p, C.POINTER(C.c_longlong)], C.c_int),
         "srl_debug_set_pose_box": ([p, C.c_int], C.c_int),
         "srl_debug_set_arm_linger": ([p, C.c_double, C.c_double], C.c_int),
         "srl_debug_pass_stamps": ([p, C.c_int, p, p], C.c_int),
@@ -769,6 +771,14 @@
     def set_bound_culling(self, on):
         self._chk(self.lib.srl_debug_set_bound_culling(self.h, 1 if on else 0), "srl_debug_set_bound_culling")
 
+    def set_shortlists(self, on):
+        self._chk(self.lib.srl_debug_set_shortlists(self.h, 1 if on else 0), "srl_debug_set_shortlists")
+
+    def shortlist_served(self):
+        v = C.c_longlong(0)
+        self._chk(self.lib.srl_debug_shortlist_served(self.h, C.byref(v)), "srl_debug_shortlist_served")
+        return int(v.value)
+
     def set_search_select_mode(self, mode):
         self._chk(self.lib.srl_debug_set_search_select_mode(self.h, int(mode)), "srl_debug_set_search_select_mode")
 
diff --git a/sr_livo_amd/csrc/srl_capi.cpp b/sr_livo_amd/csrc/srl_capi.cpp
--- a/sr_livo_amd/csrc/srl_capi.cpp
+++ b/sr_livo_amd/csrc/srl_capi.cpp
@@ -36,6 +36,22 @@
 std::atomic<int> g_live_ctx[SRL_MAX_DEVICES];
 inline int live_contexts(int device) { return (device >= 0 && device < SRL_MAX_DEVICES) ? g_live_ctx[device].load(std::memory_order_relaxed) : 1; }
 
+bool ensure_lists(srl_ctx *ctx) {
+    if (ctx->d_lists && ctx->list_cap >= ctx->work_cap) return true;
+    if (ctx->d_lists) { (void)hipFree(ctx->d_lists); ctx->d_lists = nullptr; }
+    ctx->list_cap = 0; ctx->list_n = 0;
+    const size_t bytes = (size_t)ctx->work_cap * (32 + 4 * (size_t)SRL_LIST_CAP);
+    if (ctx->work_cap <= 0 || hipMalloc((void **)&ctx->d_lists, bytes) != hipSuccess) {
+        (void)hipGetLastError();
+        ctx->d_lists = nullptr;
+        if (ctx->work_cap > 0) ctx->list_mode = -1;
+        return false;
+    }
+    ctx->list_cap = ctx->work_cap;
+    return true;
+}
+inline bool pass_writes_lists(const SrlAssocArgs &a) { return a.lists != nullptr && a.list_use == 0 && !(a.bound_in != nullptr && a.bound_use > 0); }
+
 int ensure_work(srl_ctx *ctx, int n) {
     if (n <= ctx->work_cap) return SRL_OK;
     const int cap = std::max(n, 1024);
@@ -44,7 +60,7 @@
     if ((rc = ensure(ctx, ctx->d_rec, (size_t)cap * 8))) return rc;
     if ((rc = ensure(ctx, ctx->d_status, (size_t)cap))) return rc;
     if ((rc = ensure(ctx, ctx->d_bound, (size_t)cap * 4))) return rc;
-    ctx->bound_n = 0;
+    ctx->void_neighbourhoods();
     if ((rc = ensure(ctx, ctx->d_partials, (size_t)nblocks * SRL_PART_STRIDE))) return rc;
     if ((rc = ensure(ctx, ctx->d_binfo, (size_t)nblocks))) return rc;
     ctx->work_cap = cap;
@@ -177,7 +193,7 @@
     if (ctx->d_sub_kept) hipFree(ctx->d_sub_kept);
     if (ctx->d_sub_seen) hipFree(ctx->d_sub_seen);
     void *bufs[] = {ctx->d_corr_in, ctx->d_corr_rel, ctx->d_corr_imu, ctx->d_corr_raw, ctx->d_corr_seg, ctx->d_frame_raw, ctx->d_frame_world, ctx->d_table, ctx->d_slabs, ctx->d_raw, ctx->d_rec, ctx->d_status, ctx->d_partials, ctx->d_binfo,
-                    ctx->d_out, ctx->d_count, ctx->d_bound, ctx->d_granules, ctx->d_rec_granules, ctx->d_raw_next, ctx->d_stage_next, ctx->d_stage_cur, ctx->d_tap_ids, ctx->d_tap_ncand, ctx->d_tap_normal, ctx->d_tap_a2d,
+                    ctx->d_out, ctx->d_count, ctx->d_bound, ctx->d_lists, ctx->d_granules, ctx->d_rec_granules, ctx->d_raw_next, ctx->d_stage_next, ctx->d_stage_cur, ctx->d_tap_ids, ctx->d_tap_ncand, ctx->d_tap_normal, ctx->d_tap_a2d,
                     ctx->d_tap_offset, ctx->d_gather, ctx->d_peer, ctx->d_mail};
     for (int r = 0; r < SRL_MAX_PEERS; r++) if (ctx->peer_mapped[r]) hipIpcCloseMemHandle(ctx->peer_mapped[r]);
     if (ctx->d_inbox) hipFree(ctx->d_inbox);
@@ -217,7 +233,7 @@
     if (cap != SRL_VOXEL_CAP) { ctx->err = "max_num_points_in_voxel must be 20"; return SRL_ERR_UNSUPPORTED; }
     HIPCHK(ctx, hipSetDevice(ctx->device));
     { const int rcs = srl_map_settle(ctx); if (rcs) return rcs; }
-    ctx->bound_n = 0;
+    ctx->void_neighbourhoods();
     const unsigned slab_cap = std::max<unsigned>(1024u, (unsigned)V + (unsigned)V / 2u + 4096u);
     if (slab_cap > SRL_MAX_SLABS) { ctx->err = "map too large: slab byte offsets are 32-bit (16.7 M voxels)"; return SRL_ERR_UNSUPPORTED; }
     const unsigned table_cap = next_pow2(std::max<unsigned>(2048u, SRL_TABLE_FACTOR * slab_cap));
@@ -362,7 +378,7 @@
     ctx->taps_valid = false;
     ctx->passes_in_solve = 0;
     ctx->tail_pending = false;
-    ctx->bound_n = 0;
+    ctx->void_neighbourhoods();
     if (cnt > ctx->sweep_cap) {
         const int cap = std::max(cnt, 1024);
         int rc = ensure(ctx, ctx->d_raw, (size_t)cap * 3);
@@ -460,7 +476,7 @@
         up = hipSuccess;
     }
     ctx->tail_pending = up != hipSuccess;
-    ctx->bound_n = 0;
+    ctx->void_neighbourhoods();
     ctx->cur_slot = ctx->next_slot;
     ctx->cur_prefix_n = up == hipSuccess ? ctx->next_n : ctx->next_prefix_n;
     ctx->passes_in_solve = 0;
@@ -907,10 +923,14 @@
         float sv = (float)o->size_voxel_map;
         int sv_bits; std::memcpy(&sv_bits, &sv, 4);
         const int sig[4] = {p.K, p.nb, p.thr, sv_bits};
-        if (std::memcmp(sig, ctx->bound_sig, sizeof sig) != 0) { ctx->bound_n = 0; std::memcpy(ctx->bound_sig, sig, sizeof sig); }
+        if (std::memcmp(sig, ctx->bound_sig, sizeof sig) != 0) { ctx->void_neighbourhoods(); std::memcpy(ctx->bound_sig, sig, sizeof sig); }
         a.bound_out = ctx->d_bound;
         a.bound_in = ctx->bound_mode != 0 ? ctx->d_bound : nullptr;
         a.bound_use = a.bound_in ? std::min(ctx->bound_n, n_eff) : 0;
+        const bool lists = ctx->list_mode > 0 && p.nb == 1 && (ctx->select_mode == 0 || ctx->select_mode == 4) && ensure_lists(ctx);
+        a.lists = lists ? ctx->d_lists : nullptr;
+        a.list_cap = lists ? ctx->list_cap : 0;
+        a.list_use = lists ? std::min(ctx->list_n, n_eff) : 0;
     }
     if (p.fused) {
         a.granules = ctx->d_granules;
@@ -970,6 +990,7 @@
     sg.pose_box = nullptr; sg.pose_relay = nullptr; sg.pose_relayed = 0; sg.pose_epoch = 0; sg.arm_linger_ticks = 0;
     sg.raw_x = sg.raw_y = sg.raw_z = nullptr; sg.alt_x = sg.alt_y = sg.alt_z = nullptr; sg.n = 0; sg.aos = nullptr; sg.alt_aos = nullptr;
     sg.bound_use = 0;
+    sg.list_use = 0;
     return sg;
 }
 
@@ -995,6 +1016,7 @@
         ctx->arm_stats[1]++;
         ctx->cur_measured = ctx->armed_measured;
         ctx->cur_gen = ctx->armed_gen;
+        ctx->fired_list_use = ctx->armed_list_use;
         fired = true;
         return SRL_OK;
     }
@@ -1054,6 +1076,9 @@
     SrlAssocArgs nx = a;
     nx.seq = ctx->seq + 1;
     nx.bound_use = a.bound_in ? a.n : 0;
+    const bool next_sweep = ctx->next_n >= 0 && ctx->expected_passes > 0 && ctx->passes_in_solve + 1 >= ctx->expected_passes;
+    nx.list_use = (!a.lists || next_sweep) ? 0 : (pass_writes_lists(a) ? a.n : a.list_use);
+    ctx->armed_list_use = nx.list_use;
     const bool has_alt = ctx->d_raw_next != nullptr && ctx->next_cap > 0 && ctx->d_stage_next != nullptr;
     nx.aos = nullptr;
     nx.alt_aos = has_alt ? ctx->d_stage_next : nullptr;
@@ -1233,6 +1258,7 @@
     out->num_fallback = (int32_t)(r.d_fallback + 0.5);
 
     if (a.aos != nullptr && n_eff > ctx->soa_valid_n) ctx->soa_valid_n = n_eff;
+    if (pass_writes_lists(a) && !(fired && ctx->fired_list_use > 0)) ctx->list_n = n_eff;
     ctx->bound_n = n_eff;
     ctx->last_K = p.K;
     ctx->last_nb = p.nb;
@@ -1453,6 +1479,26 @@
     SRL_DISARM(ctx);
     ctx->bound_mode = enable ? 1 : 0;
     ctx->bound_n = 0;
+    return SRL_OK;
+}
+int srl_debug_set_shortlists(srl_ctx *ctx, int enable) {
+    if (!ctx) return SRL_ERR_BAD_ARG;
+    SRL_DISARM(ctx);
+    if (ctx->list_mode >= 0) ctx->list_mode = enable ? 1 : 0;
+    ctx->void_neighbourhoods();
+    return SRL_OK;
+}
+int srl_debug_shortlist_served(srl_ctx *ctx, long long *served) {
+    if (!ctx || !served) return SRL_ERR_BAD_ARG;
+    SRL_DISARM(ctx);
+    HIPCHK(ctx, hipSetDevice(ctx->device));
+    *served = 0;
+    const int nb = ctx->last_nblocks;
+    if (nb <= 0 || !ctx->d_binfo) return SRL_OK;
+    std::vector<SrlBlockInfo> bi((size_t)nb);
+    HIPCHK(ctx, hipStreamSynchronize(ctx->stream));
+    HIPCHK(ctx, hipMemcpy(bi.data(), ctx->d_binfo, (size_t)nb * sizeof(SrlBlockInfo), hipMemcpyDeviceToHost));
+    for (const SrlBlockInfo &b : bi) *served += b.served;
     return SRL_OK;
 }
 int srl_debug_set_fused_reduce(srl_ctx *ctx, int enable) {
diff --git a/sr_livo_amd/csrc/srl_ctx.h b/sr_livo_amd/csrc/srl_ctx.h
--- a/sr_livo_amd/csrc/srl_ctx.h
+++ b/sr_livo_amd/csrc/srl_ctx.h
@@ -65,6 +65,11 @@
     int bound_n = 0;
     int bound_sig[4] = {0, 0, 0, 0};
     int bound_mode = 1;
+    unsigned char *d_lists = nullptr;
+    int list_cap = 0, list_n = 0;
+    int list_mode = 1;
+    int armed_list_use = 0, fired_list_use = 0;
+    void void_neighbourhoods() { bound_n = 0; list_n = 0; }
     bool tail_pending = false;
     int cur_slot = 0, cur_prefix_n = 0;
 
diff --git a/sr_livo_amd/csrc/srl_device.h b/sr_livo_amd/csrc/srl_device.h
--- a/sr_livo_amd/csrc/srl_device.h
+++ b/sr_livo_amd/csrc/srl_device.h
@@ -17,6 +17,8 @@
 #define SRL_SURV_CAP 64
 #define SRL_WAVE_SCRATCH 2048
 #define SRL_MAXK 32
+#define SRL_LIST_CAP 64
+#define SRL_LIST_WIDEN 0.40f
 #define SRL_EMPTY_KEY 0xFFFFFFFFFFFFFFFFull
 #define SRL_TABLE_FACTOR 4u
 #define SRL_PART_STRIDE 32
@@ -86,7 +88,8 @@
     int nan_first;
     int num_fallback;
     int planes;
-    int pad[3];
+    int served;
+    int pad[2];
 };
 static_assert(sizeof(SrlBlockInfo) == 32, "block info is 32 bytes");
 
@@ -185,7 +188,10 @@
     const float *bound_in;
     float *bound_out;
     int bound_use;
-    int pad_bound;
+    int list_use;
+    unsigned char *lists;
+    int list_cap;
+    int pad_list;
     double *rec;
     unsigned char *status;
     double *partials;
diff --git a/sr_livo_amd/csrc/srl_frame_kernels.hip b/sr_livo_amd/csrc/srl_frame_kernels.hip
--- a/sr_livo_amd/csrc/srl_frame_kernels.hip
+++ b/sr_livo_amd/csrc/srl_frame_kernels.hip
@@ -824,7 +824,7 @@
         srl_stage_end(ctx, 3);
     }
     if (num_keypoints) *num_keypoints = m;
-    ctx->total_n = m; ctx->shard_begin = 0; ctx->n = m; ctx->sweep_loaded = true; ctx->taps_valid = false; ctx->bound_n = 0; ctx->tail_pending = false;
+    ctx->total_n = m; ctx->shard_begin = 0; ctx->n = m; ctx->sweep_loaded = true; ctx->taps_valid = false; ctx->void_neighbourhoods(); ctx->tail_pending = false;
     ctx->soa_valid_n = m; ctx->passes_in_solve = 0;
     if (n > 0) { const int rcm = srl_mark_frame_read(ctx); if (rcm) return rcm; }
     srl_stage_end(ctx, 4);
diff --git a/sr_livo_amd/csrc/srl_kernels.hip b/sr_livo_amd/csrc/srl_kernels.hip
--- a/sr_livo_amd/csrc/srl_kernels.hip
+++ b/sr_livo_amd/csrc/srl_kernels.hip
@@ -385,7 +385,7 @@
     return dx * dx + dy * dy + dz * dz;
 }
 
-template <class Sink>
+template <class Sink, bool IDS = false>
 __device__ __forceinline__ int finish_survivors(double qx, double qy, double qz, int c, const VoxEnt *vox, int K, void *scratch,
                                                 int lane, Sink &sink, double *tau_out = nullptr) {
     SurvRec *recs = reinterpret_cast<SurvRec *>(__builtin_assume_aligned(scratch, 16));
@@ -434,8 +434,11 @@
     if (__ballot(bad)) return SEL_TIE;
     if (tau_out && act && rank == K - 1) *tau_out = my;
     if (win) {
-        const VoxEnt ve = vox[me.code >> 5];
-        sink.put(rank, me.x, me.y, me.z, ve.slab * SRL_CAP + ((unsigned)me.code & 31u));
+        if constexpr (IDS) sink.put(rank, me.x, me.y, me.z, (unsigned)me.code);
+        else {
+            const VoxEnt ve = vox[me.code >> 5];
+            sink.put(rank, me.x, me.y, me.z, ve.slab * SRL_CAP + ((unsigned)me.code & 31u));
+        }
     }
     __builtin_amdgcn_wave_barrier();
     return SEL_DONE;
@@ -501,10 +504,49 @@
     }
 }
 
+struct ListOut {
+    unsigned *ent;
+    unsigned *word;
+    float wmax;
+};
+__device__ __forceinline__ unsigned list_entry_id(unsigned off) {
+    return (off >> 8) * SRL_CAP + (((off & 255u) * 43u) >> 9);
+}
+template <int R>
+__device__ __forceinline__ unsigned list_write(const float (&d2f)[R], float thr, const float *qf, const VoxEnt *vox, const LaneRole &role, unsigned *ent,
+                                               float wmax) {
+    if (!(thr < 1e30f)) return 0u;
+    const float rt = sqrtf(thr);
+    float tw = 0.0f, w = wmax;
+    int n = SRL_LIST_CAP + 1;
+#pragma nounroll
+    for (int rung = 0; rung < 3 && n > SRL_LIST_CAP; ++rung) {
+        const float r = rt + w;
+        w *= 0.5f;
+        tw = r * r;
+        n = 0;
+#pragma unroll
+        for (int j = 0; j < R; ++j) n += __popcll(__ballot(d2f[j] <= tw));
+    }
+    if (n > SRL_LIST_CAP) return 0u;
+    const int cbase = role.c0 < 3 ? role.c0 : 0;
+    const unsigned slot_off = (unsigned)role.slot * 12u;
+    int base = 0;
+#pragma unroll
+    for (int j = 0; j < R; ++j) {
+        const unsigned long long m = __ballot(d2f[j] <= tw);
+        if (__builtin_amdgcn_inverse_ballot_w64(m)) ent[base + lanes_below(m)] = vox[3 * j + cbase].slab * (unsigned)SRL_SLAB_BYTES + slot_off;
+        base += __popcll(m);
+    }
+    const float rho2 = (2.0f - qf[4]) * tw - qf[3];
+    const float rho = rho2 > 0.0f ? sqrtf(rho2) * 0.9998f : 0.0f;
+    return (__float_as_uint(rho) & ~127u) | (unsigned)n;
+}
+
 template <int R, class Sink>
 __device__ __forceinline__ int cand_select(const float (&px)[R], const float (&py)[R], const float (&pz)[R], double qx, double qy, double qz,
                                            const float *qf, const VoxEnt *vox, int K, void *scratch, int lane, const LaneRole &role, Sink &sink,
-                                           int ablate) {
+                                           int ablate, const ListOut &lo_out) {
     float d2f[R];
     const unsigned v = __float_as_uint(cand_d2f<R>(px, py, pz, qf, d2f));
     unsigned lo = 0;
@@ -515,6 +557,10 @@
         lo = (cnt < K) ? trial : lo;
     }
     const float thr = thr_from_bisection(lo, qf);
+    if (lo_out.ent != nullptr) {
+        const unsigned w = list_write<R>(d2f, thr, qf, vox, role, lo_out.ent, lo_out.wmax);
+        if (lane == 0) *lo_out.word = w;
+    }
     SurvRec *recs = reinterpret_cast<SurvRec *>(__builtin_assume_aligned(scratch, 16));
     unsigned long long svm[R];
     int c = 0;
@@ -532,13 +578,14 @@
 template <int R, class Sink>
 __device__ __forceinline__ int select_topk_f32_r(double qx, double qy, double qz, const float *qf, int nv, const VoxEnt *vox,
                                                   const unsigned char *slabs, unsigned inf_off, int K, void *scratch, int lane,
-                                                  const LaneRole &role, Sink &sink, int &total_out, int ablate) {
+                                                  const LaneRole &role, Sink &sink, int &total_out, int ablate, const ListOut &lo_out) {
     (void)nv;
     float px[R], py[R], pz[R];
     cand_issue<R>(vox, slabs, inf_off, role, px, py, pz, total_out);
-    return cand_select<R>(px, py, pz, qx, qy, qz, qf, vox, K, scratch, lane, role, sink, ablate);
-}
-
+    return cand_select<R>(px, py, pz, qx, qy, qz, qf, vox, K, scratch, lane, role, sink, ablate, lo_out);
+}
+
+template <bool IDS = false>
 __device__ __forceinline__ int finish_pair(const double *qa, const double *qb, int ca, int cb, const VoxEnt *vox, int K, void *scratch, int lane,
                                            const LdsSink &sink_a, const LdsSink &sink_b, const float *qfa, const float *qfb) {
     SurvRec *recs = reinterpret_cast<SurvRec *>(__builtin_assume_aligned(scratch, 16));
@@ -578,26 +625,20 @@
     const unsigned long long bm = __ballot(bad);
     const bool tie_a = (unsigned)bm != 0u, tie_b = (unsigned)(bm >> 32) != 0u;
     if (win && !(h ? tie_b : tie_a)) {
-        const VoxEnt ve = vox[32 * h + (me.code >> 5)];
         LdsSink s = sink_a;
         if (h) { s.col = sink_b.col; s.tap_ids = sink_b.tap_ids; }
-        s.put(rank, me.x, me.y, me.z, ve.slab * SRL_CAP + ((unsigned)me.code & 31u));
+        if constexpr (IDS) s.put(rank, me.x, me.y, me.z, (unsigned)me.code);
+        else {
+            const VoxEnt ve = vox[32 * h + (me.code >> 5)];
+            s.put(rank, me.x, me.y, me.z, ve.slab * SRL_CAP + ((unsigned)me.code & 31u));
+        }
         if (rank == K - 1) *reinterpret_cast<double *>(const_cast<float *>(h ? qfb : qfa) + 6) = my;
     }
     __builtin_amdgcn_wave_barrier();
     return (tie_a ? SEL_TIE : SEL_DONE) | ((tie_b ? SEL_TIE : SEL_DONE) << 8);
 }
 
-template <int R>
-__device__ __forceinline__ int select_pair_f32_r(const double *qa, const double *qb, const float *qfa, const float *qfb, const VoxEnt *vox,
-                                                 const unsigned char *slabs, unsigned inf_off, int K, void *scratch, int lane,
-                                                 const LaneRole &role, LdsSink &sink_a, LdsSink &sink_b, int &total_a, int &total_b, int ablate) {
-    float ax[R], ay[R], az[R], bx[R], by[R], bz[R];
-    cand_issue<R>(vox, slabs, inf_off, role, ax, ay, az, total_a);
-    cand_issue<R>(vox + 32, slabs, inf_off, role, bx, by, bz, total_b);
-    float da[R], db[R];
-    const unsigned va = __float_as_uint(cand_d2f<R>(ax, ay, az, qfa, da));
-    const unsigned vb = __float_as_uint(cand_d2f<R>(bx, by, bz, qfb, db));
+__device__ __forceinline__ void pair_bisect(unsigned va, unsigned vb, int K, unsigned &lo_a_out, unsigned &lo_b_out) {
     constexpr unsigned BAND_LO = 0x38000000u, BAND_HI = 0x40000000u, BAND_LAST = 0x3FFC0000u;
     const unsigned ca_v = va < BAND_LO ? BAND_LO : (va > BAND_HI ? BAND_HI : va);
     const unsigned cb_v = vb < BAND_LO ? BAND_LO : (vb > BAND_HI ? BAND_HI : vb);
@@ -621,7 +662,28 @@
             lo_b = (cnt_b < K) ? tb : lo_b;
         }
     }
+    lo_a_out = lo_a; lo_b_out = lo_b;
+}
+
+template <int R>
+__device__ __forceinline__ int select_pair_f32_r(const double *qa, const double *qb, const float *qfa, const float *qfb, const VoxEnt *vox,
+                                                 const unsigned char *slabs, unsigned inf_off, int K, void *scratch, int lane,
+                                                 const LaneRole &role, LdsSink &sink_a, LdsSink &sink_b, int &total_a, int &total_b, int ablate,
+                                                 const ListOut &lo_out) {
+    float ax[R], ay[R], az[R], bx[R], by[R], bz[R];
+    cand_issue<R>(vox, slabs, inf_off, role, ax, ay, az, total_a);
+    cand_issue<R>(vox + 32, slabs, inf_off, role, bx, by, bz, total_b);
+    float da[R], db[R];
+    const unsigned va = __float_as_uint(cand_d2f<R>(ax, ay, az, qfa, da));
+    const unsigned vb = __float_as_uint(cand_d2f<R>(bx, by, bz, qfb, db));
+    unsigned lo_a, lo_b;
+    pair_bisect(va, vb, K, lo_a, lo_b);
     const float thr_a = thr_from_bisection(lo_a, qfa), thr_b = thr_from_bisection(lo_b, qfb);
+    if (lo_out.ent != nullptr) {
+        const unsigned wa = list_write<R>(da, thr_a, qfa, vox, role, lo_out.ent, lo_out.wmax);
+        const unsigned wb = list_write<R>(db, thr_b, qfb, vox + 32, role, lo_out.ent + SRL_LIST_CAP, lo_out.wmax);
+        if (lane == 0) { lo_out.word[0] = wa; lo_out.word[1] = wb; }
+    }
     unsigned long long sa[R], sb[R];
     int ca = 0, cb = 0;
 #pragma unroll
@@ -650,18 +712,59 @@
     return done_a | (done_b << 8);
 }
 
+__device__ __forceinline__ int select_pair_list(const double *qa, const double *qb, const float *qfa, const float *qfb, unsigned oa, unsigned ob, int na, int nb,
+                                                const unsigned char *slabs, unsigned inf_off, int K, void *scratch, int lane, LdsSink &sink_a, LdsSink &sink_b) {
+    if (lane >= na) oa = inf_off;
+    if (lane >= nb) ob = inf_off;
+    float ax[1], ay[1], az[1], bx[1], by[1], bz[1];
+    {
+        const float *pa = reinterpret_cast<const float *>(slabs + oa), *pb = reinterpret_cast<const float *>(slabs + ob);
+        ax[0] = pa[0]; ay[0] = pa[1]; az[0] = pa[2];
+        bx[0] = pb[0]; by[0] = pb[1]; bz[0] = pb[2];
+    }
+    float da[1], db[1];
+    const unsigned va = __float_as_uint(cand_d2f<1>(ax, ay, az, qfa, da));
+    const unsigned vb = __float_as_uint(cand_d2f<1>(bx, by, bz, qfb, db));
+    unsigned lo_a, lo_b;
+    pair_bisect(va, vb, K, lo_a, lo_b);
+    const float thr_a = thr_from_bisection(lo_a, qfa), thr_b = thr_from_bisection(lo_b, qfb);
+    const unsigned long long sa = __ballot(da[0] <= thr_a), sb = __ballot(db[0] <= thr_b);
+    const int ca = __popcll(sa), cb = __popcll(sb);
+    SurvRec *recs = reinterpret_cast<SurvRec *>(__builtin_assume_aligned(scratch, 16));
+    auto compact = [&](float x, float y, float z, unsigned off, unsigned long long m, SurvRec *dst) {
+        if (__builtin_amdgcn_inverse_ballot_w64(m)) {
+            SurvRec r; r.x = x; r.y = y; r.z = z; r.code = (int)list_entry_id(off);
+            dst[lanes_below(m)] = r;
+        }
+    };
+    if (ca <= 32 && cb <= 32 && K <= 31) {
+        compact(ax[0], ay[0], az[0], oa, sa, recs);
+        compact(bx[0], by[0], bz[0], ob, sb, recs + 32);
+        return finish_pair<true>(qa, qb, ca, cb, nullptr, K, scratch, lane, sink_a, sink_b, qfa, qfb);
+    }
+    compact(ax[0], ay[0], az[0], oa, sa, recs);
+    const int done_a = finish_survivors<LdsSink, true>(qa[0], qa[1], qa[2], ca, nullptr, K, scratch, lane, sink_a, reinterpret_cast<double *>(const_cast<float *>(qfa) + 6));
+    __builtin_amdgcn_wave_barrier();
+    int done_b = SEL_DONE;
+    if (nb > 0) {
+        compact(bx[0], by[0], bz[0], ob, sb, recs);
+        done_b = finish_survivors<LdsSink, true>(qb[0], qb[1], qb[2], cb, nullptr, K, scratch, lane, sink_b, reinterpret_cast<double *>(const_cast<float *>(qfb) + 6));
+    }
+    return done_a | (done_b << 8);
+}
+
 template <class Sink>
 __device__ __forceinline__ int select_topk_f32(double qx, double qy, double qz, const float *qf, int nv, const VoxEnt *vox,
                                                 const unsigned char *slabs, unsigned inf_off, int K, void *scratch, int lane,
-                                                const LaneRole &role, Sink &sink, int &total_out, int ablate) {
+                                                const LaneRole &role, Sink &sink, int &total_out, int ablate, const ListOut &lo_out) {
     switch ((nv + 2) / 3) {
         case 0: case 1: case 2: case 3:
-            return select_topk_f32_r<3>(qx, qy, qz, qf, nv, vox, slabs, inf_off, K, scratch, lane, role, sink, total_out, ablate);
-        case 4: return select_topk_f32_r<4>(qx, qy, qz, qf, nv, vox, slabs, inf_off, K, scratch, lane, role, sink, total_out, ablate);
-        case 5: return select_topk_f32_r<5>(qx, qy, qz, qf, nv, vox, slabs, inf_off, K, scratch, lane, role, sink, total_out, ablate);
-        case 6: return select_topk_f32_r<6>(qx, qy, qz, qf, nv, vox, slabs, inf_off, K, scratch, lane, role, sink, total_out, ablate);
-        case 7: return select_topk_f32_r<7>(qx, qy, qz, qf, nv, vox, slabs, inf_off, K, scratch, lane, role, sink, total_out, ablate);
-        default: return select_topk_f32_r<9>(qx, qy, qz, qf, nv, vox, slabs, inf_off, K, scratch, lane, role, sink, total_out, ablate);
+            return select_topk_f32_r<3>(qx, qy, qz, qf, nv, vox, slabs, inf_off, K, scratch, lane, role, sink, total_out, ablate, lo_out);
+        case 4: return select_topk_f32_r<4>(qx, qy, qz, qf, nv, vox, slabs, inf_off, K, scratch, lane, role, sink, total_out, ablate, lo_out);
+        case 5: return select_topk_f32_r<5>(qx, qy, qz, qf, nv, vox, slabs, inf_off, K, scratch, lane, role, sink, total_out, ablate, lo_out);
+        case 6: return select_topk_f32_r<6>(qx, qy, qz, qf, nv, vox, slabs, inf_off, K, scratch, lane, role, sink, total_out, ablate, lo_out);
+        case 7: return select_topk_f32_r<7>(qx, qy, qz, qf, nv, vox, slabs, inf_off, K, scratch, lane, role, sink, total_out, ablate, lo_out);
+        default: return select_topk_f32_r<9>(qx, qy, qz, qf, nv, vox, slabs, inf_off, K, scratch, lane, role, sink, total_out, ablate, lo_out);
     }
 }
 
@@ -758,7 +861,7 @@
     return a;
 }
 
-__device__ void eig3_jacobi(const double Ain[3][3], double ev[3], D3 &n0) {
+__device__ __forceinline__ void eig3_jacobi(const double Ain[3][3], double ev[3], D3 &n0) {
     double a[3][3], V[3][3];
     double scale = 0.0;
 #pragma unroll
@@ -880,7 +983,7 @@
 
 struct LdsLayout {
     int nb_row;
-    int off_nb, off_pw, off_pimu, off_qf, off_kv, off_nfound, off_ncand, off_next, off_defer;
+    int off_nb, off_pw, off_pimu, off_qf, off_kv, off_lst, off_ncand, off_next, off_defer;
     int off_wave, wave_bytes, off_vox, off_scratch;
     int off_wpart, off_winfo, total;
     int off_pose;
@@ -896,7 +999,7 @@
     L.off_pimu = o;    o += up16(kpb * 3 * 8);
     L.off_qf = o;      o += up16(kpb * 8 * 4);
     L.off_kv = o;      o += up16((kpb + 2) * 4 * 4);
-    L.off_nfound = o;  o += up16(kpb * 4);
+    L.off_lst = o;     o += up16(kpb * 4);
     L.off_ncand = o;   o += up16(kpb * 4);
     L.off_next = o;    o += 16;
     L.off_defer = o;   o += up16(kpb * 2);
@@ -1044,7 +1147,7 @@
 #endif
 __host__ __device__ constexpr int p2_keypoints_per_wave(int kpb) { return 64 / p2_lanes_per_keypoint(kpb); }
 
-template <int NB, int FAST, int KPW, int WPB, int DBG = 0, int ARMED = 0>
+template <int NB, int FAST, int KPW, int WPB, int DBG = 0, int ARMED = 0, int LREAD = 0>
 __device__ __forceinline__ bool assoc_tile(KargBytes karg, const SrlAssocArgs &A, const int tile) {
     constexpr int KPB = WPB * KPW;
     extern __shared__ __attribute__((aligned(16))) unsigned char smem[];
@@ -1062,7 +1165,7 @@
     double *s_pimu = reinterpret_cast<double *>(smem + L.off_pimu);
     float *s_qf = reinterpret_cast<float *>(smem + L.off_qf);
     int *s_kv = reinterpret_cast<int *>(smem + L.off_kv);
-    int *s_nfound = reinterpret_cast<int *>(smem + L.off_nfound);
+    unsigned *s_lst = reinterpret_cast<unsigned *>(smem + L.off_lst);
     int *s_ncand = reinterpret_cast<int *>(smem + L.off_ncand);
     int *s_next = reinterpret_cast<int *>(smem + L.off_next);
     unsigned short *s_defer = reinterpret_cast<unsigned short *>(smem + L.off_defer);
@@ -1094,6 +1197,13 @@
     tile_stamp(10);
     bool use_bounds = A.bound_in != nullptr && A.bound_use > 0;
     if constexpr (ARMED) use_bounds = use_bounds && reinterpret_cast<const int *>(s_pose + SRL_POSE_DOUBLES)[2] == 0 && n_pass() == A.n;
+    bool use_lists = false, write_lists = false;
+    if constexpr (NB == 1 && FAST != 0 && LREAD != 0) {
+        use_lists = A.lists != nullptr && A.list_use > 0;
+        if constexpr (ARMED) use_lists = use_lists && reinterpret_cast<const int *>(s_pose + SRL_POSE_DOUBLES)[2] == 0 && n_pass() == A.n;
+    } else if constexpr (NB == 1 && FAST != 0) {
+        write_lists = A.lists != nullptr && !use_bounds;
+    }
     const int bbase_kp = tile * KPB;
     const int wbase_kp = bbase_kp + wave * KPW;
 
@@ -1161,11 +1271,22 @@
             qf[5] = r2;
             *reinterpret_cast<double *>(qf + 6) = __builtin_huge_val();
         }
+        int list_n = 0, list_pk = 0;
+        if (LREAD != 0 && use_lists && g < A.list_use && g < n_pass()) {
+            const float4 ha = reinterpret_cast<const float4 *>(A.lists)[2 * (size_t)g];
+            const uint4 hb = reinterpret_cast<const uint4 *>(A.lists)[2 * (size_t)g + 1];
+            const float qxf = (float)p_w.x, qyf = (float)p_w.y, qzf = (float)p_w.z;
+            const float ex = qxf - ha.x, ey = qyf - ha.y, ez = qzf - ha.z;
+            const float mag = fmaxf(fabsf(qxf) + fabsf(qyf) + fabsf(qzf), fabsf(ha.x) + fabsf(ha.y) + fabsf(ha.z));
+            const float moved = 2.0f * (sqrtf(ex * ex + ey * ey + ez * ez) * 1.000001f) + (1e-3f + 1e-6f * mag);
+            const bool same_key = hb.x == (((unsigned)kv[0] & 0xFFFFu) | ((unsigned)kv[1] << 16)) && (hb.y & 0xFFFFu) == ((unsigned)kv[2] & 0xFFFFu);
+            if (same_key && moved <= ha.w) { list_n = (int)(hb.y >> 16); list_pk = (int)hb.z; }
+        }
         s_kv[kq * 4 + 0] = kv[0];
         s_kv[kq * 4 + 1] = kv[1];
         s_kv[kq * 4 + 2] = kv[2];
-        s_nfound[kq] = 0;
-        s_ncand[kq] = 0;
+        s_lst[kq] = (unsigned)list_n;
+        s_ncand[kq] = list_pk;
     } else if (wave == WPB - 1 && lane < KPW + 2) {
         const int kq = KPB + (lane - KPW);
         s_kv[kq * 4 + 0] = 0; s_kv[kq * 4 + 1] = 0; s_kv[kq * 4 + 2] = 0;
@@ -1191,20 +1312,83 @@
             const int nv = probe_voxels<NB>(qx, qy, qz, A.size_voxel, A.thr_cap, A.table, A.table_mask, vox, lane);
             select_topk(qx, qy, qz, nv, vox, A.slabs, Kn, tie ? 5 : A.select_mode, surv, lane, sink, total, fb);
             n_fallback += (NB == 1) ? 1 : fb;
-            if (lane == 0) {
-                s_nfound[kl] = total < Kn ? total : Kn;
-                s_ncand[kl] = total;
-            }
+            if (lane == 0) s_ncand[kl] = total;
         };
         if constexpr (NB == 1 && FAST != 0) {
             const LaneRole role = lane_role(lane);
             const int npairs = n_here > 0 ? (n_here + 1) >> 1 : 0;
-            auto take = [&]() { int p = 0; if (lane == 0) p = atomicAdd(s_next, 1); return __builtin_amdgcn_readfirstlane(p); };
+            auto list_ents = [&](int pr) -> const unsigned * {
+                return reinterpret_cast<const unsigned *>(A.lists + 32 * (size_t)A.list_cap) + (size_t)(bbase_kp + 2 * pr) * SRL_LIST_CAP;
+            };
+            int n_probed = npairs;
+            if constexpr (LREAD != 0) {
+                int nl = 0, np = 0;
+                for (int base = 0; base < npairs; base += 64) {
+                    const int pr = base + lane;
+                    bool is_l = false;
+                    if (pr < npairs && use_lists) is_l = s_lst[2 * pr] != 0u && (s_lst[2 * pr + 1] != 0u || 2 * pr + 1 >= n_here);
+                    const bool is_p = pr < npairs && !is_l;
+                    const unsigned long long ml = __ballot(is_l), mp = __ballot(is_p);
+                    if (is_l) s_kv[4 * (nl + lanes_below(ml)) + 3] = pr;
+                    if (is_p) s_kv[4 * (npairs - 1 - (np + lanes_below(mp))) + 3] = pr;
+                    nl += __popcll(ml); np += __popcll(mp);
+                }
+                __builtin_amdgcn_wave_barrier();
+                n_probed = np;
+                int pr_next = 0;
+                unsigned ea = 0u, eb = 0u;
+                auto fetch = [&](int ord) {
+                    if (ord < nl) {
+                        pr_next = __builtin_amdgcn_readfirstlane(s_kv[4 * ord + 3]);
+                        const unsigned *e = list_ents(pr_next);
+                        unsigned l = (unsigned)lane;
+                        asm volatile("" : "+v"(l));
+                        ea = e[l];
+                        eb = e[(2 * pr_next + 1 < n_here ? SRL_LIST_CAP : 0) + l];
+                    }
+                };
+                auto take_l = [&]() { int p = 0; if (lane == 0) p = atomicAdd(s_next, 1); return __builtin_amdgcn_readfirstlane(p); };
+                int n_served = 0;
+                int ord = take_l();
+                fetch(ord);
+                while (ord < nl) {
+                    const int nxt = take_l();
+                    const int kl = 2 * pr_next;
+                    const unsigned oa = ea, ob = eb;
+                    fetch(nxt);
+                    const int na = (int)__builtin_amdgcn_readfirstlane(s_lst[kl]);
+                    const int nb = kl + 1 < n_here ? (int)__builtin_amdgcn_readfirstlane(s_lst[kl + 1]) : 0;
+                    LdsSink sink_a = make_sink(kl), sink_b = make_sink(kl + 1);
+                    const int done = select_pair_list(s_pw + kl * 3, s_pw + kl * 3 + 3, s_qf + kl * 8, s_qf + kl * 8 + 8, oa, ob, na, nb, A.slabs, A.inf_off, Kn,
+                                                      surv, lane, sink_a, sink_b);
+                    const bool ok_a = (done & 0xFF) == SEL_DONE, ok_b = (done >> 8) == SEL_DONE;
+                    if (lane == 0) {
+                        if (!ok_a) s_defer[atomicAdd(s_next + 1, 1)] = (unsigned short)(kl | ((done & 0xFF) == SEL_TIE ? 0x8000 : 0));
+                        if (!ok_b) s_defer[atomicAdd(s_next + 1, 1)] = (unsigned short)((kl + 1) | ((done >> 8) == SEL_TIE ? 0x8000 : 0));
+                    }
+                    n_served += (ok_a ? 1 : 0) + ((ok_b && nb > 0) ? 1 : 0);
+                    ord = nxt;
+                }
+                if (lane == 0) s_winfo[wave * 8 + 7] = n_served;
+            }
+            auto take = [&]() {
+                int p = 0;
+                if (lane == 0) p = atomicAdd(s_next + (LREAD != 0 ? 3 : 0), 1);
+                p = __builtin_amdgcn_readfirstlane(p);
+                if constexpr (LREAD != 0) p = p < n_probed ? __builtin_amdgcn_readfirstlane(s_kv[4 * (npairs - 1 - p) + 3]) : npairs;
+                return p;
+            };
+            ListOut lout;
+            lout.ent = nullptr; lout.word = nullptr; lout.wmax = SRL_LIST_WIDEN * (float)A.size_voxel;
             int cur = take();
             ProbeReq preq;
             if (!(abl & 32)) preq = probe_issue(s_kv, 2 * (cur < npairs ? cur : npairs), role, A.table, A.table_mask, lane);
             while (cur < npairs) {
                 const int nxt = take();
+                if (LREAD == 0 && write_lists) {
+                    lout.ent = const_cast<unsigned *>(list_ents(cur));
+                    lout.word = s_lst + 2 * cur;
+                }
                 const int nv_pair = __builtin_amdgcn_readfirstlane((abl & 8) ? 0 : probe_finish(preq, A.thr_cap, A.table, A.table_mask, vox, lane, s_ncand + 2 * cur, use_bounds, s_qf + 16 * cur,
                                                                                                                s_kv + 8 * cur, &role, (float)A.size_voxel));
                 if (!(abl & 32)) preq = probe_issue(s_kv, 2 * (nxt < npairs ? nxt : npairs), role, A.table, A.table_mask, lane);
@@ -1221,9 +1405,9 @@
                     const int kl = 2 * cur;
                     LdsSink sink_a = make_sink(kl), sink_b = make_sink(kl + 1);
                     int total_a = 0, total_b = 0, done;
-                    if (r_max <= 2) done = select_pair_f32_r<2>(s_pw + kl * 3, s_pw + kl * 3 + 3, s_qf + kl * 8, s_qf + kl * 8 + 8, vox, A.slabs, A.inf_off, Kn, surv, lane, role, sink_a, sink_b, total_a, total_b, abl);
-                    else if (r_max <= 3) done = select_pair_f32_r<3>(s_pw + kl * 3, s_pw + kl * 3 + 3, s_qf + kl * 8, s_qf + kl * 8 + 8, vox, A.slabs, A.inf_off, Kn, surv, lane, role, sink_a, sink_b, total_a, total_b, abl);
-                    else done = select_pair_f32_r<4>(s_pw + kl * 3, s_pw + kl * 3 + 3, s_qf + kl * 8, s_qf + kl * 8 + 8, vox, A.slabs, A.inf_off, Kn, surv, lane, role, sink_a, sink_b, total_a, total_b, abl);
+                    if (r_max <= 2) done = select_pair_f32_r<2>(s_pw + kl * 3, s_pw + kl * 3 + 3, s_qf + kl * 8, s_qf + kl * 8 + 8, vox, A.slabs, A.inf_off, Kn, surv, lane, role, sink_a, sink_b, total_a, total_b, abl, lout);
+                    else if (r_max <= 3) done = select_pair_f32_r<3>(s_pw + kl * 3, s_pw + kl * 3 + 3, s_qf + kl * 8, s_qf + kl * 8 + 8, vox, A.slabs, A.inf_off, Kn, surv, lane, role, sink_a, sink_b, total_a, total_b, abl, lout);
+                    else done = select_pair_f32_r<4>(s_pw + kl * 3, s_pw + kl * 3 + 3, s_qf + kl * 8, s_qf + kl * 8 + 8, vox, A.slabs, A.inf_off, Kn, surv, lane, role, sink_a, sink_b, total_a, total_b, abl, lout);
                     (void)total_a; (void)total_b;
                     if (done != (SEL_DONE | (SEL_DONE << 8))) {
                         if (lane == 0) {
@@ -1241,7 +1425,9 @@
                         LdsSink sink = make_sink(kl);
                         int total = nv_fast;
                         int done = SEL_DONE;
-                        if (!(abl & 4)) done = select_topk_f32(qx, qy, qz, s_qf + kl * 8, nv_fast, vox + 32 * h, A.slabs, A.inf_off, Kn, surv, lane, role, sink, total, abl);
+                        ListOut lone = lout;
+                        if (lone.ent != nullptr) { lone.ent += SRL_LIST_CAP * h; lone.word += h; }
+                        if (!(abl & 4)) done = select_topk_f32(qx, qy, qz, s_qf + kl * 8, nv_fast, vox + 32 * h, A.slabs, A.inf_off, Kn, surv, lane, role, sink, total, abl, lone);
                         if (lane == 0) file(kl, done, total);
                     }
                 }
@@ -1262,7 +1448,6 @@
                 total = total_all;
                 if (lane == 0) {
                     if (done == SEL_DONE) {
-                        s_nfound[kl] = total < Kn ? total : Kn;
                         s_ncand[kl] = total;
                     } else {
                         s_defer[atomicAdd(s_next + 1, 1)] = (unsigned short)(kl | (done == SEL_TIE ? 0x8000 : 0));
@@ -1410,6 +1595,29 @@
         bo.w = (float)tau * 1.0000002f;
         reinterpret_cast<float4 *>(b.bound_out)[g] = bo;
     }
+    if constexpr (NB == 1 && FAST != 0 && LREAD == 0) {
+        bool wr = b.lists != nullptr && !(b.bound_in != nullptr && b.bound_use > 0);
+        if constexpr (ARMED) wr = b.lists != nullptr && !(b.bound_in != nullptr && b.bound_use > 0 && reinterpret_cast<const int *>(s_pose + SRL_POSE_DOUBLES)[2] == 0 && n2 == b.n);
+        if (wr && g < n2 && sl == 0) {
+            const float *qf = reinterpret_cast<const float *>(smem + L.off_qf) + kl * 8;
+            const int *kv = reinterpret_cast<const int *>(smem + L.off_kv) + kl * 4;
+            const double tau = *reinterpret_cast<const double *>(qf + 6);
+            const unsigned w = s_lst[kl];
+            const unsigned nl = w & 127u;
+            const float rho = __uint_as_float(w & ~127u);
+            float spare = -1.0f;
+            if (nl > 0u && tau < __builtin_huge_val()) spare = (rho - sqrtf((float)tau * 1.0000002f) * 1.000001f) * 0.999999f - 1e-6f;
+            float4 ha;
+            ha.x = qf[0]; ha.y = qf[1]; ha.z = qf[2]; ha.w = spare;
+            uint4 hb;
+            hb.x = ((unsigned)kv[0] & 0xFFFFu) | ((unsigned)kv[1] << 16);
+            hb.y = ((unsigned)kv[2] & 0xFFFFu) | (nl << 16);
+            hb.z = (unsigned)s_ncand[kl];
+            hb.w = w & ~127u;
+            reinterpret_cast<float4 *>(b.lists)[2 * (size_t)g] = ha;
+            reinterpret_cast<uint4 *>(b.lists)[2 * (size_t)g + 1] = hb;
+        }
+    }
     if (g < n2 && b.write_rec && sl == 0) {
         double2 *r = reinterpret_cast<double2 *>(b.rec + (size_t)g * 8);
         double2 v;
@@ -1509,7 +1717,8 @@
     if (tid == 0) {
         SrlBlockInfo bi;
         bi.accepted = 0; bi.sum_pk = 0; bi.nan_first = 0; bi.num_fallback = 0; bi.planes = 0;
-        bi.pad[0] = bi.pad[1] = bi.pad[2] = 0;
+        bi.served = 0; bi.pad[0] = bi.pad[1] = 0;
+        if constexpr (NB == 1 && FAST != 0 && LREAD != 0) for (int w = 0; w < WPB; ++w) bi.served += s_winfo[w * 8 + 7];
         for (int w = 0; w < WPB; ++w) bi.num_fallback += s_winfo[w * 8 + 3];
         for (int w = 0; w < P2W; ++w) {
             bi.accepted += s_winfo[w * 8 + 0]; bi.sum_pk += (unsigned)s_winfo[w * 8 + 1];
@@ -1779,7 +1988,7 @@
 #endif
 }
 
-template <int NB, int FAST, int KPW, int WPB, int DBG = 0, int ARMED = 0>
+template <int NB, int FAST, int KPW, int WPB, int DBG = 0, int ARMED = 0, int LREAD = 0>
 __device__ __forceinline__ void assoc_body(const SrlAssocArgs &a) {
     constexpr int KPB = WPB * KPW;
     extern __shared__ __attribute__((aligned(16))) unsigned char smem[];
@@ -1891,7 +2100,7 @@
         }
 #endif
     }
-    if (assoc_tile<NB, FAST, KPW, WPB, DBG, ARMED>((KargBytes)__builtin_amdgcn_kernarg_segment_ptr(), a, (int)blockIdx.x)) return;
+    if (assoc_tile<NB, FAST, KPW, WPB, DBG, ARMED, LREAD>((KargBytes)__builtin_amdgcn_kernarg_segment_ptr(), a, (int)blockIdx.x)) return;
     double row_v = 0.0;
     constexpr int P2W_T = (KPB + p2_keypoints_per_wave(KPB) - 1) / p2_keypoints_per_wave(KPB);
     if (tid < 32) {
@@ -1956,13 +2165,13 @@
     if constexpr (ARMED) arm_stamp((KargBytes)__builtin_amdgcn_kernarg_segment_ptr(), 7);
 }
 
-template <int NB, int FAST, int KPW, int WPB, int DBG = 0>
+template <int NB, int FAST, int KPW, int WPB, int DBG = 0, int LREAD = 0>
 __global__ void __launch_bounds__(64 * WPB, WPB == 16 ? 1 : SRL_ASSOC_WAVES_PER_SIMD) srl_assoc_kernel(const SrlAssocArgs a) {
-    assoc_body<NB, FAST, KPW, WPB, DBG>(a);
-}
-template <int NB, int KPW>
+    assoc_body<NB, FAST, KPW, WPB, DBG, 0, LREAD>(a);
+}
+template <int NB, int KPW, int LREAD = 0>
 __global__ void __launch_bounds__(1024, 1) srl_assoc_armed_kernel(const SrlAssocArgs a) {
-    assoc_body<NB, 1, KPW, 16, 0, 1>(a);
+    assoc_body<NB, 1, KPW, 16, 0, 1, LREAD>(a);
 }
 __global__ void __launch_bounds__(1024) srl_reduce_kernel(const SrlReduceArgs a, int mode_in) {
     __shared__ long long s_wtot[16];
@@ -2227,11 +2436,16 @@
         return hipGetLastError();
     };
     const bool fast = a.select_mode == 0 || a.select_mode == 4;
+    const bool lread = a.lists != nullptr && a.list_use > 0 && nb_voxels == 1 && fast;
     if (armed) {
-        if constexpr (WPB == 16) { if (fast && a.ablate == 0) return nb_voxels == 1 ? launch(srl_assoc_armed_kernel<1, KPW>) : launch(srl_assoc_armed_kernel<2, KPW>); }
+        if constexpr (WPB == 16) {
+            if (fast && a.ablate == 0 && lread) return launch(srl_assoc_armed_kernel<1, KPW, 1>);
+            if (fast && a.ablate == 0) return nb_voxels == 1 ? launch(srl_assoc_armed_kernel<1, KPW>) : launch(srl_assoc_armed_kernel<2, KPW>);
+        }
         return hipErrorInvalidConfiguration;
     }
-    if constexpr (KPW == 16 && WPB == 16) { if (a.ablate != 0 && nb_voxels == 1 && fast) return launch(srl_assoc_kernel<1, 1, 16, 16, 1>); }
+    if constexpr (KPW == 16 && WPB == 16) { if (a.ablate != 0 && nb_voxels == 1 && fast) return lread ? launch(srl_assoc_kernel<1, 1, 16, 16, 1, 1>) : launch(srl_assoc_kernel<1, 1, 16, 16, 1>); }
+    if (lread) return launch(srl_assoc_kernel<1, 1, KPW, WPB, 0, 1>);
     if (nb_voxels == 1) return fast ? launch(srl_assoc_kernel<1, 1, KPW, WPB>) : launch(srl_assoc_kernel<1, 0, KPW, WPB>);
     return fast ? launch(srl_assoc_kernel<2, 1, KPW, WPB>) : launch(srl_assoc_kernel<2, 0, KPW, WPB>);
 }
diff --git a/sr_livo_amd/csrc/srl_map_kernels.hip b/sr_livo_amd/csrc/srl_map_kernels.hip
--- a/sr_livo_amd/csrc/srl_map_kernels.hip
+++ b/sr_livo_amd/csrc/srl_map_kernels.hip
@@ -358,7 +358,7 @@
     HIPCHK(ctx, hipGetLastError());
     ctx->num_voxels = V_new;
     ctx->num_points -= pts_removed;
-    ctx->bound_n = 0;
+    ctx->void_neighbourhoods();
     ctx->taps_valid = false;
     if (num_voxels_removed) *num_voxels_removed = V - V_new;
     if (num_points_removed) *num_points_removed = pts_removed;
@@ -474,7 +474,7 @@
     if (report && report->num_cloud) *report->num_cloud = 0;
     if (n == 0) return SRL_OK;
     if (!(voxel_size > 0.0)) return SRL_ERR_BAD_ARG;
-    ctx->bound_n = 0;
+    ctx->void_neighbourhoods();
     HIPCHK(ctx, hipSetDevice(ctx->device));
     hipStream_t st = ctx->stream;
     { const int rcs = srl_map_settle(ctx); if (rcs) return rcs; }
```

Measured after the change: 9537 sweeps/s. 0.888x the previous value.
